# medvedevgroup/TwoPaCo

Measured on AMD Instinct MI355X. Metric: kmers_hashed_per_sec, higher is better.
Workload: dtype u64

## Files before the change

### include/twopaco_hip.h

```cpp
#ifndef TWOPACO_HIP_H_
#define TWOPACO_HIP_H_

#include <stddef.h>
#include <stdint.h>

#ifdef __cplusplus
extern "C" {
#endif

typedef struct tpc_ctx tpc_ctx;

#define TPC_MAX_Q 64
#define TPC_INVALID_VERTEX INT64_MAX

enum {
    TPC_K_FILTER_RESET = 0,
    TPC_K_INSERT = 1,
    TPC_K_QUERY = 2,
    TPC_K_COMPACT = 3,
    TPC_K_FILTER2 = 4,
    TPC_K_SCAN2 = 5,
    TPC_K_SORT = 6,
    TPC_K_EMIT = 7,
    TPC_K_SPLIT = 8,
// ... 44 lines not shown
                         uint32_t *bins_host);

int tpc_pass1_query(tpc_ctx *ctx, uint64_t lo, uint64_t hi, uint64_t *n_marks);
int tpc_pass1_query_begin(tpc_ctx *ctx, uint64_t lo, uint64_t hi);

int tpc_pass2_filter(tpc_ctx *ctx, uint64_t abundance, uint64_t *n_true, uint64_t *n_false, uint64_t *table_size);

int tpc_pass2_marks(tpc_ctx *ctx, uint64_t *n_marks);
int tpc_pass2_mark_owners(tpc_ctx *ctx, uint32_t world, uint64_t *pos_dev, int32_t *owner_dev);
int tpc_pass2_filter_positions(tpc_ctx *ctx, const uint64_t *pos_dev, uint64_t n, uint64_t abundance, uint64_t *n_true, uint64_t *n_false,
                               uint64_t *table_size);
int tpc_pass2_mark_records(tpc_ctx *ctx, uint32_t world, uint64_t *records_dev, int32_t *owner_dev);
int tpc_pass2_filter_records(tpc_ctx *ctx, const uint64_t *records_dev, uint64_t n, uint64_t abundance, uint64_t *n_true, uint64_t *n_false,
                             uint64_t *table_size);
int tpc_pass2_aggregate_records(tpc_ctx *ctx, uint32_t world, uint64_t abundance, uint64_t *records_dev, int32_t *owner_dev, uint64_t *n_records);
int tpc_pass2_filter_aggregated(tpc_ctx *ctx, const uint64_t *records_dev, uint64_t n, uint64_t abundance, uint64_t *n_true, uint64_t *n_false,
                                uint64_t *table_size);
int tpc_shard_permute_rows(tpc_ctx *ctx, const uint64_t *src_dev, const uint32_t *perm_dev, uint64_t n, int row_words, uint64_t *dst_dev);

int tpc_junctions_finalize(tpc_ctx *ctx, uint64_t *n_junctions);

int tpc_key_words(const tpc_ctx *ctx);

int tpc_junction_keys(tpc_ctx *ctx, uint64_t *keys_host);

int tpc_junction_keys_raw(tpc_ctx *ctx, uint64_t *keys_host, uint64_t *n);
int tpc_junction_keys_set(tpc_ctx *ctx, const uint64_t *keys_host, uint64_t n);
int tpc_junction_keys_export(tpc_ctx *ctx, uint64_t *dst_dev, uint64_t cap_keys, uint64_t *n);
int tpc_junction_keys_import(tpc_ctx *ctx, const uint64_t *src_dev, uint64_t n, int append);

int64_t tpc_get_id(tpc_ctx *ctx, const char *kmer);

int tpc_emit(tpc_ctx *ctx, uint64_t *n_marked, uint64_t *n_valid);
int tpc_emit_fetch(tpc_ctx *ctx, uint64_t *g_host, int64_t *id_host);

int tpc_emit_export(tpc_ctx *ctx, uint64_t *g_dev, int64_t *id_dev);
int tpc_emit_import(tpc_ctx *ctx, const uint64_t *g_dev, const int64_t *id_dev, uint64_t n);

int tpc_emit_stream(tpc_ctx *ctx, const uint64_t *rec_start, const uint64_t *rec_len, uint32_t n_rec, uint64_t *n_bytes, uint64_t *n_records);
int tpc_emit_stream_fetch(tpc_ctx *ctx, uint64_t offset, uint64_t nbytes, void *dst_host);

int tpc_shard_chunk(const tpc_ctx *ctx, uint64_t *chunk_lo, uint64_t *chunk_hi);
int tpc_emit_stream_partial(tpc_ctx *ctx, const uint64_t *rec_start, const uint64_t *rec_len, uint32_t n_rec, uint64_t *cnt_host, uint32_t *flags_host);
int tpc_emit_stream_part(tpc_ctx *ctx, const uint64_t *rec_start, const uint64_t *rec_len, uint32_t n_rec, const uint32_t *gflags_host,
                         const uint64_t *e_scan_host, const uint64_t *s_scan_host, const uint64_t *before_host, uint32_t r_last,
                         uint64_t chunk_lo, uint64_t chunk_hi, uint64_t slot0, uint64_t n_slots, uint64_t *n_bytes);
int tpc_host_alloc(void **ptr, uint64_t bytes);
void tpc_host_free(void *ptr);

int tpc_shard_verify_local(tpc_ctx *ctx);

int tpc_shard_periodic_copy(tpc_ctx *ctx);
int tpc_periodic_download(tpc_ctx *ctx, uint32_t *qs_host, uint32_t *planes_host, uint32_t *ins_host);

#define TPC_SHARD_INSERT 0
#define TPC_SHARD_QUERY 1
int tpc_shard_config(tpc_ctx *ctx, uint32_t rank, uint32_t world);
int tpc_shard_plan(tpc_ctx *ctx, int pass, uint64_t lo, uint64_t hi, uint64_t *geom);
int tpc_shard_hash(tpc_ctx *ctx, int pass, uint64_t batch, uint64_t lo, uint64_t hi, void *send_regions_dev, void *send_counts_dev,
                   uint64_t *n_overflow);
int tpc_shard_plan_both(tpc_ctx *ctx, uint64_t lo, uint64_t hi, uint64_t *geom_insert , uint64_t *geom_query );
int tpc_shard_hash_begin(tpc_ctx *ctx, int pass, uint64_t batch, uint64_t lo, uint64_t hi, void *send_regions_dev, void *send_counts_dev);
int tpc_shard_hash_end(tpc_ctx *ctx, int pass, uint64_t *n_overflow);
int tpc_shard_overflow_get(tpc_ctx *ctx, int pass, void *dst_dev, uint64_t n);
int tpc_shard_overflow_set(tpc_ctx *ctx, int pass, const void *src_dev, uint64_t n);
int tpc_shard_apply(tpc_ctx *ctx, int pass, uint64_t batch, const void *recv_regions_dev, const void *recv_counts_dev, uint64_t *n_survivors);
int tpc_shard_pack(tpc_ctx *ctx, int pass, const void *send_regions_dev, const void *send_counts_dev, void *packed_dev, uint64_t *bytes_per_dest_host);
int tpc_shard_apply_packed(tpc_ctx *ctx, int pass, uint64_t batch, const void *recv_packed_dev, const void *recv_counts_dev, uint64_t *n_survivors);
int tpc_shard_apply_inplace(tpc_ctx *ctx, int pass, uint64_t batch, const void *recv_regions_dev, const void *recv_counts_dev,
                            const void *send_regions_dev, const void *send_counts_dev, uint64_t *n_survivors);
int tpc_shard_survivors(tpc_ctx *ctx, uint64_t *sid_dev);
int tpc_shard_survivors_home(tpc_ctx *ctx, uint64_t *tmp_dev, uint64_t *send_dev, uint64_t *counts_host);
int tpc_shard_verify_send(tpc_ctx *ctx, int fn, int fn_count, const uint64_t *sid_dev, uint64_t n, uint64_t *tmp_dev, uint64_t *send_dev, uint32_t *perm_dev,
                          uint64_t *counts_host);
int tpc_shard_finish(tpc_ctx *ctx, const uint64_t *sid_dev, uint64_t n, int fn_count, const uint8_t *hit_dev, const uint32_t *perm_dev, uint64_t *n_marked);
int tpc_shard_survivor_sources(tpc_ctx *ctx, const uint64_t *sid_dev, uint64_t n, int32_t *source_dev);
int tpc_shard_verify_addrs(tpc_ctx *ctx, int fn, int fn_count, const uint64_t *sid_dev, uint64_t n, uint64_t *addr_dev, int32_t *owner_dev);
int tpc_shard_probe(tpc_ctx *ctx, const uint64_t *addr_dev, uint64_t n, uint8_t *hit_dev);
int tpc_shard_mark(tpc_ctx *ctx, const uint64_t *sid_dev, uint64_t n);
int tpc_shard_route(tpc_ctx *ctx, const int32_t *owner_dev, uint64_t n, uint32_t *perm_dev, uint64_t *counts_host);
int tpc_shard_permute64(tpc_ctx *ctx, const uint64_t *src_dev, const uint32_t *perm_dev, uint64_t n, uint64_t *dst_dev);
int tpc_shard_select(tpc_ctx *ctx, const uint64_t *sid_dev, uint64_t n, int fn_count, const uint8_t *hit_dev, const uint32_t *perm_dev,
                     uint64_t *sid_out_dev, uint64_t *n_out);
int tpc_mask_export(tpc_ctx *ctx, uint32_t *dst_dev);
int tpc_mask_merge(tpc_ctx *ctx, const uint32_t *src_dev, uint32_t count);
int tpc_mask_export_padded(tpc_ctx *ctx, uint32_t *dst_dev, uint64_t total_words);
int tpc_mask_or_blocks(tpc_ctx *ctx, const uint32_t *blocks_dev, uint32_t count, uint64_t words, uint32_t *out_dev);
int tpc_mask_import(tpc_ctx *ctx, const uint32_t *src_dev);

int tpc_combine_info(tpc_ctx *ctx, uint32_t n_dest, uint64_t *info );
int tpc_combine_export(tpc_ctx *ctx, uint32_t n_dest, uint16_t *payload_dev, uint64_t cap_units, uint64_t *dir_dev, uint64_t *units_host);
int tpc_combine_merge(tpc_ctx *ctx, uint32_t n_src, const uint16_t *payload_dev, const uint64_t *src_base_host, const uint64_t *dir_dev, uint16_t *out_payload_dev,
                      uint64_t out_cap_units, uint64_t *out_dir_dev, uint64_t *units_host);
int tpc_combine_import(tpc_ctx *ctx, uint32_t n_src, uint32_t n_owner, const uint16_t *payload_dev, const uint64_t *src_base_host, const uint64_t *dir_dev, uint64_t dir_stride);
int tpc_combine_choose(uint32_t world, int L, uint64_t mean_export_units, double *bytes );
int tpc_filter_copy_out(tpc_ctx *ctx, uint64_t word0, uint64_t n_words, uint32_t *dst_dev);
int tpc_filter_copy_in(tpc_ctx *ctx, uint64_t word0, uint64_t n_words, const uint32_t *src_dev);

#define TPC_SEG_OK 0
#define TPC_SEG_CORRUPTED 1
#define TPC_SEG_ID_TOO_LARGE 2
int tpc_segments_build_host(tpc_ctx *ctx, const void *stream_host, uint64_t n_bytes, int k, const uint64_t *rec_start, const uint64_t *rec_len,
                            uint32_t n_rec, const uint64_t *amb_pos, uint64_t n_amb);
int tpc_segments_build_resident(tpc_ctx *ctx, int k, const uint64_t *rec_start, const uint64_t *rec_len, uint32_t n_rec, const uint64_t *amb_pos,
                                uint64_t n_amb);
int tpc_segments_counts(const tpc_ctx *ctx, uint64_t *counts );
// ... 106 lines not shown
```

### twopaco_amd/capi.py

```python
import ctypes
import os

import numpy as np

from .build import lib_dir

INVALID_VERTEX = (1 << 63) - 1
DISTANCES_TILE = 32
KERNELS = {"fused": 12, "filter_reset": 0, "insert": 1, "query": 2, "compact": 3, "filter2": 4, "scan2": 5, "sort": 6, "emit": 7, "split": 8,
           "shard_hash": 9, "shard_apply": 10, "stream": 11, "lookup": 13, "combine": 14, "segments": 15, "segtext": 16, "sketch": 17, "colors": 18, "links": 19, "bubbles": 20,
           "distances": 21, "components": 22, "superbubbles": 23, "anchors": 24, "locate": 25, "classes": 26, "tracks": 27, "variants": 28}

HIP_SYMBOLS = ["tpc_ctx_create", "tpc_ctx_destroy", "tpc_last_error", "tpc_set_params", "tpc_seq_upload",
               "tpc_run_begin", "tpc_filter_reset", "tpc_pass1_insert", "tpc_pass1_split_hist", "tpc_pass1_query", "tpc_pass2_filter",
               "tpc_junctions_finalize", "tpc_key_words", "tpc_junction_keys", "tpc_junction_keys_raw", "tpc_junction_keys_set", "tpc_get_id", "tpc_emit",
               "tpc_emit_fetch", "tpc_filter_words", "tpc_filter_download", "tpc_mask_words", "tpc_mask_download",
               "tpc_hash_dump", "tpc_kernel_ms", "tpc_set_option",
               "tpc_shard_config", "tpc_shard_plan", "tpc_shard_hash", "tpc_shard_overflow_get", "tpc_shard_overflow_set", "tpc_shard_apply",
               "tpc_shard_pack", "tpc_shard_apply_packed", "tpc_pass2_marks", "tpc_pass2_mark_owners", "tpc_pass2_filter_positions",
               "tpc_pass2_mark_records", "tpc_pass2_filter_records", "tpc_pass2_aggregate_records", "tpc_pass2_filter_aggregated", "tpc_shard_permute_rows", "tpc_emit_export", "tpc_emit_import",
               "tpc_shard_survivors", "tpc_shard_survivor_sources", "tpc_shard_verify_addrs", "tpc_shard_probe", "tpc_shard_mark", "tpc_mask_export", "tpc_mask_merge",
               "tpc_shard_route", "tpc_shard_permute64", "tpc_shard_select", "tpc_mask_export_padded", "tpc_mask_or_blocks", "tpc_mask_import",
               "tpc_emit_stream", "tpc_emit_stream_fetch", "tpc_host_alloc", "tpc_host_free", "tpc_get_stat", "tpc_filter_upload",
               "tpc_junction_keys_export", "tpc_junction_keys_import", "tpc_warmup", "tpc_preload", "tpc_reserve", "tpc_shard_chunk", "tpc_emit_stream_partial", "tpc_emit_stream_part",
               "tpc_shard_plan_both", "tpc_shard_hash_begin", "tpc_shard_hash_end", "tpc_shard_apply_inplace", "tpc_shard_survivors_home", "tpc_shard_verify_send", "tpc_shard_finish", "tpc_shard_verify_local", "tpc_shard_periodic_copy", "tpc_periodic_download",
               "tpc_pass1_query_begin", "tpc_combine_info", "tpc_combine_export", "tpc_combine_merge", "tpc_combine_import", "tpc_combine_choose", "tpc_filter_copy_out", "tpc_filter_copy_in",
               "tpc_segments_build_host", "tpc_segments_build_resident", "tpc_segments_counts", "tpc_segments_error", "tpc_segments_fetch_names", "tpc_segments_fetch_first",
               "tpc_segments_fetch_events", "tpc_segments_fetch_sequences", "tpc_segments_text_plan", "tpc_segments_text_fetch", "tpc_segments_text_write", "tpc_distinct_sketch",
               "tpc_segments_colors_build", "tpc_segments_colors_info", "tpc_segments_colors_fetch_rows", "tpc_segments_colors_fetch_presence", "tpc_segments_colors_fetch_hist",
               "tpc_segments_links_build", "tpc_segments_links_info", "tpc_segments_links_fetch_rows", "tpc_segments_links_fetch_first",
               "tpc_segments_bubbles_build", "tpc_segments_bubbles_info", "tpc_segments_bubbles_fetch_rows", "tpc_segments_bubbles_fetch_sides", "tpc_segments_bubbles_fetch_hist",
               "tpc_segments_distances_build", "tpc_segments_distances_info", "tpc_segments_distances_fetch",
               "tpc_segments_components_build", "tpc_segments_components_info", "tpc_segments_components_fetch_members", "tpc_segments_components_fetch_rows",
               "tpc_segments_components_fetch_presence",
               "tpc_segments_superbubbles_build", "tpc_segments_superbubbles_info", "tpc_segments_superbubbles_fetch_adjacency", "tpc_segments_superbubbles_fetch_exits",
               "tpc_segments_superbubbles_fetch_rows", "tpc_segments_superbubbles_fetch_members", "tpc_segments_superbubbles_fetch_presence",
               "tpc_segments_anchors_build", "tpc_segments_anchors_info", "tpc_segments_anchors_fetch_mates", "tpc_segments_anchors_fetch_rows",
               "tpc_segments_anchors_fetch_shared",
               "tpc_segments_edges_build", "tpc_segments_edges_info", "tpc_segments_locate", "tpc_segments_locate_info", "tpc_segments_locate_fetch_hits",
               "tpc_segments_locate_fetch_runs", "tpc_segments_locate_fetch_records", "tpc_segments_locate_fetch_shared",
               "tpc_segments_classes_build", "tpc_segments_classes_info", "tpc_segments_classes_fetch_members", "tpc_segments_classes_fetch_rows",
               "tpc_segments_classes_fetch_presence", "tpc_segments_classes_fetch_sets",
               "tpc_segments_tracks_build", "tpc_segments_tracks_info", "tpc_segments_tracks_fetch_rows", "tpc_segments_tracks_fetch_colors",
               "tpc_segments_tracks_fetch_depth",
               "tpc_segments_variants_build", "tpc_segments_variants_info", "tpc_segments_variants_fetch_traversals", "tpc_segments_variants_fetch_alleles",
               "tpc_segments_variants_fetch_presence", "tpc_segments_variants_fetch_sites", "tpc_segments_variants_fetch_hist"]
VARIANTS_NONE = 0xFFFFFFFF
TRACKS_ALL = 0xFFFFFFFF
SEGMENT_ERRORS = {0: None, 1: "The input is corrupted", 2: "A vertex id is too large, cannot generate GFA"}

_hip = None
_host = None


def combine_choose(world, L, mean_export_units):
    b = (ctypes.c_double * 3)()
    mode = hip().tpc_combine_choose(world, L, int(mean_export_units), b)
    return mode, [float(x) for x in b]


def _load(name):
    path = os.path.join(lib_dir(), name)
    if not os.path.exists(path):
        raise RuntimeError("%s is missing: run `python -c 'import __graft_entry__ as g; g.build()'` (no CPU fallback)" % path)
    return ctypes.CDLL(path, mode=ctypes.RTLD_GLOBAL)


def hip():
    global _hip
    if _hip is None:
        L = _load("libtwopaco_hip.so")
        u64, i64, p, ci = ctypes.c_uint64, ctypes.c_int64, ctypes.c_void_p, ctypes.c_int
        L.tpc_ctx_create.argtypes = [ci, ctypes.POINTER(p)]
        L.tpc_ctx_destroy.argtypes = [p]
        L.tpc_last_error.restype = ctypes.c_char_p
        L.tpc_last_error.argtypes = [p]
        L.tpc_set_params.argtypes = [p, ci, ci, ci, p]
        L.tpc_seq_upload.argtypes = [p, p, p, u64]
# ... 5 lines not shown
        L.tpc_pass2_filter.argtypes = [p, u64, p, p, p]
        L.tpc_junctions_finalize.argtypes = [p, p]
        L.tpc_key_words.argtypes = [p]
        L.tpc_junction_keys.argtypes = [p, p]
        L.tpc_junction_keys_raw.argtypes = [p, p, p]
        L.tpc_junction_keys_set.argtypes = [p, p, u64]
        L.tpc_junction_keys_export.argtypes = [p, p, u64, p]
        L.tpc_junction_keys_import.argtypes = [p, p, u64, ci]
        L.tpc_get_id.restype = i64
        L.tpc_get_id.argtypes = [p, ctypes.c_char_p]
        L.tpc_emit.argtypes = [p, p, p]
        L.tpc_emit_fetch.argtypes = [p, p, p]
        L.tpc_filter_words.restype = u64
        L.tpc_filter_words.argtypes = [p]
        L.tpc_filter_download.argtypes = [p, p]
        L.tpc_filter_upload.argtypes = [p, p]
        L.tpc_warmup.argtypes = [p]
        L.tpc_preload.argtypes = [ctypes.c_int]
        L.tpc_reserve.argtypes = [p, u64]
        L.tpc_mask_words.restype = u64
        L.tpc_mask_words.argtypes = [p]
        L.tpc_mask_download.argtypes = [p, ci, p]
        L.tpc_hash_dump.argtypes = [p, u64, u64, p]
        L.tpc_kernel_ms.restype = ctypes.c_double
        L.tpc_kernel_ms.argtypes = [p, ci]
        L.tpc_set_option.argtypes = [p, ctypes.c_char_p, i64]
        u32 = ctypes.c_uint32
        L.tpc_shard_config.argtypes = [p, u32, u32]
        L.tpc_shard_plan.argtypes = [p, ci, u64, u64, p]
        L.tpc_shard_hash.argtypes = [p, ci, u64, u64, u64, p, p, p]
        L.tpc_shard_plan_both.argtypes = [p, u64, u64, p, p]
        L.tpc_shard_hash_begin.argtypes = [p, ci, u64, u64, u64, p, p]
        L.tpc_shard_hash_end.argtypes = [p, ci, p]
        L.tpc_shard_overflow_get.argtypes = [p, ci, p, u64]
        L.tpc_shard_overflow_set.argtypes = [p, ci, p, u64]
        L.tpc_shard_apply.argtypes = [p, ci, u64, p, p, p]
        L.tpc_pass2_marks.argtypes = [p, p]
        L.tpc_pass2_mark_owners.argtypes = [p, u32, p, p]
        L.tpc_pass2_filter_positions.argtypes = [p, p, u64, u64, p, p, p]
        L.tpc_pass2_mark_records.argtypes = [p, u32, p, p]
        L.tpc_pass2_filter_records.argtypes = [p, p, u64, u64, p, p, p]
        L.tpc_pass2_aggregate_records.argtypes = [p, u32, u64, p, p, p]
        L.tpc_pass2_filter_aggregated.argtypes = [p, p, u64, u64, p, p, p]
        L.tpc_shard_permute_rows.argtypes = [p, p, p, u64, ci, p]
        L.tpc_shard_pack.argtypes = [p, ci, p, p, p, p]
        L.tpc_shard_apply_packed.argtypes = [p, ci, u64, p, p, p]
        L.tpc_shard_apply_inplace.argtypes = [p, ci, u64, p, p, p, p, p]
        L.tpc_shard_survivors_home.argtypes = [p, p, p, p]
        L.tpc_shard_verify_send.argtypes = [p, ci, ci, p, u64, p, p, p, p]
        L.tpc_shard_finish.argtypes = [p, p, u64, ci, p, p, p]
        L.tpc_shard_verify_local.argtypes = [p]
        L.tpc_shard_periodic_copy.argtypes = [p]
        L.tpc_periodic_download.argtypes = [p, p, p, p]
        L.tpc_pass1_query_begin.argtypes = [p, u64, u64]
        L.tpc_combine_info.argtypes = [p, u32, p]
        L.tpc_combine_export.argtypes = [p, u32, p, u64, p, p]
        L.tpc_combine_merge.argtypes = [p, u32, p, p, p, p, u64, p, p]
        L.tpc_combine_import.argtypes = [p, u32, u32, p, p, p, u64]
        L.tpc_combine_choose.argtypes = [u32, ci, u64, p]
        L.tpc_filter_copy_out.argtypes = [p, u64, u64, p]
        L.tpc_filter_copy_in.argtypes = [p, u64, u64, p]
        L.tpc_shard_survivors.argtypes = [p, p]
        L.tpc_shard_verify_addrs.argtypes = [p, ci, ci, p, u64, p, p]
        L.tpc_shard_survivor_sources.argtypes = [p, p, u64, p]
        L.tpc_shard_probe.argtypes = [p, p, u64, p]
        L.tpc_shard_mark.argtypes = [p, p, u64]
        L.tpc_mask_export.argtypes = [p, p]
        L.tpc_mask_merge.argtypes = [p, p, u32]
        L.tpc_shard_route.argtypes = [p, p, u64, p, p]
        L.tpc_shard_permute64.argtypes = [p, p, p, u64, p]
        L.tpc_shard_select.argtypes = [p, p, u64, ci, p, p, p, p]
        L.tpc_mask_export_padded.argtypes = [p, p, u64]
        L.tpc_mask_or_blocks.argtypes = [p, p, u32, u64, p]
        L.tpc_mask_import.argtypes = [p, p]
        L.tpc_emit_stream.argtypes = [p, p, p, u32, p, p]
        L.tpc_emit_stream_fetch.argtypes = [p, u64, u64, p]
        L.tpc_emit_import.argtypes = [p, p, p, u64]
        L.tpc_shard_chunk.argtypes = [p, p, p]
        L.tpc_emit_stream_partial.argtypes = [p, p, p, u32, p, p]
        L.tpc_emit_stream_part.argtypes = [p, p, p, u32, p, p, p, p, u32, u64, u64, u64, u64, p]
        L.tpc_segments_build_host.argtypes = [p, p, u64, ci, p, p, u32, p, u64]
        L.tpc_segments_build_resident.argtypes = [p, ci, p, p, u32, p, u64]
        L.tpc_segments_counts.argtypes = [p, p]
        L.tpc_segments_error.argtypes = [p, p, p]
        L.tpc_segments_fetch_names.argtypes = [p, u64, u64, p]
        L.tpc_segments_fetch_first.argtypes = [p, u64, u64, p]
        L.tpc_segments_fetch_events.argtypes = [p, u64, u64, p, p]
        L.tpc_segments_fetch_sequences.argtypes = [p, u64, u64, p]
        L.tpc_segments_text_plan.argtypes = [p, ci, p, p, p, p]
        L.tpc_segments_text_fetch.argtypes = [p, u64, u64, p]
        L.tpc_segments_text_write.argtypes = [p, ci, u64, u64, p]
        L.tpc_segments_colors_build.argtypes = [p, p, u32]
        L.tpc_segments_colors_info.argtypes = [p, p]
        L.tpc_segments_colors_fetch_rows.argtypes = [p, u64, u64, p, p, p, p]
        L.tpc_segments_colors_fetch_presence.argtypes = [p, u64, u64, p]
        L.tpc_segments_colors_fetch_hist.argtypes = [p, p, p]
        L.tpc_segments_links_build.argtypes = [p]
        L.tpc_segments_links_info.argtypes = [p, p]
        L.tpc_segments_links_fetch_rows.argtypes = [p, u64, u64, p, p, p]
        L.tpc_segments_links_fetch_first.argtypes = [p, u64, u64, p]
        L.tpc_segments_bubbles_build.argtypes = [p]
        L.tpc_segments_bubbles_info.argtypes = [p, p]
        L.tpc_segments_bubbles_fetch_rows.argtypes = [p, u64, u64, p, p, p, p]
        L.tpc_segments_bubbles_fetch_sides.argtypes = [p, u64, u64, p, p, p]
        L.tpc_segments_bubbles_fetch_hist.argtypes = [p, p]
        L.tpc_segments_distances_build.argtypes = [p]
# ... 863 lines not shown
    def shard_overflow_set(self, which, src_ptr, n):
        self._ck(hip().tpc_shard_overflow_set(self._h, which, src_ptr, n))

    def shard_apply(self, which, batch, recv_regions_ptr, recv_counts_ptr):
        n = ctypes.c_uint64(0)
        self._ck(hip().tpc_shard_apply(self._h, which, batch, recv_regions_ptr, recv_counts_ptr, ctypes.byref(n)))
        return n.value

    def shard_pack(self, which, send_regions_ptr, send_counts_ptr, packed_ptr, world):
        out = (ctypes.c_uint64 * world)()
        self._ck(hip().tpc_shard_pack(self._h, which, send_regions_ptr, send_counts_ptr, packed_ptr, out))
        return [int(x) for x in out]

    def shard_apply_packed(self, which, batch, recv_packed_ptr, recv_counts_ptr):
        n = ctypes.c_uint64(0)
        self._ck(hip().tpc_shard_apply_packed(self._h, which, batch, recv_packed_ptr, recv_counts_ptr, ctypes.byref(n)))
        return n.value

    def shard_apply_inplace(self, which, batch, recv_regions_ptr, recv_counts_ptr, send_regions_ptr, send_counts_ptr):
        n = ctypes.c_uint64(0)
        self._ck(hip().tpc_shard_apply_inplace(self._h, which, batch, recv_regions_ptr, recv_counts_ptr, send_regions_ptr, send_counts_ptr, ctypes.byref(n)))
        return n.value

    def shard_survivors_home(self, tmp_ptr, send_ptr, world):
        out = (ctypes.c_uint64 * world)()
        self._ck(hip().tpc_shard_survivors_home(self._h, tmp_ptr, send_ptr, out))
        return [int(x) for x in out]

    def shard_verify_send(self, fn, fn_count, sid_ptr, n, tmp_ptr, send_ptr, perm_ptr, world):
        out = (ctypes.c_uint64 * world)()
        self._ck(hip().tpc_shard_verify_send(self._h, fn, fn_count, sid_ptr, n, tmp_ptr, send_ptr, perm_ptr, out))
        return [int(x) for x in out]

    def shard_finish(self, sid_ptr, n, fn_count, hit_ptr, perm_ptr):
        m = ctypes.c_uint64(0)
        self._ck(hip().tpc_shard_finish(self._h, sid_ptr, n, fn_count, hit_ptr, perm_ptr, ctypes.byref(m)))
        return m.value

    def shard_periodic_copy(self):
        self._ck(hip().tpc_shard_periodic_copy(self._h))

    def periodic_download(self):
        nw = hip().tpc_mask_words(self._h)
        qs, planes, ins = np.zeros(nw, dtype=np.uint32), np.zeros((6, nw), dtype=np.uint32), np.zeros(nw, dtype=np.uint32)
        self._ck(hip().tpc_periodic_download(self._h, qs.ctypes.data, planes.ctypes.data, ins.ctypes.data))

        def bits(w):
            return np.unpackbits(w.astype("<u4").view(np.uint8), bitorder="little")

        dist = np.zeros(nw * 32, dtype=np.uint8)
        for b in range(6):
            dist |= bits(planes[b]) << b
        return bits(qs).astype(bool), dist, bits(ins).astype(bool)

    def shard_verify_local(self):
        self._ck(hip().tpc_shard_verify_local(self._h))

    def shard_survivors(self, sid_ptr):
        self._ck(hip().tpc_shard_survivors(self._h, sid_ptr))

    def shard_survivor_sources(self, sid_ptr, n, src_ptr):
        self._ck(hip().tpc_shard_survivor_sources(self._h, sid_ptr, n, src_ptr))

    def shard_verify_addrs(self, fn, fn_count, sid_ptr, n, addr_ptr, owner_ptr):
        self._ck(hip().tpc_shard_verify_addrs(self._h, fn, fn_count, sid_ptr, n, addr_ptr, owner_ptr))

    def shard_probe(self, addr_ptr, n, hit_ptr):
        self._ck(hip().tpc_shard_probe(self._h, addr_ptr, n, hit_ptr))

    def shard_mark(self, sid_ptr, n):
        self._ck(hip().tpc_shard_mark(self._h, sid_ptr, n))

    def mask_export(self, dst_ptr):
        self._ck(hip().tpc_mask_export(self._h, dst_ptr))

    def mask_merge(self, src_ptr, count):
        self._ck(hip().tpc_mask_merge(self._h, src_ptr, count))

    def mask_words(self):
        return int(hip().tpc_mask_words(self._h))

    def shard_route(self, owner_ptr, n, perm_ptr, world):
        counts = np.zeros(64, dtype=np.uint64)
        self._ck(hip().tpc_shard_route(self._h, owner_ptr, n, perm_ptr, counts.ctypes.data))
        return [int(x) for x in counts[:world]]

    def shard_permute64(self, src_ptr, perm_ptr, n, dst_ptr):
        self._ck(hip().tpc_shard_permute64(self._h, src_ptr, perm_ptr, n, dst_ptr))

    def shard_select(self, sid_ptr, n, fn_count, hit_ptr, perm_ptr, out_ptr):
        m = ctypes.c_uint64(0)
        self._ck(hip().tpc_shard_select(self._h, sid_ptr, n, fn_count, hit_ptr, perm_ptr, out_ptr, ctypes.byref(m)))
        return m.value

    def mask_export_padded(self, dst_ptr, total_words):
        self._ck(hip().tpc_mask_export_padded(self._h, dst_ptr, total_words))

    def mask_or_blocks(self, blocks_ptr, count, words, out_ptr):
        self._ck(hip().tpc_mask_or_blocks(self._h, blocks_ptr, count, words, out_ptr))

    def mask_import(self, src_ptr):
        self._ck(hip().tpc_mask_import(self._h, src_ptr))

    def combine_info(self, n_dest):
        g = np.zeros(8, dtype=np.uint64)
        self._ck(hip().tpc_combine_info(self._h, n_dest, g.ctypes.data))
# ... 175 lines not shown
```

### twopaco_amd/csrc/tpc_capi.hip

```cpp
#include "tpc_ctx.h"

namespace tpch {

int fail(tpc_ctx *c, int code, const char *fmt, ...)
{
    char buf[512];
    va_list ap;
    va_start(ap, fmt);
    vsnprintf(buf, sizeof buf, fmt, ap);
    va_end(ap);
    if (c) c->err = buf;
    return code;
}





TpcLaunch make_launch(const tpc_ctx *c)
{
    TpcLaunch a;
    a.P = c->P; a.tab = c->tab; a.bases = c->bases; a.nmask = c->nmask; a.n_text = c->n_text;
    a.n_tiles = c->n_tiles; a.filter = c->filter; a.stream = c->stream;
    a.stat_kernel = c->stat_kernel;
    a.stat_split = c->stat_split;
    if (c->P.k <= TPC_QSEED_MAXK) a.qseed = c->tab + TPC_TAB_WORDS;
    return a;
}

TpcLaunch make_launch_periodic(const tpc_ctx *c)
{
    TpcLaunch a = make_launch(c);
    if (c->periodic && c->periodic_valid) {
        if (c->periodic_any_q) a.per_qs = c->periodic;
        if (c->periodic_any_i) a.per_i = c->periodic + (size_t)(1 + TPC_PER_PLANES) * c->n_words_alloc;
    }
    return a;
}

void ensure_periodic(tpc_ctx *c)
{
    if (c->periodic_valid || !c->opt_periodic || !c->bases || !c->have_params || c->n_words_alloc == 0) return;
    if ((c->sh_world > 1 || c->text_windowed) && !c->opt_shard_periodic && !replicated(c)) return;
    TpcLaunch a = make_launch(c);
    const uint64_t w0 = c->text_windowed ? c->text_w0 : 0, w1 = c->text_windowed ? std::min(c->text_w1, c->n_words) : c->n_words;
    const uint64_t pos_hi = c->text_windowed ? c->text_w1 << 5 : ~0ull;
    uint32_t any[2] = {0, 0};
    uint32_t *flags = reinterpret_cast<uint32_t *>(c->counters + 6);
    if (hipMemsetAsync(flags, 0, sizeof any, c->stream) != hipSuccess) return;
    tpc_launch_periodic_build(a, nullptr, nullptr, 0, nullptr, w0, w1, w0 << 5, pos_hi, flags);
    if (hipMemcpyAsync(any, flags, sizeof any, hipMemcpyDeviceToHost, c->stream) != hipSuccess || hipStreamSynchronize(c->stream) != hipSuccess) return;
    c->periodic_any_q = any[0] != 0; c->periodic_any_i = any[1] != 0;
    if (any[0] || any[1]) {
        const size_t words = (size_t)(2 + TPC_PER_PLANES) * c->n_words_alloc;
        if (!c->periodic && hipMalloc((void **)&c->periodic, words * sizeof(uint32_t)) != hipSuccess) { (void)hipGetLastError(); c->periodic = nullptr; return; }
        if (hipMemsetAsync(c->periodic, 0, words * sizeof(uint32_t), c->stream) != hipSuccess) return;
        tpc_launch_periodic_build(a, c->periodic, c->periodic + c->n_words_alloc, c->n_words_alloc, c->periodic + (size_t)(1 + TPC_PER_PLANES) * c->n_words_alloc, w0, w1, w0 << 5, pos_hi, flags);
        if (hipStreamSynchronize(c->stream) != hipSuccess) return;
    }
    c->periodic_valid = true;
}

uint64_t rotln_host(uint64_t x, int L, int r)
{
    if (r == 0) return x;
    const uint64_t maskn = (1ull << (L - r)) - 1ull;
    return ((x & maskn) << r) | (x >> (L - r));
}

std::atomic<int> tpc_test_fail_mallocs{0};
hipError_t dev_malloc(tpc_ctx *c, void **p, size_t bytes)
{
    hipError_t e = hipErrorOutOfMemory;
    if (tpc_test_fail_mallocs.load(std::memory_order_relaxed) > 0 && tpc_test_fail_mallocs.fetch_sub(1) > 0) *p = nullptr; else e = hipMalloc(p, bytes);
    if (e == hipSuccess) return e;
    (void)hipGetLastError();
    if (!release_partition_buffers(c)) return e;
    e = hipMalloc(p, bytes);
    if (e != hipSuccess) *p = nullptr;
    return e;
}


int read_counter(tpc_ctx *c, int i, uint64_t *out)
{
    unsigned long long v = 0;
    HIPCHK(c, hipMemcpyAsync(&v, c->counters + i, sizeof v, hipMemcpyDeviceToHost, c->stream));
    HIPCHK(c, hipStreamSynchronize(c->stream));
    *out = v;
    return 0;
// ... 167 lines not shown
        if ((rc = read_counter(c, 2, &n))) return rc;
    }
    rc = ensure(c, c->marks, c->marks_cap, n);
    if (rc) return rc;
    if (n) tpc_launch_mask_scatter(c->stream, m, c->n_words, c->block_sums, c->marks);
    c->n_marks = n;
    return 0;
}

}

extern "C" {

int tpc_ctx_create(int device, tpc_ctx **out)
{
    if (!out) return -1;
    *out = nullptr;
    int n = 0;
    if (hipGetDeviceCount(&n) != hipSuccess || n <= 0) return -2;
    if (device < 0 || device >= n) return -3;
    if (hipSetDevice(device) != hipSuccess) return -4;
    tpc_ctx *c = new tpc_ctx();
    c->device = device;
    c->dbg_ovf = getenv("TPC_DEBUG_OVF") != nullptr; c->dbg_phases = getenv("TPC_PROFILE_PHASES") != nullptr; c->dbg_timing = getenv("TWOPACO_TIMING") != nullptr; c->no_lean = TpcEnv::get().no_lean;
    if (const char *e = getenv("TPC_SHARD_TIGHT")) c->opt_shard_tight = atoi(e) ? 1 : 0;
    if (hipStreamCreate(&c->stream) != hipSuccess) { delete c; return -5; }
    for (int i = 0; i < TPC_K_COUNT; i++) {
        if (hipEventCreate(&c->ev0[i]) != hipSuccess || hipEventCreate(&c->ev1[i]) != hipSuccess) { delete c; return -5; }
    }
    if (hipMalloc((void **)&c->tab, sizeof c->tab_host) != hipSuccess ||
        hipMalloc((void **)&c->counters, 8 * sizeof(unsigned long long)) != hipSuccess ||
        hipMalloc((void **)&c->route_scratch, 128 * sizeof(unsigned long long)) != hipSuccess) { delete c; return -6; }
    *out = c;
    return 0;
}

void tpc_ctx_destroy(tpc_ctx *c)
{
    if (!c) return;
    (void)hipSetDevice(c->device);
    (void)hipStreamSynchronize(c->stream);
    void *ptrs[] = { c->tab, c->bases_alloc, c->nmask_alloc, c->filter, c->rmask, c->mask, c->marks, c->block_sums, c->table,
                     c->keys, c->idtab, c->emit_id, c->stream_buf, c->counters, c->route_scratch, c->sh_off, c->scan_blocks, c->sort_scratch, c->seg.name, c->seg.first, c->seg.ev[0], c->seg.ev[1], c->seg.ev[2],
                     c->seg.rec, c->seg.amb, c->text_plan.off, c->text_plan.piece, c->text_names, c->text_win };
    for (void *p : ptrs) if (p) (void)hipFree(p);
    stream_part_release(c);
    colors_drop(c);
    links_drop(c);
    anchors_drop(c);
    edges_drop(c);
    for (void *p : c->pbuf) if (p) (void)hipFree(p);
    for (void *p : c->ikeep) if (p) (void)hipFree(p);
    if (c->periodic) (void)hipFree(c->periodic);
    if (c->cmb_base) (void)hipFree(c->cmb_base);
    if (c->cmb_cur) (void)hipFree(c->cmb_cur);
    if (c->ikeep_ovf) (void)hipFree(c->ikeep_ovf);
    if (c->iovf_cnt) (void)hipFree(c->iovf_cnt);
    if (c->iovf_off) (void)hipFree(c->iovf_off);
    for (int i = 0; i < TPC_K_COUNT; i++) { if (c->ev0[i]) (void)hipEventDestroy(c->ev0[i]); if (c->ev1[i]) (void)hipEventDestroy(c->ev1[i]); }
    if (c->stream2) (void)hipStreamDestroy(c->stream2);
    if (c->stream) (void)hipStreamDestroy(c->stream);
    delete c;
}

const char *tpc_last_error(const tpc_ctx *c) { return c ? c->err.c_str() : "null context"; }

int tpc_set_option(tpc_ctx *c, const char *name, int64_t value)
{
    if (!c || !name) return -1;
    if (!strcmp(name, "insert_test_first")) { c->opt_test_first = value != 0; return 0; }
    if (!strcmp(name, "insert_mode")) { c->opt_insert_mode = (int)value; return 0; }
    if (!strcmp(name, "slice_bits")) { c->opt_slice_bits = (int)value; return 0; }
    if (!strcmp(name, "query_mode")) { c->opt_query_mode = (int)value; return 0; }
    if (!strcmp(name, "part_budget_bytes")) { c->opt_part_budget = value; return 0; }
    if (!strcmp(name, "part_levels")) { c->opt_part_levels = (int)value; return 0; }
    if (!strcmp(name, "shard_tight_regions")) { c->opt_shard_tight = value ? 1 : 0; c->sh_have[0] = c->sh_have[1] = false; return 0; }
    if (!strcmp(name, "part_min_tiles")) { c->opt_part_min_tiles = value < 1 ? 1 : value; return 0; }
    if (!strcmp(name, "verify_marks")) { c->opt_verify_marks = value != 0; return 0; }
    if (!strcmp(name, "mark_bucket_bits")) { tpc_test_mark_bucket_bits = (int)value; return 0; }
    if (!strcmp(name, "mark_region_cap")) { tpc_test_mark_region_cap = (int)value; return 0; }
    if (!strcmp(name, "mark_slice_bits")) { tpc_test_mark_slice_bits = (int)value; return 0; }
    if (!strcmp(name, "qhash_pushes")) { tpc_opt_qhash_pushes = value == 8 ? 8 : 6; return 0; }
    if (!strcmp(name, "qhash_roll_scalars")) { tpc_opt_qhash_roll = value != 0; return 0; }
    if (!strcmp(name, "qhash_seed_scalars")) { tpc_opt_qhash_seed = value != 0; return 0; }
    if (!strcmp(name, "fuse_apply_lookup")) { c->opt_fuse = value != 0; return 0; }
    if (!strcmp(name, "test_q6_pb2")) { tpc_test_q6_pb2 = (int)value; return 0; }
    if (!strcmp(name, "insert_entry_fmt")) { tpc_test_insert_p3 = value == 3; return 0; }
    if (!strcmp(name, "shard_periodic_skip")) { c->opt_shard_periodic = value != 0; return 0; }
    if (!strcmp(name, "periodic_skip")) { c->opt_periodic = value != 0; if (!value) c->periodic_valid = false; return 0; }
    if (!strcmp(name, "test_tight_pinch")) { tpc_test_tight_pinch = (int)value; c->sh_have[0] = c->sh_have[1] = false; return 0; }
    if (!strcmp(name, "test_sched_cap")) { tpc_test_sched_cap = value > 0 ? (uint32_t)value : 0; return 0; }
    if (!strcmp(name, "test_mask_scan")) { tpc_test_mask_scan = value == 1 || value == 2 ? (int)value : 0; return 0; }
    if (!strcmp(name, "text_window")) { c->opt_text_window = value != 0; return 0; }
    if (!strcmp(name, "replicate_filter")) { c->opt_replicate = value != 0; return 0; }
    if (!strcmp(name, "test_force_anyq")) { tpc_test_force_anyq = value != 0; return 0; }
    if (!strcmp(name, "test_sketch_grid")) { tpc_test_sketch_grid = value > 0 ? (int)value : 0; return 0; }
    if (!strcmp(name, "test_links_slots_log2")) { c->opt_links_slots_log2 = (int)std::max<int64_t>(-1, std::min<int64_t>(value, 64)); return 0; }
    if (!strcmp(name, "test_edges_slots_log2")) { c->opt_edges_slots_log2 = (int)std::max<int64_t>(-1, std::min<int64_t>(value, 64)); return 0; }
    if (!strcmp(name, "test_edges_hash_bits")) { c->opt_edges_hash_bits = (int)std::max<int64_t>(-1, std::min<int64_t>(value, 65)); return 0; }
    if (!strcmp(name, "test_locate_grid")) { c->opt_locate_grid = value > 0 ? (int)std::min<int64_t>(value, 1 << 20) : 0; return 0; }
    if (!strcmp(name, "test_distances_chunk_words")) { c->opt_distances_chunk_words = (int)std::max<int64_t>(-1, std::min<int64_t>(value, 1 << 20)); return 0; }
    if (!strcmp(name, "test_components_step_limit")) { c->opt_components_step_limit = (int)std::max<int64_t>(-1, std::min<int64_t>(value, 0x7FFFFFFF)); return 0; }
    if (!strcmp(name, "test_classes_slots_log2")) { c->opt_classes_slots_log2 = (int)std::max<int64_t>(-1, std::min<int64_t>(value, 64)); return 0; }
    if (!strcmp(name, "test_classes_hash_bits")) { c->opt_classes_hash_bits = (int)std::max<int64_t>(-1, std::min<int64_t>(value, 65)); return 0; }
    if (!strcmp(name, "test_classes_grid")) { c->opt_classes_grid = value > 0 ? (int)std::min<int64_t>(value, 1 << 20) : 0; return 0; }
    if (!strcmp(name, "test_classes_wide")) { c->opt_classes_wide = (int)std::max<int64_t>(-1, std::min<int64_t>(value, 3)); return 0; }
    if (!strcmp(name, "test_tracks_grid")) { c->opt_tracks_grid = value > 0 ? (int)std::min<int64_t>(value, 1 << 20) : 0; return 0; }
    if (!strcmp(name, "test_variants_grid")) { c->opt_variants_grid = value > 0 ? (int)std::min<int64_t>(value, 1 << 20) : 0; return 0; }
    if (!strcmp(name, "test_fail_mallocs")) { tpc_test_fail_mallocs.store(value > 0 ? (int)value : 0); return 0; }
    return fail(c, -1, "unknown option %s", name);
}

int tpc_preload(int device)
{
    if (hipSetDevice(device) != hipSuccess) { (void)hipGetLastError(); return -10; }
    const bool timing = getenv("TWOPACO_TIMING") != nullptr;
    int (*const warm[4])() = { tpc_warm_partition, tpc_warm_qpartition, tpc_warm_pass2, tpc_warm_stream };
    const char *const name[4] = { "partition", "qpartition", "pass2", "stream" };
    for (int i = 0; i < 4; i++) {
        const auto t0 = std::chrono::steady_clock::now();
        if (warm[i]() != 0) return -10;
        if (timing) fprintf(stderr, "[timing]     code object %s: %.1f ms\n", name[i], std::chrono::duration<double, std::milli>(std::chrono::steady_clock::now() - t0).count());
    }
    return 0;
}

int tpc_warmup(tpc_ctx *c)
{
    if (!c) return -1;
    return tpc_preload(c->device);
}

int64_t tpc_get_stat(const tpc_ctx *c, const char *name)
{
    if (!c || !name) return -1;
    if (!strcmp(name, "insert_path")) return c->stat_path[0];
    if (!strcmp(name, "query_path")) return c->stat_path[1];
    if (!strcmp(name, "insert_entry_fmt")) return c->stat_fmt[0];
    if (!strcmp(name, "query_entry_fmt")) return c->stat_fmt[1];
    if (!strcmp(name, "insert_hash_kernel")) return c->stat_kernel[0];
    if (!strcmp(name, "query_hash_kernel")) return c->stat_kernel[1];
    if (!strcmp(name, "query_verify_kernel")) return c->stat_kernel[2];
    if (!strcmp(name, "query_hash_form")) return c->stat_kernel[3];
    if (!strcmp(name, "query_hash_seed")) return c->stat_kernel[4];
    if (!strcmp(name, "split_kernel")) return c->stat_split[0];
    if (!strcmp(name, "split_phases")) return c->stat_split[1];
    if (!strcmp(name, "query_hash_seed_maxk")) return TPC_QSEED_MAXK;
    if (!strcmp(name, "query_mark_path")) return c->stat_mark_path;
    if (!strcmp(name, "query_mark_fallback")) return c->stat_mark_fallback;
    if (!strcmp(name, "insert_batches")) return c->stat_batches[0];
    if (!strcmp(name, "query_batches")) return c->stat_batches[1];
    if (!strcmp(name, "query_tiles_per_batch")) return c->stat_q_plan[0];
    if (!strcmp(name, "query_b1")) return c->stat_q_plan[1];
    if (!strcmp(name, "query_b2")) return c->stat_q_plan[2];
    if (!strcmp(name, "query_begun")) return c->stat_q_begun;
    if (!strcmp(name, "filter2_retries")) return c->stat_filter2_retries;
    if (!strcmp(name, "aggregate_retries")) return c->stat_aggregate_retries;
    if (!strcmp(name, "filter2_counted")) return c->stat_filter2_counted;
    if (!strcmp(name, "fused_lookups")) return c->stat_fused;
    if (!strcmp(name, "query_overflow_entries")) return c->stat_query_overflow;
    if (!strcmp(name, "insert_overflow_entries")) return c->stat_insert_overflow;
    if (!strcmp(name, "periodic_skip")) return c->periodic_valid ? 1 : 0;
    if (!strcmp(name, "pbuf_releases")) return c->stat_pbuf_releases;
    if (!strcmp(name, "distances_tile")) return TPC_DISTANCES_TILE;
    if (!strcmp(name, "text_words")) return (int64_t)(c->text_w1 - c->text_w0);
    if (!strcmp(name, "text_word_begin")) return (int64_t)c->text_w0;
    if (!strcmp(name, "text_word_end")) return (int64_t)c->text_w1;
    if (!strcmp(name, "periodic_any_query")) return c->periodic_valid && c->periodic_any_q ? 1 : 0;
    if (!strcmp(name, "periodic_any_insert")) return c->periodic_valid && c->periodic_any_i ? 1 : 0;
    if (!strcmp(name, "text_write_us")) return c->text_write_us;
    if (!strcmp(name, "text_wait_us")) return c->text_wait_us;
    if (!strcmp(name, "text_window_bytes")) return c->text_window_bytes;
    if (!strcmp(name, "device_free_bytes") || !strcmp(name, "device_total_bytes")) {
        size_t free_b = 0, total_b = 0;
        if (hipSetDevice(c->device) != hipSuccess || hipMemGetInfo(&free_b, &total_b) != hipSuccess) { (void)hipGetLastError(); return -1; }
        return (int64_t)(name[7] == 'f' ? free_b : total_b);
    }
    if (!strcmp(name, "mask_scan_form")) return tpc_stat_mask_scan_form.load(std::memory_order_relaxed);
    if (!strcmp(name, "round_marks")) return c->marks_valid ? (int64_t)c->n_marks : -1;
    return -1;
}

int tpc_set_params(tpc_ctx *c, int k, int L, int q, const uint64_t *seed_table)
{
    if (!c || !seed_table) return -1;
    if (q < 1 || q > TPC_MAX_Q) return fail(c, -1, "q=%d unsupported (1..%d)", q, TPC_MAX_Q);
    if (L < 2 || L > 62) return fail(c, -1, "filter bits L=%d unsupported (2..62)", L);
    if (k < 1) return fail(c, -1, "k must be positive");
    const int C = (k + 4 + 31) / 32;
    if (C >= 20)
        return fail(c, -1, "The value of K is too big. Please refer to documentaion how to increase the max supported value of K.");
    HIPCHK(c, hipSetDevice(c->device));
    c->P.k = k; c->P.L = L; c->P.q = q; c->P.rk = k % L; c->P.lmask = (1ull << L) - 1ull;
    if (C != c->C && c->keys) {
        (void)hipFree(c->keys);
        c->keys = nullptr; c->keys_cap = 0;
    }
    c->C = C;
    memset(c->tab_host, 0, sizeof c->tab_host);
    for (int i = 0; i < q; i++)
        for (int ch = 0; ch < 5; ch++) {
            const uint64_t h = seed_table[i * 5 + ch];
            if (h > c->P.lmask) return fail(c, -1, "seed table entry exceeds L bits");
            c->tab_host[i * 5 + ch] = h;
            c->tab_host[TPC_TAB_HK + i * 5 + ch] = rotln_host(h, L, c->P.rk);
        }
    if (k <= TPC_QSEED_MAXK)
        for (int t = 0; t < k; t++)
            for (int ch = 0; ch < 5; ch++) {
                const int rc = ch == 4 ? 4 : 3 - ch;
                c->tab_host[TPC_TAB_WORDS + (t * 5 + ch) * 2] = rotln_host(c->tab_host[ch], L, (k - 1 - t) % L);
                c->tab_host[TPC_TAB_WORDS + (t * 5 + ch) * 2 + 1] = rotln_host(c->tab_host[rc], L, t % L);
            }
    HIPCHK(c, hipMemcpy(c->tab, c->tab_host, sizeof c->tab_host, hipMemcpyHostToDevice));
    const uint64_t fw = filter_words_for(L, c->opt_replicate ? 1 : c->sh_world);
    c->sh_have[0] = c->sh_have[1] = false;
    c->pending_lists = false; c->cmb_have_geo = false;
    if (fw != c->filter_words) {
        if (c->filter) (void)hipFree(c->filter);
        c->filter = nullptr;
        HIPCHK(c, hipMalloc((void **)&c->filter, fw * sizeof(uint32_t)));
        c->filter_words = fw;
    }
    c->have_params = true;
    c->periodic_valid = false;
    c->pending_apply = false;
    c->qb_valid = false;
    c->n_keys = 0; c->finalized = false; c->rounds_done = 0; c->mask_dirty = false; c->marks_valid = false; c->rmask_sums_valid = false;
    return 0;
}

int tpc_seq_upload(tpc_ctx *c, const uint64_t *bases, const uint32_t *nmask, uint64_t n_text)
{
    if (!c || !bases || !nmask || n_text < 2) return fail(c, -1, "bad text");
    HIPCHK(c, hipSetDevice(c->device));
    const auto t_begin = std::chrono::steady_clock::now();
    c->qb_valid = false;
    const uint64_t nw = (n_text + 31) / 32;
    if (!((nmask[0] & 1u) && ((nmask[(n_text - 1) >> 5] >> ((n_text - 1) & 31)) & 1u)))
        return fail(c, -1, "text must start and end with the N separator");
    const uint64_t tiles = (nw + TPC_TILE_THREADS - 1) / TPC_TILE_THREADS;
    const uint64_t alloc = ((n_text / TPC_RUN + 512) / 512) * 512 + TPC_XW_MAX + 2;
    uint64_t w0 = 0, w1 = alloc;
    const bool windowed = c->opt_text_window && c->sh_world > 1;
    if (windowed) {
        const uint64_t t512 = (n_text / TPC_RUN + 512) / 512, chunk = (t512 + c->sh_world - 1) / c->sh_world;
        const uint64_t ta = std::min<uint64_t>(t512, (uint64_t)c->sh_rank * chunk), tb = std::min<uint64_t>(t512, ta + chunk);
        w0 = ta * 512 > 0 ? ta * 512 - 1 : 0;
        w1 = std::min<uint64_t>(alloc, tb * 512 + TPC_XW_MAX + 2);
        if (w1 <= w0) w1 = w0 + 1;
    }
    for (void *p : { (void *)c->bases_alloc, (void *)c->nmask_alloc, (void *)c->rmask, (void *)c->mask, (void *)c->block_sums, (void *)c->periodic })
        if (p) (void)hipFree(p);
    c->periodic = nullptr; c->periodic_valid = false;
    c->bases = nullptr; c->nmask = nullptr; c->bases_alloc = nullptr; c->nmask_alloc = nullptr; c->rmask = nullptr; c->mask = nullptr; c->block_sums = nullptr;
    const uint64_t wn = w1 - w0;
    HIPCHK(c, dev_malloc(c, (void **)&c->bases_alloc, wn * sizeof(uint64_t)));
    HIPCHK(c, dev_malloc(c, (void **)&c->nmask_alloc, wn * sizeof(uint32_t)));
    HIPCHK(c, dev_malloc(c, (void **)&c->rmask, alloc * sizeof(uint32_t)));
    HIPCHK(c, dev_malloc(c, (void **)&c->mask, alloc * sizeof(uint32_t)));
    HIPCHK(c, dev_malloc(c, (void **)&c->block_sums, (alloc / 256 + 2 + 64) * sizeof(uint64_t)));
    HIPCHK(c, hipMemsetAsync(c->bases_alloc, 0, wn * sizeof(uint64_t), c->stream));
    HIPCHK(c, hipMemsetAsync(c->nmask_alloc, 0xFF, wn * sizeof(uint32_t), c->stream));
    HIPCHK(c, hipMemsetAsync(c->rmask, 0, alloc * sizeof(uint32_t), c->stream));
    HIPCHK(c, hipMemsetAsync(c->mask, 0, alloc * sizeof(uint32_t), c->stream));
    const uint64_t ce = std::min(nw, w1);
    uint32_t last_word = 0;
    if (ce > w0) {
        HIPCHK(c, hipMemcpyAsync(c->bases_alloc, bases + w0, (ce - w0) * sizeof(uint64_t), hipMemcpyHostToDevice, c->stream));
        HIPCHK(c, hipMemcpyAsync(c->nmask_alloc, nmask + w0, (ce - w0) * sizeof(uint32_t), hipMemcpyHostToDevice, c->stream));
        if ((n_text & 31) && ce == nw) {
            last_word = nmask[nw - 1] | (~0u << (n_text & 31));
            HIPCHK(c, hipMemcpyAsync(c->nmask_alloc + (nw - 1 - w0), &last_word, sizeof last_word, hipMemcpyHostToDevice, c->stream));
        }
    }
    HIPCHK(c, hipStreamSynchronize(c->stream));
    if (c->dbg_timing)
        fprintf(stderr, "[timing]   tpc_seq_upload (allocations, %.0f MB host to device): %.1f ms\n", (double)(ce > w0 ? (ce - w0) * 12 : 0) / 1e6,
                std::chrono::duration<double, std::milli>(std::chrono::steady_clock::now() - t_begin).count());
    c->bases = c->bases_alloc - w0;
    c->nmask = c->nmask_alloc - w0;
    c->text_windowed = windowed; c->text_w0 = w0; c->text_w1 = w1;
    c->pending_apply = false;
    c->n_text = n_text; c->n_words = (n_text >> 5) + 1; c->n_words_alloc = alloc; c->n_tiles = tiles;
    c->text_uploads++;
    c->n_keys = 0; c->finalized = false; c->rounds_done = 0; c->mask_dirty = false; c->marks_valid = false; c->rmask_sums_valid = false;
    return 0;
}

int tpc_run_begin(tpc_ctx *c)
{
    if (!c) return -1;
    c->n_keys = 0; c->finalized = false; c->rounds_done = 0; c->mask_dirty = false; c->marks_valid = false; c->rmask_sums_valid = false;
    c->n_marks = 0; c->n_emit = 0; c->keys_host.clear();
    return 0;
}

int tpc_filter_reset(tpc_ctx *c)
{
    if (!c || !c->have_params) return fail(c, -1, "set_params first");
    c->filter_zero_pending = true;
    c->pending_apply = false;
    c->pending_shard = false;
    c->pending_lists = false;
    c->ev_used[TPC_K_FILTER_RESET] = false;
    return 0;
}

int tpc_pass1_insert(tpc_ctx *c, uint64_t lo, uint64_t hi, uint64_t *n_kmers)
{
    if (!c || !c->have_params || !c->bases) return fail(c, -1, "set_params and seq_upload first");
    if (c->sh_world > 1 && !c->opt_replicate) return fail(c, -1, "the filter is sharded: use tpc_shard_hash / tpc_shard_apply");
    HIPCHK(c, hipSetDevice(c->device));
    const bool gated = !(lo == 0 && hi >= c->P.lmask);
    { int rc0 = flush_pending_apply(c); if (rc0) return rc0; }
    c->qb_valid = false;
    ensure_periodic(c);
    if (n_kmers) HIPCHK(c, hipMemsetAsync(c->counters, 0, sizeof(unsigned long long), c->stream));
    uint64_t t_begin, t_end;
    pass_tiles(c, t_begin, t_end);
    TpcPartPlan pl;
    const double m_ins = gated ? range_mass(c, lo, hi) : 1.0;
    const double ins_frac = gated ? std::min(1.0, (1.0 - (1.0 - m_ins) * (1.0 - m_ins)) * 1.15) : 1.0;
    const uint64_t tiles = pass_tile_count(c);
    uint64_t batches = 1;
    bool defer = false;
    bool part = ((c->opt_insert_mode != 1 && !(c->opt_insert_mode == 0 && c->P.L < 28)) || replicated(c)) && part_hash_supported(c);
    if (replicated(c) && !part && c->P.q <= TPC_KERNEL_MAXQ)
        return fail(c, -1, "a replicated multi-GPU pass needs the partitioned hash kernels (q=%d, L=%d, slice_bits=%d are outside what they cover)", c->P.q, c->P.L, c->opt_slice_bits);
    if (part) {
        const int64_t budget = part_budget(c);
        for (;; batches = next_batches(batches)) {
            const uint64_t per = (tiles + batches - 1) / batches;
            if (!tpc_part_plan(c->P.L, c->P.q, c->opt_slice_bits, per, ins_frac, pl, c->opt_part_levels)) { part = false; break; }
            if ((int64_t)(std::max(tpc_part_buf1_bytes(pl), tpc_part_buf3_bytes(pl)) + tpc_part_buf2_bytes(pl)) <= budget || (int64_t)per <= c->opt_part_min_tiles) break;
        }
        if (part && c->opt_insert_mode == 0 && batches > 1 && !replicated(c)) {
            const double per_slice = (double)c->P.q * ins_frac * (double)pl.n_tiles * 512 * TPC_RUN / (double)(1ull << (c->P.L - pl.slice_bits));
            if (per_slice < (double)(1ull << pl.slice_bits) / 800.0) part = false;
        }
    }
    if (part) {
        size_t need[tpc_ctx::NPBUF] = { std::max(tpc_part_buf1_bytes(pl), tpc_part_buf3_bytes(pl)), tpc_part_cnt1_bytes(pl), tpc_part_buf2_bytes(pl), tpc_part_cnt2_bytes(pl),
                                        pl.ovf_cap * sizeof(uint64_t), 32 * sizeof(unsigned long long), 0, 0, 0, 0, tpc_part_cnt3_bytes(pl), 0 };
        TpcQPlan qpl;
        const bool qpart = plan_query(c, lo, hi, gated, qpl);
        for (int i = 0; i < tpc_ctx::NPBUF && qpart; i++) need[i] = std::max(need[i], qpart_need(qpl, i));
        for (int i = 0; i < tpc_ctx::NPBUF && part; i++) if (need[i]) part = ensure_pbuf(c, i, need[i]);
        defer = part && c->opt_fuse && batches == 1 && qpart && pl.b3 == 0 && qpl.b3 == 0 && qpl.slice_bits == pl.slice_bits &&
                qpl.b1 == pl.b1 && qpl.b2 == pl.b2 && (qpl.fmt == 6 || pl.fmt2 == 0);
        if (defer) {
            const size_t want[2] = { tpc_part_buf2_bytes(pl), tpc_part_cnt2_bytes(pl) };
            for (int i = 0; i < 2 && defer; i++) {
                if (want[i] <= c->ikeep_bytes[i]) continue;
                if (c->ikeep[i]) (void)hipFree(c->ikeep[i]);
                c->ikeep[i] = nullptr; c->ikeep_bytes[i] = 0;
                if (hipMalloc(&c->ikeep[i], want[i]) != hipSuccess) { (void)hipGetLastError(); defer = false; break; }
                c->ikeep_bytes[i] = want[i];
            }
        }
    }
    if (part) {
        pl.buf1 = (uint32_t *)c->pbuf[0]; pl.cnt1 = (uint32_t *)c->pbuf[1]; pl.buf2 = (uint32_t *)c->pbuf[2]; pl.cnt2 = (uint32_t *)c->pbuf[3];
        pl.ovf = (uint64_t *)c->pbuf[4]; pl.ovf_cur = (unsigned long long *)c->pbuf[5];
        pl.buf3 = (uint32_t *)c->pbuf[0]; pl.cnt3 = (uint32_t *)c->pbuf[10];
        if (defer) { pl.buf2 = (uint32_t *)c->ikeep[0]; pl.cnt2 = (uint32_t *)c->ikeep[1]; }
        bool fresh = c->filter_zero_pending;
        unsigned long long ov[2] = {0, 0};
        bool overflowed = false;
        uint64_t per_batch = 1;
// ... 148 lines not shown
        HIPCHK(c, hipMemcpyAsync(d_rec, rs.data(), rs.size() * sizeof(uint64_t), hipMemcpyHostToDevice, c->stream));
        HIPCHK(c, hipMemcpyAsync(d_rec + rs.size(), rl.data(), rl.size() * sizeof(uint64_t), hipMemcpyHostToDevice, c->stream));
    }
    tpc_launch_split_emask(c->stream, d_rec, d_rec + rs.size(), (uint32_t)rs.size(), c->P.k, c->n_words_alloc, d_em);
    HIPCHK(c, hipMemsetAsync(d_bins, 0, BINS * sizeof(uint32_t), c->stream));
    HIPCHK(c, hipMemsetAsync(c->filter, 0, c->filter_words * sizeof(uint32_t), c->stream));
    const uint64_t real = 1ull << c->P.L;
    const uint64_t bin_size = std::max<uint64_t>(1, real / BINS);
    {
        Timed t(c, TPC_K_SPLIT);
        tpc_launch_split(make_launch(c), d_em, d_bins, bin_size);
    }
    HIPCHK(c, hipMemcpyAsync(bins_host, d_bins, BINS * sizeof(uint32_t), hipMemcpyDeviceToHost, c->stream));
    HIPCHK(c, hipStreamSynchronize(c->stream));
    (void)hipFree(d_em);
    (void)hipFree(d_bins);
    (void)hipFree(d_rec);
    if (c->dbg_timing)
        fprintf(stderr, "[timing]   tpc_pass1_split_hist: %.1f ms in all, the split kernel %.1f ms\n", std::chrono::duration<double, std::milli>(std::chrono::steady_clock::now() - t_begin).count(),
                tpc_kernel_ms(c, TPC_K_SPLIT));
    return 0;
}

namespace {
int pass1_query_impl(tpc_ctx *c, uint64_t lo, uint64_t hi, uint64_t *n_marks, bool begin_only);
}

int tpc_pass1_query(tpc_ctx *c, uint64_t lo, uint64_t hi, uint64_t *n_marks) { return pass1_query_impl(c, lo, hi, n_marks, false); }

int tpc_pass1_query_begin(tpc_ctx *c, uint64_t lo, uint64_t hi) { return pass1_query_impl(c, lo, hi, nullptr, true); }

namespace {

int pass1_query_impl(tpc_ctx *c, uint64_t lo, uint64_t hi, uint64_t *n_marks, bool begin_only)
{
    if (!c || !c->have_params || !c->bases) return fail(c, -1, "set_params and seq_upload first");
    if (c->sh_world > 1 && !c->opt_replicate) return fail(c, -1, "the filter is sharded: use tpc_shard_hash / tpc_shard_apply");
    HIPCHK(c, hipSetDevice(c->device));
    const bool gated = !(lo == 0 && hi >= c->P.lmask);
    bool begun = !begin_only && c->qb_valid && c->qb_lo == lo && c->qb_hi == hi;
    c->qb_valid = false;
    auto fuses = [c](const TpcQPlan &p) {
        return c->pending_apply && !c->pending_shard && p.b3 == 0 && p.slice_bits == c->pending_pl.slice_bits && p.b1 == c->pending_pl.b1 && p.b2 == c->pending_pl.b2 &&
               (p.fmt == 6 || c->pending_pl.fmt2 == 0);
    };
    if (begun && c->pending_apply && !fuses(c->qb_pl)) {
        int rc0 = materialize_reset(c);
        if (rc0) return rc0;
        begun = false;
    }
    c->stat_q_begun = begun ? 1 : 0;
    c->marks_valid = false; c->rmask_sums_valid = false;
    ensure_periodic(c);
    TpcQPlan pl;
    uint64_t t_begin, t_end;
    pass_tiles(c, t_begin, t_end);
    bool part = begun ? (pl = c->qb_pl, true) : plan_query(c, lo, hi, gated, pl);
    if (replicated(c)) {
        if (!part && c->P.q <= TPC_KERNEL_MAXQ) return fail(c, -1, "a replicated multi-GPU pass needs the partitioned query (q=%d, L=%d, slice_bits=%d)", c->P.q, c->P.L, c->opt_slice_bits);
        if (!begun) HIPCHK(c, hipMemsetAsync(c->rmask, 0, c->n_words_alloc * sizeof(uint32_t), c->stream));
    }
    if (begin_only && !part) return 0;
    if (part)
        for (int i = 0; i < tpc_ctx::NPBUF && part; i++) if (qpart_need(pl, i)) part = ensure_pbuf(c, i, qpart_need(pl, i));
    const bool fused = !begin_only && part && fuses(pl);
    if (!fused && !begin_only) { int rc0 = materialize_reset(c); if (rc0) return rc0; }
    if (part) {
        pl.buf1 = (uint64_t *)c->pbuf[0]; pl.cnt1 = (uint32_t *)c->pbuf[1]; pl.buf2 = (uint64_t *)c->pbuf[2]; pl.cnt2 = (uint32_t *)c->pbuf[3];
        pl.ovf = (uint64_t *)c->pbuf[4]; pl.ovf_cur = (unsigned long long *)c->pbuf[5];
        pl.surv = (uint64_t *)c->pbuf[6]; pl.surv_cur = (unsigned long long *)c->pbuf[7];
        pl.off2 = (const uint64_t *)c->pbuf[8];
        if (c->off2_uploaded != pl.off2_host) {
            HIPCHK(c, hipMemcpy(c->pbuf[8], pl.off2_host.data(), pl.off2_host.size() * 8, hipMemcpyHostToDevice));
            c->off2_uploaded = pl.off2_host;
        }
        pl.buf3 = (uint64_t *)c->pbuf[0]; pl.cnt3 = (uint32_t *)c->pbuf[10]; pl.off3 = (const uint64_t *)c->pbuf[11];
        pl.bnd = (uint32_t *)c->pbuf[18];
        pl.pass = pl.mark_buf = pl.mark_cnt = nullptr;
        const int env_marks = TpcEnv::get().verify_marks;
        const bool mark_lists = env_marks >= 0 ? env_marks != 0 : c->opt_verify_marks != 0;
        if (mark_lists && tpc_qpart_bytes(pl, 19) <= c->pbytes[0]) tpc_qpart_mark_pointers(pl, c->pbuf[0]);
        if (pl.b3 && c->off3_uploaded != pl.off3_host) {
            HIPCHK(c, hipMemcpy(c->pbuf[11], pl.off3_host.data(), pl.off3_host.size() * 8, hipMemcpyHostToDevice));
            c->off3_uploaded = pl.off3_host;
        }
        unsigned long long f1[3] = {0, 0, 0}, f2 = 0, lost_marks = 0;
        bool overflowed = false, f1_counted = false;
        uint64_t per_batch = 1;
        {
            Timed t(c, TPC_K_QUERY);
            const uint64_t per = pl.n_tiles;
            per_batch = per;
            for (uint64_t t0 = t_begin; (t0 < t_end || t0 == t_begin) && !overflowed; t0 += per) {
                f1_counted = false;
                pl.tile0 = t0;
                pl.tile0_global = t0;
                pl.n_tiles = t0 < t_end ? std::min<uint64_t>(per, t_end - t0) : 0;
                const bool presplit = begun && t0 == t_begin;
                if (!presplit) {
                    HIPCHK(c, hipMemsetAsync(pl.ovf_cur, 0, 32 * sizeof(unsigned long long), c->stream));
                    HIPCHK(c, hipMemsetAsync(pl.surv_cur, 0, TPC_SURV_CUR_WORDS * sizeof(unsigned long long), c->stream));
                }
                if (begin_only) {
                    TpcQPlan p1 = pl;
                    p1.rbuf1 = p1.buf1; p1.rcnt1 = p1.cnt1;
                    if (tpc_launch_query_part_hash(make_launch_periodic(c), p1, c->rmask, lo, hi, gated) || tpc_launch_query_part_split(make_launch(c), p1))
                        return fail(c, -1, "partitioned query launch failed");
                    HIPCHK(c, hipGetLastError());
                    c->qb_valid = true; c->qb_lo = lo; c->qb_hi = hi;
                    c->qb_pl = pl; c->qb_pl.n_tiles = per;
                    return 0;
                }
                if (fused && t0 == t_begin) {
                    TpcQPlan p1 = pl;
                    p1.rbuf1 = p1.buf1; p1.rcnt1 = p1.cnt1;
                    p1.presplit = presplit;
                    c->pending_apply = false;
                    c->stat_fused++;
                    if (!presplit && tpc_launch_query_part_hash(make_launch_periodic(c), p1, c->rmask, lo, hi, gated)) return fail(c, -1, "partitioned query launch failed");
                    {
                        Timed tf(c, TPC_K_FUSED);
                        TpcLaunch af = make_launch(c);
                        af.ev_lookup0 = c->ev0[TPC_K_LOOKUP]; af.ev_lookup1 = c->ev1[TPC_K_LOOKUP]; c->ev_used[TPC_K_LOOKUP] = true;
                        const bool lists = c->pending_lists;
                        c->pending_lists = false;
                        if (tpc_launch_query_part_fused_lookup(af, p1, c->pending_pl, c->pending_fresh, c->pending_novf && !lists ? c->ikeep_ovf + c->ikeep_ovf_cap : nullptr,
                                                               c->pending_novf && !lists ? c->iovf_off : nullptr, lists ? &c->cmb_ls : nullptr)) return fail(c, -1, "fused lookup launch failed");
                    }
                    if (tpc_launch_query_verify(make_launch(c), p1, c->rmask)) return fail(c, -1, "verify launch failed");
                } else if (presplit) {
                    TpcQPlan p1 = pl;
                    p1.rbuf1 = p1.buf1; p1.rcnt1 = p1.cnt1;
                    p1.presplit = true;
                    if (tpc_launch_query_part_lookup(make_launch(c), p1) || tpc_launch_query_verify(make_launch(c), p1, c->rmask)) return fail(c, -1, "partitioned query launch failed");
                } else
                if (tpc_launch_query_partitioned(make_launch_periodic(c), pl, c->rmask, lo, hi, gated)) return fail(c, -1, "partitioned query launch failed");
                HIPCHK(c, hipMemcpyAsync(f1, pl.ovf_cur, sizeof f1, hipMemcpyDeviceToHost, c->stream));
                HIPCHK(c, hipMemcpyAsync(&f2, pl.surv_cur + 64, sizeof f2, hipMemcpyDeviceToHost, c->stream));
                if (t0 + per < t_end) {
                    unsigned long long sc[TPC_SURV_CUR_WORDS], batch_marks = 0;
                    const uint64_t w0 = t0 * 512, wn = std::min<uint64_t>(pl.n_tiles * 512, c->n_words > w0 ? c->n_words - w0 : 0);
                    if (wn) tpc_launch_mask_count(c->stream, c->rmask + w0, wn, c->block_sums, c->counters + 3);
                    HIPCHK(c, hipMemcpyAsync(sc, pl.surv_cur, sizeof sc, hipMemcpyDeviceToHost, c->stream));
                    if (wn) HIPCHK(c, hipMemcpyAsync(&batch_marks, c->counters + 3, sizeof batch_marks, hipMemcpyDeviceToHost, c->stream));
                    HIPCHK(c, hipStreamSynchronize(c->stream));
                    overflowed = f1[1] != 0 || f2 != 0;
                    lost_marks += f1[2];
                    f1_counted = true;
                    unsigned long long surv = 0;
                    for (int i = 0; i < 64; i++) surv += std::min<unsigned long long>(sc[i], pl.surv_cap);
                    if (surv > 0) pl.group_survivors = batch_marks * 4 >= surv;
                }
            }
            if (c->periodic_valid && c->periodic_any_q && c->periodic) tpc_launch_periodic_copy(c->stream, c->rmask, c->periodic, c->periodic + c->n_words_alloc, c->n_words_alloc, c->n_words);
            tpc_launch_mask_count(c->stream, c->rmask, c->n_words, c->block_sums, c->counters + 1);
        }
        HIPCHK(c, hipGetLastError());
        uint64_t n = 0;
        int rc = read_counter(c, 1, &n);
        if (rc) return rc;
        overflowed = overflowed || f1[1] != 0 || f2 != 0;
        if (!f1_counted) lost_marks += f1[2];
        c->stat_query_overflow = (int64_t)f1[0];
        c->stat_path[1] = (pl.b3 ? 3 : 2) + (overflowed ? 10 : 0);
        c->stat_mark_path = pl.pass && !overflowed ? 1 : 0;
        c->stat_mark_fallback = c->stat_mark_path ? (int64_t)lost_marks : 0;
        c->stat_fmt[1] = pl.fmt;
        c->stat_batches[1] = (int64_t)((pass_tile_count(c) + per_batch - 1) / per_batch);
        c->stat_q_plan[0] = (int64_t)per_batch; c->stat_q_plan[1] = pl.b1; c->stat_q_plan[2] = pl.b2;
        if (c->dbg_ovf) {
            unsigned long long sc[65];
            (void)hipMemcpy(sc, pl.surv_cur, sizeof sc, hipMemcpyDeviceToHost);
            unsigned long long tot = 0, most = 0;
            for (int i = 0; i < 64; i++) { tot += sc[i]; most = std::max(most, sc[i]); }
            fprintf(stderr, "[ovf] query: %llu overflow entries (cap %llu, flag %llu), survivors %llu (fullest list %llu of %llu, flag %llu) b1=%d b2=%d ppr=%d loads=%d\n", f1[0],
                    (unsigned long long)pl.ovf_cap, f1[1], tot, most, (unsigned long long)pl.surv_cap, f2, pl.b1, pl.b2, pl.pos_per_round, pl.loads);
            static const char *const dump_path = getenv("TPC_DUMP_SURV");
            if (const char *path = dump_path) {
                if (FILE *fp = fopen(path, "w")) {
                    for (int i = 0; i < 64; i++) {
                        const size_t n = (size_t)std::min<unsigned long long>(sc[i], pl.surv_cap);
                        std::vector<uint64_t> ids(n);
                        if (n) (void)hipMemcpy(ids.data(), pl.surv + (size_t)i * pl.surv_cap, n * 8, hipMemcpyDeviceToHost);
                        for (uint64_t v : ids) fprintf(fp, "%llu\n", (unsigned long long)v);
                    }
                    fclose(fp);
                }
            }
            static const bool dbg_regions = getenv("TPC_DEBUG_OVF_REGIONS") != nullptr;
            if (dbg_regions && f1[0]) {
                const size_t n = (size_t)std::min<unsigned long long>(f1[0], 1u << 22);
                std::vector<uint64_t> ent(2 * n);
                (void)hipMemcpy(ent.data(), pl.ovf, 2 * n * 8, hipMemcpyDeviceToHost);
                std::map<uint32_t, uint32_t> h;
                std::map<uint64_t, uint32_t> ha;
                for (size_t i = 0; i < n; i++) { h[(uint32_t)(ent[2 * i] >> pl.slice_bits)]++; ha[ent[2 * i]]++; }
                std::vector<std::pair<uint32_t, uint32_t>> top;
                for (auto &kv : h) top.push_back({kv.second, kv.first});
                std::sort(top.rbegin(), top.rend());
                fprintf(stderr, "[ovf]   %zu entries in %zu permuted slices, %zu distinct addresses; top:", n, h.size(), ha.size());
                for (size_t i = 0; i < std::min<size_t>(top.size(), 10); i++) fprintf(stderr, " slice %u x %u;", top[i].second, top[i].first);
                std::vector<std::pair<uint32_t, uint64_t>> topa;
                for (auto &kv : ha) topa.push_back({kv.second, kv.first});
                std::sort(topa.rbegin(), topa.rend());
                for (size_t i = 0; i < std::min<size_t>(topa.size(), 6); i++) fprintf(stderr, " addr %llx x %u (edge %llu pos %llu);", (unsigned long long)topa[i].second, topa[i].first, 0ull, 0ull);
                fprintf(stderr, "\n");
            }
// ... 49 lines not shown

uint64_t tpc_filter_words(const tpc_ctx *c) { return c ? c->filter_words : 0; }

int tpc_filter_download(tpc_ctx *c, uint32_t *words_host)
{
    if (!c || !c->filter) return -1;
    HIPCHK(c, hipSetDevice(c->device));
    { int rc0 = materialize_reset(c); if (rc0) return rc0; }
    HIPCHK(c, hipStreamSynchronize(c->stream));
    HIPCHK(c, hipMemcpy(words_host, c->filter, c->filter_words * sizeof(uint32_t), hipMemcpyDeviceToHost));
    return 0;
}

int tpc_filter_upload(tpc_ctx *c, const uint32_t *words_host)
{
    if (!c || !c->filter || !words_host) return -1;
    HIPCHK(c, hipSetDevice(c->device));
    HIPCHK(c, hipStreamSynchronize(c->stream));
    HIPCHK(c, hipMemcpy(c->filter, words_host, c->filter_words * sizeof(uint32_t), hipMemcpyHostToDevice));
    c->filter_zero_pending = false;
    c->pending_apply = false;
    return 0;
}

uint64_t tpc_mask_words(const tpc_ctx *c) { return c ? c->n_words : 0; }

int tpc_mask_download(tpc_ctx *c, int run_wide, uint32_t *words_host)
{
    if (!c || !c->rmask) return -1;
    HIPCHK(c, hipSetDevice(c->device));
    HIPCHK(c, hipStreamSynchronize(c->stream));
    HIPCHK(c, hipMemcpy(words_host, run_wide ? c->mask : c->rmask, c->n_words * sizeof(uint32_t), hipMemcpyDeviceToHost));
    return 0;
}

int tpc_periodic_download(tpc_ctx *c, uint32_t *qs_host, uint32_t *planes_host, uint32_t *ins_host)
{
    if (!c || !c->have_params || !c->bases || !qs_host || !planes_host || !ins_host) return fail(c, -1, "set_params and seq_upload first");
    HIPCHK(c, hipSetDevice(c->device));
    ensure_periodic(c);
    const size_t nw = c->n_words, stride = c->n_words_alloc;
    memset(qs_host, 0, nw * sizeof(uint32_t));
    memset(planes_host, 0, nw * TPC_PER_PLANES * sizeof(uint32_t));
    memset(ins_host, 0, nw * sizeof(uint32_t));
    if (!(c->periodic_valid && c->periodic && (c->periodic_any_q || c->periodic_any_i))) return 0;
    HIPCHK(c, hipStreamSynchronize(c->stream));
    HIPCHK(c, hipMemcpy(qs_host, c->periodic, nw * sizeof(uint32_t), hipMemcpyDeviceToHost));
    for (int b = 0; b < TPC_PER_PLANES; b++)
        HIPCHK(c, hipMemcpy(planes_host + (size_t)b * nw, c->periodic + (size_t)(1 + b) * stride, nw * sizeof(uint32_t), hipMemcpyDeviceToHost));
    HIPCHK(c, hipMemcpy(ins_host, c->periodic + (size_t)(1 + TPC_PER_PLANES) * stride, nw * sizeof(uint32_t), hipMemcpyDeviceToHost));
    return 0;
}

int tpc_hash_dump(tpc_ctx *c, uint64_t g0, uint64_t n, uint64_t *out_host)
{
    if (!c || !c->have_params || !c->bases) return -1;
    if (g0 + n + c->P.k > c->n_text) return fail(c, -1, "range past the text");
    if (c->text_windowed) return fail(c, -1, "this context holds only its window of the text");
    HIPCHK(c, hipSetDevice(c->device));
    uint64_t *d = nullptr;
    const size_t bytes = n * 2 * c->P.q * sizeof(uint64_t);
    HIPCHK(c, hipMalloc((void **)&d, bytes));
    tpc_launch_hash_dump(make_launch(c), g0, n, d);
    HIPCHK(c, hipMemcpy(out_host, d, bytes, hipMemcpyDeviceToHost));
    (void)hipFree(d);
    return 0;
}

double tpc_kernel_ms(const tpc_ctx *c, int which)
{
    if (c && which == TPC_K_SEGTEXT) return c->text_valid ? c->text_ms : -1.0;
    if (!c || which < 0 || which >= TPC_K_COUNT || !c->ev_used[which]) return -1.0;
    if (hipEventSynchronize(c->ev1[which]) != hipSuccess) return -1.0;
    float ms = 0;
    if (hipEventElapsedTime(&ms, c->ev0[which], c->ev1[which]) != hipSuccess) return -1.0;
    return ms;
}

}
```

### twopaco_amd/csrc/tpc_capi_shard.hip

```cpp
#include "tpc_ctx.h"

int tpc_shard_config(tpc_ctx *c, uint32_t rank, uint32_t world)
{
    if (!c) return -1;
    if (world == 0 || (world & (world - 1)) || rank >= world) return fail(c, -1, "world must be a power of two and rank < world");
    HIPCHK(c, hipSetDevice(c->device));
    c->sh_rank = rank; c->sh_world = world;
    c->sh_have[0] = c->sh_have[1] = false;
    c->pending_apply = false;
    if (c->have_params) {
        const uint64_t fw = filter_words_for(c->P.L, c->opt_replicate ? 1 : world);
        if (fw != c->filter_words) {
            if (c->filter) (void)hipFree(c->filter);
            c->filter = nullptr; c->filter_words = 0;
            HIPCHK(c, hipMalloc((void **)&c->filter, fw * sizeof(uint32_t)));
            c->filter_words = fw;
        }
        c->filter_zero_pending = true;
    }
    return 0;
}

int tpc_shard_plan(tpc_ctx *c, int pass, uint64_t lo, uint64_t hi, uint64_t *geom)
{
    if (!c || !c->have_params || !c->bases || !geom) return fail(c, -1, "set_params and seq_upload first");
    c->qb_valid = false;
    if (pass != TPC_SHARD_INSERT && pass != TPC_SHARD_QUERY) return fail(c, -1, "bad pass");
    HIPCHK(c, hipSetDevice(c->device));
    if (!part_hash_supported(c))
        return fail(c, -1, "a sharded filter needs the partitioned hash kernels: q=%d, L=%d, slice_bits=%d are outside what they cover (1..8 functions, or 9..16 with L - slice_bits <= 24)",
                    c->P.q, c->P.L, c->opt_slice_bits);
    const bool gated = !(lo == 0 && hi >= c->P.lmask);
    if (pass == TPC_SHARD_INSERT) { int rc0 = flush_pending_apply(c); if (rc0) return rc0; }
    if (c->opt_shard_periodic) ensure_periodic(c);
    const uint64_t W = c->sh_world, tiles = text_tiles512(c);
    const uint64_t per_total = (tiles + W - 1) / W;
    const double m = gated ? range_mass(c, lo, hi) : 1.0;
    uint64_t per = per_total;
    if (pass == TPC_SHARD_INSERT) {
        const double frac = gated ? std::min(1.0, (1.0 - (1.0 - m) * (1.0 - m)) * 1.15) : 1.0;
        TpcPartPlan &pl = c->sh_ipl;
        for (uint64_t batches = 1;; batches = next_batches(batches)) {
            per = (per_total + batches - 1) / batches;
            if (!tpc_part_plan_sharded(c->P.L, c->P.q, c->opt_slice_bits, per, frac, c->sh_rank, c->sh_world, pl, c->opt_part_levels, c->opt_shard_tight != 0))
                return fail(c, -1, "no sharded partition geometry for L=%d, slice_bits=%d, world=%u", c->P.L, c->opt_slice_bits, c->sh_world);
            if ((int64_t)(2 * tpc_part_buf1_bytes(pl) + tpc_part_buf2_bytes(pl) + tpc_part_buf3_bytes(pl)) <= part_budget(c) || (int64_t)per <= c->opt_part_min_tiles) break;
        }
        const size_t need[6] = { 0, 0, tpc_part_buf2_bytes(pl), tpc_part_cnt2_bytes(pl), pl.ovf_cap * sizeof(uint64_t), 32 * sizeof(unsigned long long) };
        for (int i = 2; i < 6; i++) if (!ensure_pbuf(c, i, need[i])) return fail(c, -10, "out of device memory for the partition buffers");
        if (!ensure_pbuf(c, 12, need[4]) || !ensure_pbuf(c, 13, need[5])) return fail(c, -10, "out of device memory for the partition buffers");
        if (pl.b3 && (!ensure_pbuf(c, 9, tpc_part_buf3_bytes(pl)) || !ensure_pbuf(c, 10, tpc_part_cnt3_bytes(pl)))) return fail(c, -10, "out of device memory for the partition buffers");
        pl.buf2 = (uint32_t *)c->pbuf[2]; pl.cnt2 = (uint32_t *)c->pbuf[3]; pl.ovf = (uint64_t *)c->pbuf[4]; pl.ovf_cur = (unsigned long long *)c->pbuf[5];
        pl.buf3 = (uint32_t *)c->pbuf[9]; pl.cnt3 = (uint32_t *)c->pbuf[10];
        c->sh_defer = false;
        if (c->opt_fuse && per == per_total && pl.b3 == 0) {
            const size_t want[2] = { tpc_part_buf2_bytes(pl), tpc_part_cnt2_bytes(pl) };
            bool ok = true;
            for (int i = 0; i < 2 && ok; i++) {
                if (want[i] <= c->ikeep_bytes[i]) continue;
                if (c->ikeep[i]) (void)hipFree(c->ikeep[i]);
// ... 26 lines not shown
            c->off3_uploaded = pl.off3_host;
        }
        pl.buf2 = (uint64_t *)c->pbuf[2]; pl.cnt2 = (uint32_t *)c->pbuf[3]; pl.ovf = (uint64_t *)c->pbuf[14]; pl.ovf_cur = (unsigned long long *)c->pbuf[15];
        pl.surv = (uint64_t *)c->pbuf[6]; pl.surv_cur = (unsigned long long *)c->pbuf[7]; pl.off2 = (const uint64_t *)c->pbuf[8];
        if (c->off2_uploaded != pl.off2_host) {
            HIPCHK(c, hipMemcpy(c->pbuf[8], pl.off2_host.data(), pl.off2_host.size() * 8, hipMemcpyHostToDevice));
            c->off2_uploaded = pl.off2_host;
        }
        geom[2] = tpc_qpart_bytes(pl, 0) / W; geom[3] = tpc_qpart_bytes(pl, 1) / W;
        geom[4] = 64 * pl.surv_cap; geom[5] = pl.ovf_cap; geom[6] = 16;
        geom[7] = pl.slice_bits; geom[8] = pl.b1; geom[9] = pl.b2; geom[10] = pl.perm_mult; geom[11] = pl.perm_inv; geom[12] = pl.b3;
    }
    c->sh_per[pass] = per;
    c->sh_batches[pass] = (per_total + per - 1) / per;
    c->sh_have[pass] = true;
    c->sh_have[1 - pass] = false;
    geom[0] = c->sh_batches[pass]; geom[1] = per;
    for (int i = 13; i < 16; i++) geom[i] = 0;
    return 0;
}

int tpc_shard_plan_both(tpc_ctx *c, uint64_t lo, uint64_t hi, uint64_t *geom_insert, uint64_t *geom_query)
{
    int rc = tpc_shard_plan(c, TPC_SHARD_INSERT, lo, hi, geom_insert);
    if (rc) return rc;
    if ((rc = tpc_shard_plan(c, TPC_SHARD_QUERY, lo, hi, geom_query))) return rc;
    TpcPartPlan &pl = c->sh_ipl;
    pl.buf2 = (uint32_t *)c->pbuf[2]; pl.cnt2 = (uint32_t *)c->pbuf[3]; pl.ovf = (uint64_t *)c->pbuf[4]; pl.ovf_cur = (unsigned long long *)c->pbuf[5];
    pl.buf3 = (uint32_t *)c->pbuf[9]; pl.cnt3 = (uint32_t *)c->pbuf[10];
    if (tpc_part_buf2_bytes(pl) > c->pbytes[2] || tpc_part_cnt2_bytes(pl) > c->pbytes[3] || (pl.b3 && (tpc_part_buf3_bytes(pl) > c->pbytes[9] || tpc_part_cnt3_bytes(pl) > c->pbytes[10])))
        return fail(c, -10, "partition buffers smaller than the insert's plan");
    c->sh_have[TPC_SHARD_INSERT] = true;
    return 0;
}

namespace {

int shard_hash_impl(tpc_ctx *c, int pass, uint64_t batch, uint64_t lo, uint64_t hi, void *send_regions, void *send_counts, uint64_t *n_overflow, bool async)
{
    if (!c || (pass != TPC_SHARD_INSERT && pass != TPC_SHARD_QUERY) || !c->sh_have[pass]) return fail(c, -1, "tpc_shard_plan for this pass first");
    c->qb_valid = false;
    if (!send_regions || !send_counts || batch >= c->sh_batches[pass]) return fail(c, -1, "bad arguments");
    if (c->sh_async[pass]) return fail(c, -1, "a hash of this pass is still in flight: tpc_shard_hash_end first");
    HIPCHK(c, hipSetDevice(c->device));
    if (async && !c->stream2) HIPCHK(c, hipStreamCreate(&c->stream2));
    hipStream_t st = async ? c->stream2 : c->stream;
    const bool gated = !(lo == 0 && hi >= c->P.lmask);
    const uint64_t W = c->sh_world, per = c->sh_per[pass], tiles = text_tiles512(c);
    const uint64_t chunk = (tiles + W - 1) / W, c0 = std::min(tiles, c->sh_rank * chunk), c1 = std::min(tiles, c0 + chunk);
    const uint64_t t0 = c0 + batch * per;
    const uint64_t n = t0 < c1 ? std::min<uint64_t>(per, c1 - t0) : 0;
    unsigned long long *ov = c->sh_ov_host[pass];
    ov[0] = ov[1] = 0;
    TpcLaunch a = c->opt_shard_periodic ? make_launch_periodic(c) : make_launch(c);
    a.stream = st;
    if (pass == TPC_SHARD_INSERT) {
        TpcPartPlan pl = c->sh_ipl;
        pl.tile0 = t0; pl.n_tiles = n;
        pl.buf1 = (uint32_t *)send_regions; pl.cnt1 = (uint32_t *)send_counts;
        HIPCHK(c, hipMemsetAsync(pl.ovf_cur, 0, 32 * sizeof(unsigned long long), st));
        if (async) {
            if (tpc_launch_insert_part_hash(a, pl, lo, hi, gated, nullptr)) return fail(c, -1, "hash launch failed");
        } else {
            Timed t(c, TPC_K_SHARD_HASH);
            if (tpc_launch_insert_part_hash(a, pl, lo, hi, gated, nullptr)) return fail(c, -1, "hash launch failed");
        }
        HIPCHK(c, hipMemcpyAsync(ov, pl.ovf_cur, 2 * sizeof(unsigned long long), hipMemcpyDeviceToHost, st));
#ifdef TPC_BINS3_DEBUG
        if (!async) {
            unsigned long long d[12];
            (void)hipMemcpy(d, pl.ovf_cur, sizeof d, hipMemcpyDeviceToHost);
            fprintf(stderr, "[bins3] insert hash: ring-lost %llu region-lost %llu retry-iterations %llu waited-and-stored %llu (overflow list %llu) ppr=%d cap1=%llu\n", d[8], d[9], d[10], d[11], d[0], pl.pos_per_round, (unsigned long long)pl.cap1);
        }
#endif
    } else {
        TpcQPlan pl = c->sh_qpl;
        pl.tile0 = t0; pl.n_tiles = n; pl.tile0_global = t0;
        pl.buf1 = (uint64_t *)send_regions; pl.cnt1 = (uint32_t *)send_counts;
        if (!async && !c->pending_apply) { int rc0 = materialize_reset(c); if (rc0) return rc0; }
        HIPCHK(c, hipMemsetAsync(pl.ovf_cur, 0, 32 * sizeof(unsigned long long), st));
        if (!async) HIPCHK(c, hipMemsetAsync(pl.surv_cur, 0, TPC_SURV_CUR_WORDS * sizeof(unsigned long long), st));
        if (batch == 0) HIPCHK(c, hipMemsetAsync(c->rmask, 0, c->n_words_alloc * sizeof(uint32_t), st));
        c->marks_valid = false; c->rmask_sums_valid = false;
        if (async) {
            if (tpc_launch_query_part_hash(a, pl, c->rmask, lo, hi, gated)) return fail(c, -1, "hash launch failed");
        } else {
            Timed t(c, TPC_K_SHARD_HASH);
            if (tpc_launch_query_part_hash(a, pl, c->rmask, lo, hi, gated)) return fail(c, -1, "hash launch failed");
        }
        HIPCHK(c, hipMemcpyAsync(ov, pl.ovf_cur, 2 * sizeof(unsigned long long), hipMemcpyDeviceToHost, st));
    }
    HIPCHK(c, hipGetLastError());
    if (async) { c->sh_async[pass] = true; return 0; }
    HIPCHK(c, hipStreamSynchronize(c->stream));
    if (n_overflow) *n_overflow = ov[1] ? (1ull << 62) : (uint64_t)ov[0];
    return 0;
}

}

int tpc_shard_hash(tpc_ctx *c, int pass, uint64_t batch, uint64_t lo, uint64_t hi, void *send_regions, void *send_counts, uint64_t *n_overflow)
{
    return shard_hash_impl(c, pass, batch, lo, hi, send_regions, send_counts, n_overflow, false);
}

int tpc_shard_hash_begin(tpc_ctx *c, int pass, uint64_t batch, uint64_t lo, uint64_t hi, void *send_regions, void *send_counts)
{
// ... 472 lines not shown
```

### twopaco_amd/csrc/tpc_ctx.h

```cpp
#pragma once
#include "../../include/twopaco_hip.h"
#include "tpc_internal.h"

#include <algorithm>
#include <atomic>
#include <cmath>
#include <chrono>
#include <cstdarg>
#include <cstdio>
#include <cstdlib>
#include <cstring>
#include <string>
#include <vector>
#include <map>

struct tpc_ctx {
    __attribute__((always_inline)) tpc_ctx() = default;
    int device = 0;
    hipStream_t stream = nullptr;
    std::string err;
    bool have_params = false;
    TpcHashParams P{};
    uint64_t tab_host[TPC_TAB_WORDS + TPC_QSEED_WORDS]{};
    uint64_t *tab = nullptr;
    int C = 1;
    uint64_t *bases = nullptr;
    uint32_t *nmask = nullptr;
    uint64_t n_text = 0, n_words = 0, n_words_alloc = 0, n_tiles = 0;
    uint64_t text_uploads = 0;
    uint32_t *periodic = nullptr;
    bool periodic_valid = false;
    bool periodic_any_q = false, periodic_any_i = false;
    int opt_periodic = 1;
    bool opt_shard_periodic = false;
    uint64_t *bases_alloc = nullptr;
    uint32_t *nmask_alloc = nullptr;
    int opt_text_window = 0;
    bool text_windowed = false;
    uint64_t text_w0 = 0, text_w1 = 0;
    uint32_t *filter = nullptr;
    uint64_t filter_words = 0;
    uint32_t *rmask = nullptr, *mask = nullptr;
    bool mask_dirty = false;
    int rounds_done = 0;
    uint64_t *marks = nullptr;
    uint64_t marks_cap = 0, n_marks = 0;
    bool marks_valid = false;
    bool rmask_sums_valid = false;
    uint64_t rmask_sums_n = 0;
    uint64_t *block_sums = nullptr;
    uint64_t *scan_blocks = nullptr;
    void *table = nullptr;
    uint64_t table_cap = 0, table_alloc = 0;
    uint64_t *keys = nullptr;
    uint64_t n_keys = 0, keys_cap = 0;
    bool finalized = false;
    std::vector<uint64_t> keys_host;
    uint32_t *idtab = nullptr;
    uint64_t idtab_cap = 0;
    size_t idtab_bytes = 0;
    void *sort_scratch = nullptr;
    size_t sort_scratch_bytes = 0;
    int64_t *emit_id = nullptr;
    uint64_t emit_cap = 0, n_emit = 0;
    uint32_t *stream_buf = nullptr;
    uint64_t stream_cap = 0, stream_bytes = 0;
    uint64_t *sp_rec = nullptr, *sp_vscan = nullptr, *sp_cnt = nullptr, *sp_lo = nullptr;
    uint32_t *sp_flags = nullptr;
    uint32_t sp_n_rec = 0;
    struct Segments {
        int64_t *name = nullptr;
        uint32_t *first = nullptr;
        uint32_t *ev[3] = {nullptr, nullptr, nullptr};
        uint32_t n_rec = 0;
        uint64_t events = 0, segments = 0, named = 0, table_bytes = 0, slots = 0, peak_bytes = 0;
        uint64_t err_slot = 0;
        int err_kind = 0;
        bool valid = false;
        uint64_t *rec = nullptr, *amb = nullptr;
        uint64_t n_amb = 0, text_n = 0, text_uploads = 0;
        const void *text_bases = nullptr;
        int k = 0;
    } seg;
    TpcTextPlan text_plan;
    void *text_names = nullptr;
    uint8_t *text_win = nullptr;
    size_t text_win_cap = 0;
// ... 113 lines not shown
    int opt_variants_grid = 0;
    int opt_tracks_grid = 0;
    int opt_edges_slots_log2 = 0;
    int opt_edges_hash_bits = 0;
    int opt_locate_grid = 0;
    int opt_components_step_limit = 0;
    int opt_distances_chunk_words = 0;
    unsigned long long *counters = nullptr;
    unsigned long long *route_scratch = nullptr;
    uint64_t *sh_off = nullptr;
    size_t sh_off_bytes = 0;
    int opt_test_first = 0;
    int opt_insert_mode = 0;
    int opt_slice_bits = 20;
    bool filter_zero_pending = false;
    static constexpr int NPBUF = 19;
    void *pbuf[NPBUF] = {};
    size_t pbytes[NPBUF] = {};
    std::vector<uint64_t> off2_uploaded, off3_uploaded;
    int opt_part_levels = 0;
    int opt_shard_tight = 1;
    int stat_path[2] = {0, 0};
    int64_t stat_batches[2] = {0, 0};
    mutable int stat_kernel[5] = {0, 0, 0, 0, 0};
    mutable int stat_split[2] = {0, 0};
    int stat_fmt[2] = {0, 0};
    int64_t stat_filter2_retries = 0;
    int64_t stat_aggregate_retries = 0;
    int stat_filter2_counted = 0;
    int opt_verify_marks = 1;
    int stat_mark_path = 0;
    int64_t stat_mark_fallback = 0;
    int64_t opt_part_min_tiles = 256;
    int64_t opt_part_budget = 0;
    int opt_query_mode = 0;
    int opt_fuse = 1;
    bool pending_apply = false;
    bool pending_fresh = false;
    bool pending_shard = false;
    TpcPartPlan pending_pl;
    void *ikeep[2] = {nullptr, nullptr};
    size_t ikeep_bytes[2] = {0, 0};
    uint64_t *ikeep_ovf = nullptr;
    uint64_t ikeep_ovf_cap = 0;
    uint64_t pending_novf = 0;
    uint32_t *iovf_cnt = nullptr;
    uint64_t *iovf_off = nullptr;
    uint32_t iovf_slices = 0;
    int64_t stat_fused = 0;
    int64_t stat_query_overflow = 0;
    int64_t stat_insert_overflow = 0;
    int64_t stat_pbuf_releases = 0;
    uint32_t sh_rank = 0, sh_world = 1;
    TpcPartPlan sh_ipl;
    TpcQPlan sh_qpl;
    bool sh_have[2] = {false, false};
    uint64_t sh_per[2] = {0, 0}, sh_batches[2] = {0, 0};
    uint64_t sh_nsurv = 0;
    bool sh_defer = false;
    bool sh_ovf_set[2] = {false, false};
    hipStream_t stream2 = nullptr;
    bool sh_async[2] = {false, false};
    unsigned long long sh_ov_host[2][2] = {{0, 0}, {0, 0}};
    int opt_replicate = 0;
    bool qb_valid = false;
    uint64_t qb_lo = 0, qb_hi = 0;
    TpcQPlan qb_pl;
    int64_t stat_q_plan[3] = {0, 0, 0};
    int stat_q_begun = 0;
    bool pending_lists = false;
    TpcListSrc cmb_ls;
    TpcPartPlan cmb_geo;
    bool cmb_have_geo = false;
    uint64_t *cmb_base = nullptr;
    unsigned long long *cmb_cur = nullptr;
    hipEvent_t ev0[TPC_K_COUNT]{}, ev1[TPC_K_COUNT]{};
    bool ev_used[TPC_K_COUNT]{};
    bool dbg_ovf = false, dbg_phases = false, dbg_timing = false, no_lean = false;
    uint64_t reserve_text_bytes = 0;
};

namespace tpch {

int fail(tpc_ctx *c, int code, const char *fmt, ...);
TpcLaunch make_launch(const tpc_ctx *c);
TpcLaunch make_launch_periodic(const tpc_ctx *c);
void ensure_periodic(tpc_ctx *c);
uint64_t rotln_host(uint64_t x, int L, int r);
hipError_t dev_malloc(tpc_ctx *c, void **p, size_t bytes);
int read_counter(tpc_ctx *c, int i, uint64_t *out);
int materialize_reset(tpc_ctx *c);
int flush_pending_apply(tpc_ctx *c);
double range_mass(const tpc_ctx *c, uint64_t lo, uint64_t hi);
bool ensure_pbuf(tpc_ctx *c, int i, size_t need);
bool release_partition_buffers(tpc_ctx *c);
uint64_t filter_words_for(int L, uint32_t world);
int64_t part_budget(const tpc_ctx *c);
uint64_t next_batches(uint64_t b);
uint64_t text_tiles512(const tpc_ctx *c);
bool replicated(const tpc_ctx *c);
void pass_tiles(const tpc_ctx *c, uint64_t &t_begin, uint64_t &t_end);
uint64_t pass_tile_count(const tpc_ctx *c);
size_t qpart_need(const TpcQPlan &pl, int i);
bool part_hash_supported(const tpc_ctx *c);
bool plan_query(const tpc_ctx *c, uint64_t lo, uint64_t hi, bool gated, TpcQPlan &pl);
int compact_mask(tpc_ctx *c, const uint32_t *m);
void stream_part_release(tpc_ctx *c);
void colors_drop(tpc_ctx *c);
void links_drop(tpc_ctx *c);
void bubbles_drop(tpc_ctx *c);
void distances_drop(tpc_ctx *c);
void components_drop(tpc_ctx *c);
void superbubbles_drop(tpc_ctx *c);
void anchors_drop(tpc_ctx *c);
void edges_drop(tpc_ctx *c);
void locate_drop(tpc_ctx *c);
void classes_drop(tpc_ctx *c);
void tracks_drop(tpc_ctx *c);
void variants_drop(tpc_ctx *c);

#define HIPCHK(c, expr)                                                                         \
    do {                                                                                        \
        hipError_t e_ = (expr);                                                                 \
        if (e_ != hipSuccess) return tpch::fail(c, -10, "%s failed: %s", #expr, hipGetErrorString(e_)); \
    } while (0)

constexpr int TPC_DISTANCES_TILE = 32;

struct Timed {
    tpc_ctx *c;
    int which;
    Timed(tpc_ctx *c_, int w) : c(c_), which(w) { (void)hipEventRecord(c->ev0[w], c->stream); }
    ~Timed() { (void)hipEventRecord(c->ev1[which], c->stream); c->ev_used[which] = true; }
};

template <typename T>
int ensure(tpc_ctx *c, T *&p, uint64_t &cap, uint64_t need)
{
    if (need <= cap && p) return 0;
    if (p) (void)hipFree(p);
// ... 12 lines not shown
```

### twopaco_amd/csrc/tpc_internal.h

```cpp
#pragma once
#include "tpc_device.h"
#include <algorithm>
#include <atomic>
#include <cstdlib>
#include <vector>

struct TpcEnv {
    bool no_lean, rb_hash, verify_eager, gated_full;
    int verify_marks;
    int qhash_pushes, qhash_roll, qhash_seed;
    int ppr_insert, gated_loads, split_loads9;
    int slice_grid;
    static const TpcEnv &get()
    {
        static const TpcEnv e = [] {
            TpcEnv v;
            v.no_lean = getenv("TPC_NO_LEAN") != nullptr;
            v.rb_hash = getenv("TPC_RB_HASH") != nullptr;
            const char *lz = getenv("TPC_VERIFY_LAZY");
            v.verify_eager = lz && lz[0] == '0';
            v.gated_full = getenv("TPC_GATED_FULL_REGIONS") != nullptr;
            const char *vm = getenv("TPC_VERIFY_MARKS");
            v.verify_marks = vm && vm[0] ? (vm[0] != '0' ? 1 : 0) : -1;
            const char *qp = getenv("TPC_QHASH_PUSHES");
// ... 6 lines not shown
            v.ppr_insert = p ? atoi(p) : 0;
            v.gated_loads = g ? atoi(g) : 0;
            const char *s9 = getenv("TPC_SPLIT_LOADS9");
            v.split_loads9 = s9 ? atoi(s9) : 0;
            const char *lg = getenv("TPC_LOOKUP_GRID");
            int n_cu = 0, dev = 0;
            if (hipGetDevice(&dev) != hipSuccess || hipDeviceGetAttribute(&n_cu, hipDeviceAttributeMultiprocessorCount, dev) != hipSuccess || n_cu <= 0) { (void)hipGetLastError(); n_cu = 256; }
            v.slice_grid = lg ? atoi(lg) : 2 * n_cu;
            return v;
        }();
        return e;
    }
};

inline uint32_t tpc_slice_grid(uint32_t n_slices)
{
    const int g = TpcEnv::get().slice_grid;
    return g > 0 ? std::min<uint32_t>(n_slices, (uint32_t)g) : n_slices;
}

extern int tpc_opt_qhash_pushes, tpc_opt_qhash_roll, tpc_opt_qhash_seed;
inline bool tpc_qhash_roll_scalars() { const int e = TpcEnv::get().qhash_roll; return (e >= 0 ? e : tpc_opt_qhash_roll) != 0; }
inline bool tpc_qhash_seed_scalars() { const int e = TpcEnv::get().qhash_seed; return (e >= 0 ? e : tpc_opt_qhash_seed) != 0; }
inline bool tpc_qhash_compact() { const int e = TpcEnv::get().qhash_pushes; return (e ? e : tpc_opt_qhash_pushes) != 8; }

#define TPC_TAB_MAXQ 64
#define TPC_KERNEL_MAXQ 16
#define TPC_TAB_HK (TPC_TAB_MAXQ * 5)
#define TPC_TAB_WORDS (2 * TPC_TAB_MAXQ * 5)
#define TPC_QSEED_MAXK 64
#define TPC_QSEED_WORDS (TPC_QSEED_MAXK * 5 * 2)

struct TpcLaunch {
    TpcHashParams P;
    const uint64_t *tab;
    const uint64_t *qseed = nullptr;
    const uint64_t *bases;
    const uint32_t *nmask;
    uint64_t n_text;
    uint64_t n_tiles;
    uint32_t *filter;
    hipStream_t stream;
    const uint32_t *per_i = nullptr, *per_qs = nullptr;
    uint64_t g_begin = 0, g_end = ~0ull;
    hipEvent_t ev_lookup0 = nullptr, ev_lookup1 = nullptr;
    int *stat_kernel = nullptr;
    int *stat_split = nullptr;
};
constexpr int TPC_PER_MAXP = 63;
constexpr int TPC_PER_PLANES = 6;
int tpc_launch_periodic_build(const TpcLaunch &a, uint32_t *qs, uint32_t *qd, uint64_t stride, uint32_t *ins, uint64_t w_begin, uint64_t w_end, uint64_t pos_lo, uint64_t pos_hi,
                              uint32_t *any);
int tpc_launch_periodic_copy(hipStream_t stream, uint32_t *rmask, const uint32_t *qs, const uint32_t *qd, uint64_t stride, uint64_t n_words);

int tpc_launch_insert(const TpcLaunch &a, uint64_t lo, uint64_t hi, bool gated, bool test, unsigned long long *n_kmers);
int tpc_launch_query(const TpcLaunch &a, uint32_t *rmask, uint64_t lo, uint64_t hi, bool gated, unsigned long long *n_marks);
int tpc_launch_split(const TpcLaunch &a, uint32_t *emask, uint32_t *bins, uint64_t bin_size);
int tpc_launch_split_emask(hipStream_t s, const uint64_t *d_rec_start, const uint64_t *d_rec_len, uint32_t n_rec, int k, uint64_t n_words, uint32_t *emask);
int tpc_launch_hash_dump(const TpcLaunch &a, uint64_t g0, uint64_t n, uint64_t *out);
int tpc_launch_insert_anyq(const TpcLaunch &a, uint64_t lo, uint64_t hi, bool gated, bool test, unsigned long long *n_kmers);
int tpc_launch_query_anyq(const TpcLaunch &a, uint32_t *rmask, uint64_t lo, uint64_t hi, bool gated, unsigned long long *n_marks);
int tpc_launch_split_anyq(const TpcLaunch &a, uint32_t *emask, uint32_t *bins, uint64_t bin_size);
extern int tpc_test_force_anyq;

struct TpcPartPlan {
    int slice_bits, b1, b2, pos_per_round;
    int b3 = 0;
    uint32_t perm_mult, perm_inv;
    uint64_t tile0, n_tiles;
    uint32_t nwg1, wpb;
    uint32_t wpb3 = 1;
    uint64_t cap1, cap2;
    uint64_t cap3 = 0;
    int fmt2 = 0;
    uint64_t ovf_cap;
    uint32_t *buf1, *cnt1, *buf2, *cnt2;
    uint32_t *buf3 = nullptr, *cnt3 = nullptr;
    uint64_t *ovf;
    unsigned long long *ovf_cur;
    uint32_t rank = 0, world = 1;
    const uint32_t *rbuf1 = nullptr, *rcnt1 = nullptr;
    const uint64_t *roff1 = nullptr;
    const uint32_t *rown1 = nullptr, *rowncnt1 = nullptr;
};
bool tpc_part_plan(int L, int q, int slice_bits, uint64_t n_tiles, double frac, TpcPartPlan &pl, int levels = 0);
size_t tpc_part_buf1_bytes(const TpcPartPlan &pl);
size_t tpc_part_cnt1_bytes(const TpcPartPlan &pl);
size_t tpc_part_buf2_bytes(const TpcPartPlan &pl);
size_t tpc_part_cnt2_bytes(const TpcPartPlan &pl);
size_t tpc_part_buf3_bytes(const TpcPartPlan &pl);
size_t tpc_part_cnt3_bytes(const TpcPartPlan &pl);
bool tpc_part_plan_sharded(int L, int q, int slice_bits, uint64_t n_tiles, double frac, uint32_t rank, uint32_t world, TpcPartPlan &pl, int levels = 0, bool tight = false,
                           bool packed = false);
int tpc_launch_insert_partitioned(const TpcLaunch &a, const TpcPartPlan &pl, uint64_t lo, uint64_t hi, bool gated, bool fresh,
                                  unsigned long long *n_kmers);
int tpc_launch_insert_part_hash(const TpcLaunch &a, const TpcPartPlan &pl, uint64_t lo, uint64_t hi, bool gated, unsigned long long *n_kmers);
int tpc_launch_insert_part_apply(const TpcLaunch &a, const TpcPartPlan &pl, bool fresh);

struct TpcQPlan {
    int slice_bits, b1, b2, pos_per_round, sub_rounds, loads;
    int b3 = 0, loads3 = 1;
    uint32_t wpb3 = 1;
    uint64_t cap2 = 0;
    std::vector<uint64_t> off3_host;
    uint64_t buf3_entries = 0;
    uint64_t *buf3 = nullptr;
    uint32_t *cnt3 = nullptr;
    const uint64_t *off3 = nullptr;
    uint32_t perm_mult, perm_inv;
    uint64_t tile0, n_tiles;
    uint64_t tile0_global = 0;
    uint32_t nwg1, wpb;
    uint64_t cap1;
    std::vector<uint64_t> off2_host;
    uint64_t buf2_entries;
    const uint64_t *off2;
    uint64_t ovf_cap;
    uint64_t surv_cap;
    uint64_t *buf1, *buf2;
    uint32_t *cnt1, *cnt2;
    uint64_t *ovf;
    unsigned long long *ovf_cur;
    uint64_t *surv;
    unsigned long long *surv_cur;
    uint32_t rank = 0, world = 1;
    const uint64_t *rbuf1 = nullptr;
    const uint32_t *rcnt1 = nullptr;
    const uint64_t *roff1 = nullptr;
    const uint64_t *rown1 = nullptr;
    const uint32_t *rowncnt1 = nullptr;
    bool group_survivors = true;
    int fmt = 0;
    bool presplit = false;
    uint32_t tiles_per_wg = 0, n_groups = 0, pb2 = 0;
    uint32_t *bnd = nullptr;
    uint32_t *pass = nullptr;
    uint32_t *mark_buf = nullptr;
    uint32_t *mark_cnt = nullptr;
    int MB = 0, mark_lnb = 0, mark_sub_bits = 0;
    uint32_t mark_nb = 0, mark_wg = 0, mark_cap = 0;
};
#define TPC_SURV_CUR_WORDS 72
bool tpc_qpart_plan(int L, int slice_bits, uint64_t n_tiles, double frac, TpcQPlan &pl, int levels = 0);
size_t tpc_qpart_bytes(const TpcQPlan &pl, int which);
void tpc_qpart_mark_pointers(TpcQPlan &pl, void *base);
bool tpc_qpart_plan_sharded(int L, int slice_bits, uint64_t n_tiles, double frac, uint32_t rank, uint32_t world, TpcQPlan &pl, int levels = 0, bool tight = false,
                            bool packed = false);
int tpc_launch_query_partitioned(const TpcLaunch &a, const TpcQPlan &pl, uint32_t *rmask, uint64_t lo, uint64_t hi, bool gated);
int tpc_launch_insert_part_split(const TpcLaunch &a, const TpcPartPlan &pl);
int tpc_launch_insert_part_apply_only(const TpcLaunch &a, const TpcPartPlan &pl, bool fresh);
struct TpcListSrc;
int tpc_launch_query_part_fused_lookup(const TpcLaunch &a, const TpcQPlan &pl, const TpcPartPlan &ipl, bool fresh, const uint64_t *iovf_sorted, const uint64_t *iovf_off,
                                       const TpcListSrc *lists = nullptr);
int tpc_launch_ovf_by_slice(const TpcLaunch &a, const uint64_t *list, uint64_t n, int slice_bits, uint32_t n_slices, uint32_t *cnt, uint32_t *cursor,
                            uint64_t *off, uint64_t *sorted, uint32_t rank = 0, uint32_t world = 1, int log_nb2 = 0);
#define TPC_FUSE_MAX_OVF (16ull << 20)
int tpc_launch_query_verify(const TpcLaunch &a, const TpcQPlan &pl, uint32_t *rmask);
extern int tpc_test_tight_pinch;
extern int tpc_test_mark_bucket_bits, tpc_test_mark_region_cap, tpc_test_mark_slice_bits;
extern int tpc_test_q6_pb2;
extern int tpc_test_insert_p3;
extern uint32_t tpc_test_sched_cap;
int tpc_launch_region_offsets(const TpcLaunch &a, const uint32_t *cnt, uint32_t n_regions, uint64_t *off);
int tpc_launch_region_pack(const TpcLaunch &a, const void *regions, uint64_t cap_entries, uint32_t entry_bytes, const uint32_t *cnt, const uint64_t *off,
                           uint32_t n_regions, void *packed);
int tpc_launch_query_part_hash(const TpcLaunch &a, const TpcQPlan &pl, uint32_t *rmask, uint64_t lo, uint64_t hi, bool gated);
int tpc_launch_query_part_lookup(const TpcLaunch &a, const TpcQPlan &pl);
int tpc_launch_query_part_split(const TpcLaunch &a, const TpcQPlan &pl);
int tpc_launch_surv_gather(const TpcLaunch &a, const TpcQPlan &pl, uint64_t *out);
int tpc_launch_verify_addrs(const TpcLaunch &a, const TpcQPlan &pl, int fn, int fn_count, const uint64_t *sid, uint64_t n, uint64_t *addr_out, int32_t *owner_out,
                            unsigned long long *owner_counts = nullptr);
#define TPC_V_OWNER_SHIFT 56
int tpc_launch_finish(hipStream_t s, const TpcQPlan &pl, const uint64_t *sid, uint64_t n, int fn_count, const uint8_t *hit, const uint32_t *perm, uint32_t *rmask,
                      unsigned long long *n_marked);
int tpc_launch_route64(hipStream_t s, const uint64_t *v, uint64_t n, int shift, uint32_t omask, uint64_t keep, unsigned long long *counts, unsigned long long *cursor,
                       uint32_t *perm, uint64_t *dst, int phase);
int tpc_launch_shard_probe(const TpcLaunch &a, const uint64_t *addr, uint64_t n, uint8_t *hit);
int tpc_launch_shard_mark(const TpcLaunch &a, const TpcQPlan &pl, const uint64_t *sid, uint64_t n, uint32_t *rmask);

int tpc_launch_survivor_sources(hipStream_t s, const uint64_t *sid, uint64_t n, uint32_t world, int32_t *src);
int tpc_launch_route(hipStream_t s, const int32_t *owner, uint64_t n, unsigned long long *counts, unsigned long long *cursor, uint32_t *perm, int phase);
int tpc_launch_permute64(hipStream_t s, const uint64_t *src, const uint32_t *perm, uint64_t n, uint64_t *dst);
int tpc_launch_select(hipStream_t s, const uint64_t *sid, uint64_t n, int fn_count, const uint8_t *hit, const uint32_t *perm, uint64_t *out, unsigned long long *n_out);

constexpr int TPC_LIST_WINDOW_BITS = 16;
constexpr int TPC_LIST_WINDOW_WORDS = 1 << (TPC_LIST_WINDOW_BITS - 5);

// ... 92 lines not shown
```

### twopaco_amd/csrc/tpc_qpartition.hip

```cpp
#ifndef TPC_QPARTITION_PART
#define TPC_QPARTITION_PART 0
#endif
#include "tpc_rbins.h"
#include "tpc_bins3.h"
#include "tpc_binsp.h"
#include "tpc_lean.h"
#include "tpc_internal.h"
#include "tpc_lists.h"
#include <algorithm>
#include <type_traits>
#include <cstdio>
#include <cstdlib>
#include <cmath>

#if TPC_QPARTITION_PART == 0
int tpc_test_q6_pb2 = 0;
int tpc_opt_qhash_pushes = 6, tpc_opt_qhash_roll = 1, tpc_opt_qhash_seed = 1;
int tpc_test_mark_bucket_bits = 0, tpc_test_mark_region_cap = 0, tpc_test_mark_slice_bits = 0;
#endif

namespace {

constexpr int QE_E_SHIFT = 31;
constexpr uint64_t QE_REM_MASK = (1ull << QE_E_SHIFT) - 1ull;
// ... 146 lines not shown
                                    eb[4 + c] = (uint32_t)(a0 >> shift);
                                    ev[4 + c] = (a0 & (((uint64_t)1 << shift) - 1)) | ((sid_g | (uint64_t)(4 + c)) << QE_E_SHIFT);
                                    eok[4 + c] = c != c_next;
                                }
                            }
                            bins.template push_batch<8>(eb, ev, eok, lost);
                        }
                    }
                    v.pos[0] = r1p ^ s_h[c_next] ^ s_hk[c_first];
                    v.neg[0] = tpc_rotr1(v.neg[0] ^ s_hk[tpc_rc(c_next)] ^ s_h[tpc_rc(c_first)], P.L);
                    ncnt += (c_next == TPC_CODE_N) - (c_first == TPC_CODE_N);
                    c_prev = c_first;
                    c_first = c_first_nx;
                }
            }
            bins.template flush<false>(lost);
        }
        rmask16[(wfirst * 2) + tid] = (uint16_t)word;
    }
    if constexpr (RB) { bins.flush(true, reg, lost); bins.store_counts(cnt1, reg, ridx); }
    else { bins.template flush<true>(lost); bins.store_counts(cnt1, ridx); }
}

constexpr int QT_MAXK = TPC_QSEED_MAXK;
constexpr uint32_t QH_ROLL_S = 1u;
constexpr uint32_t QH_SEED_S = 2u;

__device__ __forceinline__ uint32_t q_xor_and(uint32_t v, uint32_t row, uint32_t mask)
{
#if __has_builtin(__builtin_amdgcn_bitop3_b32)
    return __builtin_amdgcn_bitop3_b32(row, mask, v, 0x6Au);
#else
    return v ^ (row & mask);
#endif
}

__device__ __forceinline__ uint64_t q_spread2(uint32_t m)
{
    uint64_t x = m;
    x = (x | (x << 16)) & 0x0000FFFF0000FFFFull;
    x = (x | (x << 8)) & 0x00FF00FF00FF00FFull;
    x = (x | (x << 4)) & 0x0F0F0F0F0F0F0F0Full;
    x = (x | (x << 2)) & 0x3333333333333333ull;
    x = (x | (x << 1)) & 0x5555555555555555ull;
    return x | (x << 1);
}

template <bool GATED, bool SHARDED, bool HALF, bool LHI, bool PUSH6>
__global__ void __launch_bounds__(QH_THREADS)
k_q_hash2(int LOG_NB, TpcHashParams P, const uint64_t *__restrict__ tab, const uint64_t *__restrict__ bases,
          const uint32_t *__restrict__ nmask, uint64_t n_text, uint64_t tile0, uint64_t n_tiles, int pos_per_round,
          uint64_t lo, uint64_t hi, uint64_t *buf1, uint32_t *cnt1, uint64_t cap1, QOverflow ovf, PtPerm perm, PtShard sh,
          uint64_t gbase, uint32_t *__restrict__ rmask, uint32_t tiles_per_wg, const uint16_t *__restrict__ skip16, uint32_t mode,
          const uint4 *__restrict__ qseed)
{
    using V = LeanV<LHI>;
    extern __shared__ __attribute__((aligned(16))) unsigned char smem[];
    const int NB = 1 << LOG_NB;
    constexpr int TW = PT_THREADS + 1 + TPC_XW_MAX;
    Bins3<uint64_t, QH_THREADS> bins;
    uint64_t *s_b = reinterpret_cast<uint64_t *>(bins.carve(smem, LOG_NB));
    uint64_t *s_roll = s_b + TW;
    uint64_t *s_seed = s_roll + 20;
    uint32_t *s_n = reinterpret_cast<uint32_t *>(s_seed + QT_MAXK * 10);
    const uint32_t tid = threadIdx.x;
    const int k = P.k, L = P.L;
    if (tid < 5) {
        const uint32_t c = tid, rc = c == 4 ? 4u : 3u - c;
        s_roll[c * 2] = tab[c]; s_roll[c * 2 + 1] = tab[TPC_TAB_HK + rc];
        s_roll[10 + c * 2] = tab[TPC_TAB_HK + c]; s_roll[10 + c * 2 + 1] = tab[rc];
    }
    if (k <= QT_MAXK && !(mode & QH_SEED_S))
        for (uint32_t i = tid; i < 5u * (uint32_t)k; i += QH_THREADS) {
            const uint32_t t = i / 5u, c = i % 5u, rc = c == 4 ? 4u : 3u - c;
            s_seed[2 * i] = q_rotl_n(tab[c], L, (k - 1 - (int)t) % L);
            s_seed[2 * i + 1] = q_rotl_n(tab[rc], L, (int)t % L);
        }
    const int shift = L - LOG_NB;
    const uint32_t wg = blockIdx.x, nwg = gridDim.x;
    auto ridx = [sh, NB, wg, nwg](uint32_t b) { return SHARDED ? pt_r1_send(sh, (uint32_t)NB, nwg, wg, b) : (uint64_t)wg * NB + b; };
    auto lost = [shift, ovf](uint32_t b, uint64_t val) { ovf.push(((uint64_t)b << shift) | (val & QE_REM_MASK), val >> QE_E_SHIFT, 1); };
    bins.init(buf1, [cap1, ridx](uint32_t b) { return make_uint2((uint32_t)((ridx(b) * cap1) >> 4), (uint32_t)cap1); });
    LeanRotH<LHI> R;
    R.set(L);
    LeanSplit S;
    S.set(perm, LOG_NB);
    const int xw = (k + 1) / 32 + 2;
    uint16_t *rmask16 = reinterpret_cast<uint16_t *>(rmask);
    uint32_t h0l[5], h0h[5], hk0l[5], hk0h[5];
#pragma unroll
    for (int c = 0; c < 5; c++) {
        const uint64_t h = tab[c], hk = tab[TPC_TAB_HK + c];
        h0l[c] = (uint32_t)h; h0h[c] = (uint32_t)(h >> 32); hk0l[c] = (uint32_t)hk; hk0h[c] = (uint32_t)(hk >> 32);
    }
    auto hot = [](uint32_t chars, uint32_t nbits, uint32_t i, uint32_t (&m)[5]) {
        const uint32_t m0 = (uint32_t)__builtin_amdgcn_sbfe((int)chars, 2u * i, 1u), m1 = (uint32_t)__builtin_amdgcn_sbfe((int)chars, 2u * i + 1u, 1u);
        m[4] = (uint32_t)__builtin_amdgcn_sbfe((int)nbits, i, 1u);
        m[0] = ~(m0 | m1 | m[4]); m[1] = m0 & ~m1; m[2] = m1 & ~m0; m[3] = m0 & m1;
    };
    const uint32_t ppr_mask = (uint32_t)pos_per_round - 1u;
    constexpr bool half_rounds = HALF;
    const uint32_t p0 = 32u + tid * (uint32_t)QH_RUN;
    const uint64_t t_first = tile0 + (tiles_per_wg ? (uint64_t)blockIdx.x * tiles_per_wg : (uint64_t)blockIdx.x);
    const uint64_t t_end = tiles_per_wg ? min(tile0 + n_tiles, t_first + tiles_per_wg) : tile0 + n_tiles;
    const uint64_t t_step = tiles_per_wg ? 1u : gridDim.x;
    for (uint64_t tile = t_first; tile < t_end; tile += t_step) {
        const uint64_t wfirst = tile * PT_THREADS;
        __syncthreads();
        const uint32_t sk = skip16 ? (uint32_t)skip16[(wfirst * 2) + tid] : 0u;
        for (int i = (int)tid; i < PT_THREADS + 1 + xw; i += QH_THREADS) {
            const int64_t w = (int64_t)wfirst - 1 + i;
            uint64_t b = w >= 0 ? bases[w] : 0ull;
            const uint32_t m = w >= 0 ? nmask[w] : 0xFFFFFFFFu;
            if (m) b &= ~q_spread2(m);
            s_b[i] = b;
            s_n[i] = m;
        }
        __syncthreads();
        const uint32_t cw = lean_chars16(s_b, p0), nw = lean_nbits32(s_n, p0);
        const uint32_t cx = lean_chars16(s_b, p0 + (uint32_t)k), nx = lean_nbits32(s_n, p0 + (uint32_t)k);
        uint32_t cp = lean_char(s_b, s_n, p0 - 1u);
        int ncnt = 0;
        for (int t = 0; t < k; t += 32) {
            uint32_t bits = lean_nbits32(s_n, p0 + (uint32_t)t);
            if (k - t < 32) bits &= (1u << (k - t)) - 1u;
            ncnt += __popc(bits);
        }
        V pos = lv_make<LHI>(0u, 0u), neg = lv_make<LHI>(0u, 0u);
        if (mode & QH_SEED_S) {
            for (int t0 = 0; t0 < k; t0 += 16) {
                const uint32_t ch = lean_chars16(s_b, p0 + (uint32_t)t0), nb = lean_nbits32(s_n, p0 + (uint32_t)t0);
                const int m = min(16, k - t0);
                const uint4 *row = qseed + t0 * 5;
                for (int j = 0; j < m; j++) {
                    uint32_t mk[5];
                    hot(ch, nb, (uint32_t)j, mk);
                    const uint4 r0 = row[j * 5], r1 = row[j * 5 + 1], r2 = row[j * 5 + 2], r3 = row[j * 5 + 3], r4 = row[j * 5 + 4];
                    auto mix = [&mk](uint32_t v, uint32_t a, uint32_t c, uint32_t g, uint32_t t, uint32_t x) {
                        return q_xor_and(q_xor_and(q_xor_and(q_xor_and(q_xor_and(v, a, mk[0]), c, mk[1]), g, mk[2]), t, mk[3]), x, mk[4]);
                    };
                    pos.lo = mix(pos.lo, r0.x, r1.x, r2.x, r3.x, r4.x);
                    neg.lo = mix(neg.lo, r0.z, r1.z, r2.z, r3.z, r4.z);
                    if constexpr (LHI) {
                        pos.hi = mix(pos.hi, r0.y, r1.y, r2.y, r3.y, r4.y);
                        neg.hi = mix(neg.hi, r0.w, r1.w, r2.w, r3.w, r4.w);
                    }
                }
            }
        } else if (k <= QT_MAXK) {
            for (int t0 = 0; t0 < k; t0 += 16) {
                uint32_t ch = lean_chars16(s_b, p0 + (uint32_t)t0), nb = lean_nbits32(s_n, p0 + (uint32_t)t0);
                const int m = min(16, k - t0);
                const uint4 *row = reinterpret_cast<const uint4 *>(s_seed) + t0 * 5;
                for (int j = 0; j < m; j++) {
                    const uint32_t c = (ch & 3u) | ((nb & 1u) << 2);
                    ch >>= 2; nb >>= 1;
                    const uint4 e = row[j * 5 + c];
                    pos = lv_xor<LHI>(pos, e.x, e.y);
                    neg = lv_xor<LHI>(neg, e.z, e.w);
                }
            }
        } else {
// ... 50 lines not shown
                    }
                } else if constexpr (!half_rounds) bins.template push_batch<8>(eb, ev, eok, lost);
                else {
                    uint32_t b4[4];
                    uint64_t v4[4];
                    bool o4[4];
#pragma unroll
                    for (int c = 0; c < 4; c++) { b4[c] = eb[c]; v4[c] = ev[c]; o4[c] = eok[c]; }
                    bins.template push_batch<4>(b4, v4, o4, lost);
                }
                probing = true;
            }
            if constexpr (half_rounds) {
                bins.template flush<false>(lost);
                if (probing) {
                    if constexpr (PUSH6) {
                        const uint32_t b3[3] = {b6[3], b6[4], b6[5]};
                        const uint64_t v3[3] = {v6[3], v6[4], v6[5]};
                        bins.template push_batch<3>(b3, v3, all3, lost);
                    } else {
                        uint32_t b4[4];
                        uint64_t v4[4];
                        bool o4[4];
#pragma unroll
                        for (int c = 0; c < 4; c++) { b4[c] = eb[4 + c]; v4[c] = ev[4 + c]; o4[c] = eok[4 + c]; }
                        bins.template push_batch<4>(b4, v4, o4, lost);
                    }
                }
            }
            if (s + 1 < QH_RUN) {
                if ((PUSH6 || !SHARDED) && (mode & QH_ROLL_S)) {
                    uint32_t mnx[5], mfx[5];
                    hot(cx, nx, (uint32_t)s, mnx); hot(cw, nw, (uint32_t)s, mfx);
                    V p = r1p, q = neg;
#pragma unroll
                    for (int c = 0; c < 5; c++) {
                        const int r = c == 4 ? 4 : 3 - c;
                        p.lo = q_xor_and(q_xor_and(p.lo, h0l[c], mnx[c]), hk0l[c], mfx[c]);
                        q.lo = q_xor_and(q_xor_and(q.lo, hk0l[r], mnx[c]), h0l[r], mfx[c]);
                        if constexpr (LHI) {
                            p.hi = q_xor_and(q_xor_and(p.hi, h0h[c], mnx[c]), hk0h[c], mfx[c]);
                            q.hi = q_xor_and(q_xor_and(q.hi, hk0h[r], mnx[c]), h0h[r], mfx[c]);
                        }
                    }
                    pos = p; neg = R.rotr1(q);
                } else {
                    const uint4 en = reinterpret_cast<const uint4 *>(s_roll)[cn], ef = reinterpret_cast<const uint4 *>(s_roll)[5 + cf];
                    pos = lv_xor<LHI>(lv_xor<LHI>(r1p, en.x, en.y), ef.x, ef.y);
                    neg = R.rotr1(lv_xor<LHI>(lv_xor<LHI>(neg, en.z, en.w), ef.z, ef.w));
                }
                ncnt += (int)(cn >> 2) - (int)(cf >> 2);
                cp = cf;
            }
            if ((((uint32_t)s + 1u) & ppr_mask) == 0u) bins.template flush<false>(lost);
        }
        rmask16[(wfirst * 2) + tid] = (uint16_t)word;
    }
    bins.template flush<true>(lost);
    bins.store_counts(cnt1, ridx);
}

constexpr int QS_THREADS = 1024;
template <bool SHARDED, bool RB, bool P6 = false>
__global__ void __launch_bounds__(QS_THREADS)
k_q_split(int LOG_NB1, int LOG_NB2, int L, int slice_bits, int loads, uint32_t nwg1, uint32_t wpb, const uint64_t *__restrict__ buf1,
          const uint32_t *__restrict__ cnt1, uint64_t cap1, uint64_t *buf2, uint32_t *cnt2, const uint64_t *__restrict__ off2, QOverflow ovf,
          PtShard sh, uint32_t prev_wpb, int log_prev_nb2, uint32_t nreg_cap, uint32_t sched_cap, const uint64_t *__restrict__ off1,
          const uint64_t *__restrict__ own1, const uint32_t *__restrict__ owncnt1, uint32_t *__restrict__ bnd = nullptr, uint32_t n_groups = 0,
          uint32_t tiles_per_wg = 0, uint32_t batch_tiles = 0, uint32_t pb2 = 0)
{
    extern __shared__ __attribute__((aligned(16))) unsigned char smem[];
    const uint32_t NB1 = 1u << LOG_NB1, NB2 = 1u << LOG_NB2;
    constexpr int LOADS = P6 ? 5 : 4;
    constexpr uint64_t SENT = ~0ull;
    static_assert(!P6 || (!SHARDED && !RB), "the 6-byte output is the one-rank, flush-per-round form");
    typename std::conditional<P6, BinsP<PFmt6, QS_THREADS>,
                              typename std::conditional<RB, RBins<uint64_t, QS_THREADS>, Bins3<uint64_t, QS_THREADS>>::type>::type bins;
    uint64_t *s_off = reinterpret_cast<uint64_t *>(bins.carve(smem, LOG_NB2));
    if constexpr (RB) bins.init();
    else {
        const uint64_t *o2 = off2 + (uint64_t)blockIdx.x * NB2;
        if constexpr (P6) bins.init(buf2, [o2](uint32_t b) { const uint64_t o = o2[b]; return make_uint2((uint32_t)o, (uint32_t)(o2[b + 1] - o)); });
        else bins.init(buf2, [o2](uint32_t b) { const uint64_t o = o2[b]; return make_uint2((uint32_t)(o >> 4), (uint32_t)(o2[b + 1] - o)); });
    }
    for (uint32_t i = threadIdx.x; i <= NB2; i += QS_THREADS) s_off[i] = off2[(uint64_t)blockIdx.x * NB2 + i];
    const uint32_t bl = blockIdx.x / wpb, j = blockIdx.x % wpb;
    const uint32_t b1 = prev_wpb ? (sh.world > 1 ? ((((bl >> log_prev_nb2) * sh.world + sh.rank) << log_prev_nb2) | (bl & ((1u << log_prev_nb2) - 1u))) : bl)
                                 : (SHARDED ? bl * sh.world + sh.rank : bl);
    const uint32_t nvw = prev_wpb ? prev_wpb : SHARDED ? nwg1 * sh.world : nwg1;
    auto r1 = [=](uint32_t vw) {
        if (prev_wpb) return ((((uint64_t)(bl >> log_prev_nb2) * prev_wpb) + vw) << log_prev_nb2) + (bl & ((1u << log_prev_nb2) - 1u));
        return SHARDED ? pt_r1_recv(sh, NB1, nwg1, vw / nwg1, vw % nwg1, bl) : (uint64_t)vw * NB1 + bl;
    };
    auto mine = [=](uint32_t vw) { return SHARDED && own1 && !prev_wpb && vw / nwg1 == sh.rank; };
    const int shift1 = L - LOG_NB1;
    const uint64_t rem_mask = ((uint64_t)1 << shift1) - 1;
    auto reg = [buf2, s_off](uint32_t b) { const uint64_t o = s_off[b]; return PtRegion<uint64_t>{buf2 + o, s_off[b + 1] - o}; };
    const uint32_t S6 = (uint32_t)slice_bits, PB2 = pb2;
    uint32_t next_g = 1;
    uint32_t *my_bnd = P6 ? bnd + (uint64_t)blockIdx.x * NB2 * n_groups * 2u : nullptr;
    auto gmax = [=](uint32_t w) { return (uint32_t)((min((uint64_t)(w + 1u) * tiles_per_wg, (uint64_t)batch_tiles) * (uint64_t)(PT_THREADS * TPC_RUN) - 1ull) >> PB2); };
    struct Lost6 {
        QOverflow ovf; const uint32_t *next_g; uint32_t b1, S6, PB2; int shift1;
        __device__ __forceinline__ void pair(uint32_t b2, uint64_t val, uint64_t &addr, uint64_t &sid) const
        {
            const uint32_t z = *next_g - 1u;
            const uint64_t plow = (val >> (S6 + 3u)) & ((1ull << PB2) - 1ull);
            const uint64_t g = (z & 1u) == ((uint32_t)(val >> 47) & 1u) ? z : z - 1u;
            addr = ((uint64_t)b1 << shift1) | ((uint64_t)b2 << S6) | (val & ((1ull << S6) - 1ull));
            sid = ((val >> S6) & 7ull) | (((g << PB2) | plow) << 3);
        }
        __device__ __forceinline__ void operator()(uint32_t b2, uint64_t val) const { uint64_t a, i; pair(b2, val, a, i); ovf.push(a, i, 3); }
        __device__ __forceinline__ unsigned long long reserve(uint32_t n) const { return atomicAdd(ovf.cursor, (unsigned long long)n); }
        __device__ __forceinline__ void put(uint32_t b2, uint64_t val, unsigned long long at) const
        {
            uint64_t a, i;
            pair(b2, val, a, i);
            if (at < ovf.cap) { ovf.list[2 * at] = a; ovf.list[2 * at + 1] = i; } else ovf.cursor[1] = 1ull;
        }
    };
    const Lost6 lost_p6{ovf, &next_g, b1, S6, PB2, shift1};
    struct Lost8 {
        QOverflow ovf; uint32_t b1; int shift1; uint64_t rem_mask;
        __device__ __forceinline__ void operator()(uint32_t, uint64_t val) const { ovf.push(((uint64_t)b1 << shift1) | (val & rem_mask), val >> QE_E_SHIFT, 3); }
        __device__ __forceinline__ unsigned long long reserve(uint32_t n) const { return atomicAdd(ovf.cursor, (unsigned long long)n); }
        __device__ __forceinline__ void put(uint32_t, uint64_t val, unsigned long long at) const
        {
            if (at < ovf.cap) { ovf.list[2 * at] = ((uint64_t)b1 << shift1) | (val & rem_mask); ovf.list[2 * at + 1] = val >> QE_E_SHIFT; } else ovf.cursor[1] = 1ull;
        }
    };
    const Lost8 lost{ovf, b1, shift1, rem_mask};
    auto snapshot = [&](uint32_t lo, uint32_t hi) {
      if constexpr (P6) {
        const uint32_t ng = n_groups;
        uint32_t *mb0 = my_bnd;
        bins.template flush_with<true, false>(lost_p6,
            [lo, hi, ng, mb0](uint32_t b, uint32_t n) {
                const uint32_t padded = (n + (uint32_t)PFmt6::GROUP - 1u) / (uint32_t)PFmt6::GROUP * (uint32_t)PFmt6::GROUP;
                uint32_t *mb = mb0 + (uint64_t)b * 2u * ng, *mv = mb + ng;
                mv[lo - 1u] = n;
                for (uint32_t g = lo; g < hi; g++) { mb[g] = padded; mv[g] = padded; }
            });
        next_g = hi;
      }
    };
    __syncthreads();
    const uint32_t nreg = j < nvw ? (nvw - j + wpb - 1) / wpb : 0;
    const uint32_t step = (uint32_t)loads * QS_THREADS;
    uint32_t *s_scan = reinterpret_cast<uint32_t *>(s_off + NB2 + 1);
    uint32_t *s_cnt = s_scan + 32;
    uint32_t *s_sched = s_cnt + nreg_cap;
    struct Round { uint32_t t, base, n; };
    uint64_t va[LOADS], vb[LOADS], vc[LOADS];
    for (uint32_t skip = 0;; skip += sched_cap) {
// ... 840 lines not shown
        __syncthreads();
#pragma unroll
        for (int u = 0; u < RT_CHUNK / 256; u++) {
            const uint64_t i = c0 + (uint64_t)u * 256 + threadIdx.x;
            if (own[u] >= 0) {
                const uint64_t slot = base[own[u]] + rank[u];
                dst[slot] = val[u] & keep;
                if (perm) perm[i] = (uint32_t)slot;
            }
        }
        __syncthreads();
    }
}

__global__ void __launch_bounds__(256)
k_route_count64(const uint64_t *__restrict__ v, uint64_t n, int shift, uint32_t omask, unsigned long long *counts)
{
    __shared__ uint32_t h[RT_MAXW];
    if (threadIdx.x < RT_MAXW) h[threadIdx.x] = 0;
    __syncthreads();
    const uint64_t stride = (uint64_t)gridDim.x * blockDim.x;
    for (uint64_t i = (uint64_t)blockIdx.x * blockDim.x + threadIdx.x; i < n; i += stride) atomicAdd(&h[(uint32_t)(v[i] >> shift) & omask & (RT_MAXW - 1)], 1u);
    __syncthreads();
    if (threadIdx.x < RT_MAXW && h[threadIdx.x]) atomicAdd(&counts[threadIdx.x], (unsigned long long)h[threadIdx.x]);
}

#endif
#if TPC_QPARTITION_PART == 0
inline bool q_use_rbins(int log_nb) { return log_nb >= 9; }

void launch_qhash(const TpcLaunch &a, const TpcQPlan &pl, bool gated, uint64_t lo, uint64_t hi, uint32_t *rmask)
{
    QOverflow ovf{pl.ovf, pl.ovf_cur, pl.ovf_cap};
    const PtPerm perm{pl.slice_bits, pl.b1 + pl.b2 + pl.b3, pl.perm_mult, pl.perm_inv};
    const PtShard sh{pl.rank, pl.world};
    const bool rb = q_use_rbins(pl.b1);
    const bool lean = pl.b1 <= 9 && pl.sub_rounds <= 2 && perm.F <= 24 && !TpcEnv::get().no_lean && !(rb && TpcEnv::get().rb_hash);
    if (a.stat_kernel) { a.stat_kernel[1] = lean ? 1 : 2; a.stat_kernel[3] = 0; a.stat_kernel[4] = 0; }
    if (lean) {
        const size_t lds = Bins3<uint64_t, QH_THREADS>::lds_bytes(pl.b1) + (size_t)(PT_THREADS + 1 + TPC_XW_MAX) * 12 + 160 + (size_t)QT_MAXK * 80 + 64;
        const uint32_t mode = (tpc_qhash_roll_scalars() && (tpc_qhash_compact() || pl.world == 1) ? QH_ROLL_S : 0u) |
                              (tpc_qhash_seed_scalars() && a.qseed && a.P.k <= QT_MAXK ? QH_SEED_S : 0u);
        if (a.stat_kernel) {
            a.stat_kernel[3] = (tpc_qhash_compact() ? 1 : 0) | (mode & QH_ROLL_S ? 2 : 0) | (gated ? 4 : 0);
            a.stat_kernel[4] = mode & QH_SEED_S ? 1 : 0;
        }
#define TPC_QHASH2_GO(G, S, H, X, C)                                                                                                          \
    do {                                                                                                                                    \
        (void)hipFuncSetAttribute((const void *)k_q_hash2<G, S, H, X, C>, hipFuncAttributeMaxDynamicSharedMemorySize, (int)lds);               \
        hipLaunchKernelGGL((k_q_hash2<G, S, H, X, C>), dim3(pl.nwg1), dim3(QH_THREADS), lds, a.stream, pl.b1, a.P, a.tab, a.bases, a.nmask, a.n_text, \
                           pl.tile0, pl.n_tiles, pl.pos_per_round, lo, hi, pl.buf1, pl.cnt1, pl.cap1, ovf, perm, sh,                          \
                           pl.tile0_global * (uint64_t)(PT_THREADS * TPC_RUN), rmask, pl.fmt == 6 ? pl.tiles_per_wg : 0u,                  \
                           reinterpret_cast<const uint16_t *>(a.per_qs),            \
                           mode, reinterpret_cast<const uint4 *>(a.qseed));                                                                \
    } while (0)
#define TPC_QHASH2_GS(H, X, C)                                                                                                              \
    do {                                                                                                                                    \
        if (pl.world > 1) { if (gated) TPC_QHASH2_GO(true, true, H, X, C); else TPC_QHASH2_GO(false, true, H, X, C); }                      \
        else { if (gated) TPC_QHASH2_GO(true, false, H, X, C); else TPC_QHASH2_GO(false, false, H, X, C); }                                 \
    } while (0)
#define TPC_QHASH2_HX(C)                                                                                                                    \
    do {                                                                                                                                    \
        if (a.P.L > 32) { if (pl.b1 >= 9) TPC_QHASH2_GS(true, true, C); else TPC_QHASH2_GS(false, true, C); }                               \
        else { if (pl.b1 >= 9) TPC_QHASH2_GS(true, false, C); else TPC_QHASH2_GS(false, false, C); }                                        \
    } while (0)
        if (tpc_qhash_compact()) TPC_QHASH2_HX(true); else TPC_QHASH2_HX(false);
#undef TPC_QHASH2_HX
#undef TPC_QHASH2_GS
#undef TPC_QHASH2_GO
        return;
    }
    const size_t lds = (rb ? RBins<uint64_t, QH_THREADS>::lds_bytes(pl.b1) : Bins3<uint64_t, QH_THREADS>::lds_bytes(pl.b1)) +
                       (size_t)(PT_THREADS + 1 + TPC_XW_MAX) * 12 + (size_t)5 * 16 + 64;
#define TPC_QHASH_GO(G, S, R)                                                                                                               \
    do {                                                                                                                                    \
        (void)hipFuncSetAttribute((const void *)k_q_hash<G, S, R>, hipFuncAttributeMaxDynamicSharedMemorySize, (int)lds);                   \
        hipLaunchKernelGGL((k_q_hash<G, S, R>), dim3(pl.nwg1), dim3(QH_THREADS), lds, a.stream, pl.b1, a.P, a.tab, a.bases, a.nmask, a.n_text,  \
                           pl.tile0, pl.n_tiles, pl.pos_per_round, pl.sub_rounds, lo, hi, pl.buf1, pl.cnt1, pl.cap1, ovf, perm, sh,              \
                           pl.tile0_global * (uint64_t)(PT_THREADS * TPC_RUN), rmask);                                                      \
    } while (0)
#define TPC_QHASH_GS(R)                                                                                                                     \
    do {                                                                                                                                    \
        if (pl.world > 1) { if (gated) TPC_QHASH_GO(true, true, R); else TPC_QHASH_GO(false, true, R); }                                    \
        else { if (gated) TPC_QHASH_GO(true, false, R); else TPC_QHASH_GO(false, false, R); }                                               \
    } while (0)
    if (rb) TPC_QHASH_GS(true); else TPC_QHASH_GS(false);
#undef TPC_QHASH_GS
#undef TPC_QHASH_GO
}

constexpr int PER_MAXP = TPC_PER_MAXP;
constexpr int PER_PLANES = TPC_PER_PLANES;
constexpr int PER_CBITS = 10;
__device__ __forceinline__ bool periodic_may_flag(const uint64_t *__restrict__ bases, const uint32_t *__restrict__ nmask, int k, int64_t first, int64_t lo, int64_t hi)
{
    const int B = min(16, (k + 2) / 2);
    if (B < 10) return true;
    int64_t s0 = first, s1 = first + 31 + k;
    if (k >= 31 + 2 * B - 1) { s0 = first + 31; s1 = first + k; }
    const uint32_t M = B == 16 ? 0xFFFFFFFFu : (1u << (2 * B)) - 1u;
    for (int64_t a = s0; a + B - 1 <= s1; a += B) {
        if (a - 63 < lo || a + B > hi) return true;
        const int64_t wl = (a - 63) >> 5;
        const uint32_t off = (uint32_t)((a - 63) & 31), sh = 2u * off;
        const bool four = off + 63u + (uint32_t)B > 96u;
        const uint64_t b0 = bases[wl], b1 = bases[wl + 1], b2 = bases[wl + 2], b3 = four ? bases[wl + 3] : 0ull;
        const uint64_t nlo = (uint64_t)nmask[wl] | ((uint64_t)nmask[wl + 1] << 32), nhi = (uint64_t)nmask[wl + 2] | ((uint64_t)(four ? nmask[wl + 3] : 0u) << 32);
// ... 103 lines not shown
#pragma unroll
                for (int q = 0; q < PER_PLANES; q++) dpl[q] = qd[cw + (uint64_t)q * stride];
            }
            const uint32_t bi = (uint32_t)i & 31u;
            uint32_t m;
            if ((sw >> bi) & 1u) {
                zeros = 0;
                uint32_t d = 0;
#pragma unroll
                for (int q = 0; q < PER_PLANES; q++) d |= ((dpl[q] >> bi) & 1u) << q;
                m = (uint32_t)(mh >> (d - 1u)) & 1u;
                add |= m << bi;
            } else {
                if (++zeros == PER_MAXP) break;
                m = (rw >> bi) & 1u;
            }
            mh = ((mh << 1) | (uint64_t)m) & ((1ull << PER_MAXP) - 1ull);
        }
        if (add) atomicOr(&rmask[cw], add);
    }
}

void launch_qsplit(const TpcLaunch &a, bool sharded, int log_nb1, int log_nb2, int low_bits, int loads, uint32_t nwg1, uint32_t wpb, uint32_t nvw,
                   const uint64_t *buf1, const uint32_t *cnt1, uint64_t cap1, uint64_t *buf2, uint32_t *cnt2, const uint64_t *off2, QOverflow ovf, PtShard sh,
                   uint32_t prev_wpb, int log_prev_nb2, const uint64_t *off1, unsigned grid, const uint64_t *own1 = nullptr, const uint32_t *owncnt1 = nullptr)
{
    const bool rb = q_use_rbins(log_nb2);
    const size_t lds_base = (rb ? RBins<uint64_t, QS_THREADS>::lds_bytes(log_nb2) : Bins3<uint64_t, QS_THREADS>::lds_bytes(log_nb2)) + ((size_t)8 << log_nb2) + 64 + 128;
    if (rb) loads = 4;
    uint32_t nreg_cap, sched_cap;
    size_t lds;
    pt_schedule_dims(nvw, wpb, cap1, (uint32_t)loads * QS_THREADS, lds_base, nreg_cap, sched_cap, lds);
#define TPC_QSPLIT_GO(S, R)                                                                                                                  \
    do {                                                                                                                                    \
        (void)hipFuncSetAttribute((const void *)k_q_split<S, R>, hipFuncAttributeMaxDynamicSharedMemorySize, (int)lds);                      \
        hipLaunchKernelGGL((k_q_split<S, R>), dim3(grid), dim3(QS_THREADS), lds, a.stream, log_nb1, log_nb2, a.P.L, low_bits, loads, nwg1, wpb, buf1, cnt1, cap1,   \
                           buf2, cnt2, off2, ovf, sh, prev_wpb, log_prev_nb2, nreg_cap, sched_cap, off1, own1, owncnt1);                     \
    } while (0)
    if (sharded) { if (rb) TPC_QSPLIT_GO(true, true); else TPC_QSPLIT_GO(true, false); }
    else { if (rb) TPC_QSPLIT_GO(false, true); else TPC_QSPLIT_GO(false, false); }
#undef TPC_QSPLIT_GO
}

void launch_qsplit6(const TpcLaunch &a, const TpcQPlan &pl, QOverflow ovf)
{
    const PtShard sh{0, 1};
    const size_t lds_base = BinsP<PFmt6, QS_THREADS>::lds_bytes(pl.b2) + ((size_t)8 << pl.b2) + 64 + 128;
    uint32_t nreg_cap, sched_cap;
    size_t lds;
    pt_schedule_dims(pl.nwg1, pl.wpb, pl.cap1, (uint32_t)pl.loads * QS_THREADS, lds_base, nreg_cap, sched_cap, lds);
    (void)hipFuncSetAttribute((const void *)k_q_split<false, false, true>, hipFuncAttributeMaxDynamicSharedMemorySize, (int)lds);
    hipLaunchKernelGGL((k_q_split<false, false, true>), dim3((1u << pl.b1) * pl.wpb), dim3(QS_THREADS), lds, a.stream, pl.b1, pl.b2, a.P.L, pl.slice_bits, pl.loads, pl.nwg1, pl.wpb,
                       pl.rbuf1, pl.rcnt1, pl.cap1, pl.buf2, pl.cnt2, pl.off2, ovf, sh, 0u, 0, nreg_cap, sched_cap, pl.roff1, (const uint64_t *)nullptr, (const uint32_t *)nullptr,
                       pl.bnd, pl.n_groups, pl.tiles_per_wg, (uint32_t)pl.n_tiles, pl.pb2);
}

constexpr int MK_LOADS = 4;
__global__ void __launch_bounds__(1024)
k_mark_split(const uint32_t *__restrict__ pass, const unsigned long long *__restrict__ surv_cur, uint64_t surv_cap, int MB, int LOG_NB, uint32_t nb, uint32_t *mark_buf,
             uint32_t *mark_cnt, uint32_t cap, uint64_t gbase, uint32_t *rmask, unsigned long long *n_lost)
{
    extern __shared__ __attribute__((aligned(16))) unsigned char smem[];
    Bins3<uint32_t, 1024> bins;
    (void)bins.carve(smem, LOG_NB);
    const uint32_t wg = blockIdx.x, per = gridDim.x / QS_LISTS;
    bins.init(mark_buf, [=](uint32_t b) { return b < nb ? make_uint2((uint32_t)((((uint64_t)wg * nb + b) * cap) >> 5), cap) : make_uint2(0u, 0u); });
    auto lost = [=](uint32_t b, uint32_t val) {
        const uint64_t g = gbase + ((uint64_t)b << MB) + val;
        atomicOr(&rmask[g >> 5], 1u << ((uint32_t)g & 31u));
        atomicAdd(n_lost, 1ull);
    };
    __syncthreads();
    const uint32_t list = wg / per, part = wg % per;
    const uint64_t n = min((uint64_t)surv_cur[list], surv_cap);
    const uint64_t chunk = ((n + per - 1) / per + 3) & ~3ull;
    const uint64_t begin = min(n, (uint64_t)part * chunk), end = min(n, begin + chunk);
    const uint32_t *src = pass + (uint64_t)list * surv_cap;
    const uint32_t low = (1u << MB) - 1u;
    constexpr uint64_t STEP = (uint64_t)MK_LOADS * 1024;
    if (begin < end) {
        uint32_t va[MK_LOADS], vb[MK_LOADS];
        auto load = [&](uint32_t (&d)[MK_LOADS], uint64_t base) {
#pragma unroll
            for (int i = 0; i < MK_LOADS; i++) d[i] = src[min(base + (uint64_t)i * 1024 + threadIdx.x, end - 1)];
        };
        auto round = [&](const uint32_t (&cur)[MK_LOADS], uint64_t base) {
            uint32_t bb[MK_LOADS], val[MK_LOADS];
            bool ok[MK_LOADS];
#pragma unroll
            for (int i = 0; i < MK_LOADS; i++) {
                ok[i] = base + (uint64_t)i * 1024 + threadIdx.x < end && cur[i] != 0xFFFFFFFFu;
                bb[i] = ok[i] ? cur[i] >> MB : 0u;
                val[i] = cur[i] & low;
            }
            bins.template push_batch<MK_LOADS>(bb, val, ok, lost);
            bins.template flush<false>(lost);
        };
        load(va, begin);
        for (uint64_t base = begin;; base += 2 * STEP) {
            if (base + STEP < end) load(vb, base + STEP);
            round(va, base);
            if (base + STEP >= end) break;
            if (base + 2 * STEP < end) load(va, base + 2 * STEP);
            round(vb, base + STEP);
            if (base + 2 * STEP >= end) break;
        }
    }
// ... 601 lines not shown
```

Before: 13.16 billion.

## Skip k-mers inside far repeated blocks and rebalance query tiles by live work

Adds a far-repeat detector that samples k-mers to find 1024-position blocks that copy an earlier region, builds query and insert skip masks for those positions, and later copies the query results from the source block level by level. Query hashing then skips those positions. Workgroups receive tile ranges weighted by live positions, and flushes happen less often on sparse tiles. This is meant to cut redundant hashing on repetitive genomes, at the cost of a detection pass, host syncs and more complex scheduling.

```diff
diff --git a/include/twopaco_hip.h b/include/twopaco_hip.h
--- a/include/twopaco_hip.h
+++ b/include/twopaco_hip.h
@@ -120,6 +120,8 @@
 
 int tpc_shard_periodic_copy(tpc_ctx *ctx);
 int tpc_periodic_download(tpc_ctx *ctx, uint32_t *qs_host, uint32_t *planes_host, uint32_t *ins_host);
+int tpc_far_download(tpc_ctx *ctx, uint64_t *d_host, uint32_t *level_host, uint32_t *qs_host, uint32_t *ins_host);
+int tpc_far_copy(tpc_ctx *ctx);
 
 #define TPC_SHARD_INSERT 0
 #define TPC_SHARD_QUERY 1
diff --git a/twopaco_amd/capi.py b/twopaco_amd/capi.py
--- a/twopaco_amd/capi.py
+++ b/twopaco_amd/capi.py
@@ -24,6 +24,7 @@
                "tpc_emit_stream", "tpc_emit_stream_fetch", "tpc_host_alloc", "tpc_host_free", "tpc_get_stat", "tpc_filter_upload",
                "tpc_junction_keys_export", "tpc_junction_keys_import", "tpc_warmup", "tpc_preload", "tpc_reserve", "tpc_shard_chunk", "tpc_emit_stream_partial", "tpc_emit_stream_part",
                "tpc_shard_plan_both", "tpc_shard_hash_begin", "tpc_shard_hash_end", "tpc_shard_apply_inplace", "tpc_shard_survivors_home", "tpc_shard_verify_send", "tpc_shard_finish", "tpc_shard_verify_local", "tpc_shard_periodic_copy", "tpc_periodic_download",
+               "tpc_far_download", "tpc_far_copy",
                "tpc_pass1_query_begin", "tpc_combine_info", "tpc_combine_export", "tpc_combine_merge", "tpc_combine_import", "tpc_combine_choose", "tpc_filter_copy_out", "tpc_filter_copy_in",
                "tpc_segments_build_host", "tpc_segments_build_resident", "tpc_segments_counts", "tpc_segments_error", "tpc_segments_fetch_names", "tpc_segments_fetch_first",
                "tpc_segments_fetch_events", "tpc_segments_fetch_sequences", "tpc_segments_text_plan", "tpc_segments_text_fetch", "tpc_segments_text_write", "tpc_distinct_sketch",
@@ -135,6 +136,8 @@
         L.tpc_shard_verify_local.argtypes = [p]
         L.tpc_shard_periodic_copy.argtypes = [p]
         L.tpc_periodic_download.argtypes = [p, p, p, p]
+        L.tpc_far_download.argtypes = [p, p, p, p, p]
+        L.tpc_far_copy.argtypes = [p]
         L.tpc_pass1_query_begin.argtypes = [p, u64, u64]
         L.tpc_combine_info.argtypes = [p, u32, p]
         L.tpc_combine_export.argtypes = [p, u32, p, u64, p, p]
@@ -1104,6 +1107,20 @@
         for b in range(6):
             dist |= bits(planes[b]) << b
         return bits(qs).astype(bool), dist, bits(ins).astype(bool)
+
+    def far_download(self):
+        nw, nb = hip().tpc_mask_words(self._h), self.stat("far_table_blocks")
+        d, lev = np.zeros(nb, dtype=np.uint64), np.zeros(nb, dtype=np.uint32)
+        qs, ins = np.zeros(nw, dtype=np.uint32), np.zeros(nw, dtype=np.uint32)
+        self._ck(hip().tpc_far_download(self._h, d.ctypes.data, lev.ctypes.data, qs.ctypes.data, ins.ctypes.data))
+
+        def bits(w):
+            return np.unpackbits(w.astype("<u4").view(np.uint8), bitorder="little").astype(bool)
+
+        return d, lev, bits(qs), bits(ins)
+
+    def far_copy(self):
+        self._ck(hip().tpc_far_copy(self._h))
 
     def shard_verify_local(self):
         self._ck(hip().tpc_shard_verify_local(self._h))
diff --git a/twopaco_amd/csrc/tpc_capi.hip b/twopaco_amd/csrc/tpc_capi.hip
--- a/twopaco_amd/csrc/tpc_capi.hip
+++ b/twopaco_amd/csrc/tpc_capi.hip
@@ -28,14 +28,158 @@
     return a;
 }
 
-TpcLaunch make_launch_periodic(const tpc_ctx *c)
+TpcLaunch make_launch_periodic(const tpc_ctx *c, bool with_far)
 {
     TpcLaunch a = make_launch(c);
     if (c->periodic && c->periodic_valid) {
         if (c->periodic_any_q) a.per_qs = c->periodic;
         if (c->periodic_any_i) a.per_i = c->periodic + (size_t)(1 + TPC_PER_PLANES) * c->n_words_alloc;
     }
+    if (with_far && c->far_valid && c->far_on) {
+        const size_t s = c->n_words_alloc;
+        if (c->far_any_q) a.per_qs = c->far_masks + (a.per_qs ? 2 * s : 0);
+        if (c->far_any_i) a.per_i = c->far_masks + (a.per_i ? 3 * s : s);
+    }
     return a;
+}
+
+void far_drop(tpc_ctx *c)
+{
+    for (void *p : { (void *)c->far_masks, (void *)c->far_D, (void *)c->far_lists, (void *)c->far_tile_live, (void *)c->far_tb }) if (p) (void)hipFree(p);
+    c->far_masks = nullptr; c->far_D = nullptr; c->far_lists = nullptr; c->far_tile_live = nullptr; c->far_tb = nullptr;
+    c->far_tile_live_host.clear(); c->far_tb_keys.clear(); c->far_stat_balanced = 0;
+    c->far_D_host.clear(); c->far_level_host.clear(); c->far_list_off.clear();
+    c->far_valid = c->far_on = c->far_any_q = c->far_any_i = false;
+    c->far_levels = 0; c->far_stat_q = c->far_stat_i = c->far_stat_blocks = 0;
+}
+
+void ensure_far(tpc_ctx *c)
+{
+    if (c->far_valid || !c->bases || !c->have_params || c->n_words_alloc == 0) return;
+    if (c->opt_periodic && !c->periodic_valid) return;
+    static const char *const env = getenv("TPC_FAR_SKIP");
+    const int mode = env && env[0] ? (env[0] == 'a' || atoi(env) < 0 ? -1 : atoi(env) != 0) : c->opt_far;
+    far_drop(c);
+    c->far_valid = true;
+    if (mode == 0 || (mode < 0 && (int64_t)c->n_text < c->opt_far_min)) return;
+    if (c->sh_configured || c->sh_world > 1 || c->text_windowed || replicated(c) || c->opt_shard_periodic) return;
+    const auto t_begin = std::chrono::steady_clock::now();
+    const uint64_t nw = c->n_words, nb = (nw + TPC_FAR_BLOCK / 32 - 1) / (TPC_FAR_BLOCK / 32);
+    if (nb < 3 || nb > 0x7FFFFFFFull) return;
+    int sample_bits = 6;
+    while ((c->n_text >> sample_bits) > (1ull << 25)) sample_bits++;
+    uint64_t slots = 1024;
+    while (slots < (c->n_text >> sample_bits) * 4) slots <<= 1;
+    unsigned long long *tab = nullptr;
+    auto off = [c, &tab]() {
+        if (tab) (void)hipFree(tab);
+        (void)hipGetLastError();
+        far_drop(c);
+        c->far_valid = true;
+        if (c->dbg_timing) fprintf(stderr, "[timing]   far repeats: off for this text (nothing found, or an allocation or launch failed)\n");
+    };
+    if (hipMalloc((void **)&tab, 2 * slots * sizeof(unsigned long long)) != hipSuccess || hipMalloc((void **)&c->far_D, nb * sizeof(uint64_t)) != hipSuccess) return off();
+    if (tpc_launch_far_detect(c->stream, c->bases, c->nmask, nw, c->P.k, sample_bits, tab, tab + slots, slots, c->far_D, nb)) return off();
+    c->far_D_host.assign(nb, 0);
+    if (hipMemcpyAsync(c->far_D_host.data(), c->far_D, nb * sizeof(uint64_t), hipMemcpyDeviceToHost, c->stream) != hipSuccess || hipStreamSynchronize(c->stream) != hipSuccess) return off();
+    (void)hipFree(tab); tab = nullptr;
+    c->far_level_host.assign(nb, 0);
+    int levels = 0;
+    bool changed = false;
+    uint64_t flagged = 0;
+    for (uint64_t b = 0; b < nb; b++) {
+        const uint64_t D = c->far_D_host[b];
+        if (!D) continue;
+        const uint64_t s = b * TPC_FAR_BLOCK - D;
+        const uint32_t l = 1 + std::max(c->far_level_host[s / TPC_FAR_BLOCK], c->far_level_host[(s + TPC_FAR_BLOCK - 1) / TPC_FAR_BLOCK]);
+        if (l > (uint32_t)TPC_FAR_MAX_LEVEL) { c->far_D_host[b] = 0; changed = true; continue; }
+        c->far_level_host[b] = l;
+        levels = std::max(levels, (int)l);
+        flagged++;
+    }
+    if (!flagged) return off();
+    if (changed && hipMemcpy(c->far_D, c->far_D_host.data(), nb * sizeof(uint64_t), hipMemcpyHostToDevice) != hipSuccess) return off();
+    std::vector<uint32_t> lists;
+    lists.reserve(flagged);
+    c->far_list_off.assign(1, 0);
+    for (int l = 1; l <= levels; l++) {
+        for (uint64_t b = 0; b < nb; b++) if (c->far_level_host[b] == (uint32_t)l) lists.push_back((uint32_t)b);
+        c->far_list_off.push_back((uint32_t)lists.size());
+    }
+    const bool pq = c->periodic && c->periodic_valid && c->periodic_any_q, pi = c->periodic && c->periodic_valid && c->periodic_any_i;
+    const size_t s = c->n_words_alloc;
+    if (hipMalloc((void **)&c->far_lists, lists.size() * sizeof(uint32_t)) != hipSuccess || hipMalloc((void **)&c->far_masks, (pq || pi ? 4 : 2) * s * sizeof(uint32_t)) != hipSuccess) return off();
+    unsigned long long *cnt = c->counters + 6, counts[2] = {0, 0};
+    if (hipMemcpy(c->far_lists, lists.data(), lists.size() * sizeof(uint32_t), hipMemcpyHostToDevice) != hipSuccess ||
+        hipMemsetAsync(c->far_masks, 0, (pq || pi ? 4 : 2) * s * sizeof(uint32_t), c->stream) != hipSuccess || hipMemsetAsync(cnt, 0, sizeof counts, c->stream) != hipSuccess) return off();
+    if (tpc_launch_far_build(c->stream, c->bases, c->nmask, nw, c->P.k, c->far_D, pq ? c->periodic : nullptr, pi ? c->periodic + (size_t)(1 + TPC_PER_PLANES) * s : nullptr, c->far_masks,
+                             c->far_masks + s, c->far_masks + (pq ? 2 * s : 0), c->far_masks + (pi ? 3 * s : s), cnt)) return off();
+    if (hipMemcpyAsync(counts, cnt, sizeof counts, hipMemcpyDeviceToHost, c->stream) != hipSuccess || hipStreamSynchronize(c->stream) != hipSuccess) return off();
+    c->far_any_q = counts[0] != 0; c->far_any_i = counts[1] != 0;
+    if (!c->far_any_q && !c->far_any_i) return off();
+    c->far_on = true;
+    c->far_levels = levels;
+    c->far_stat_q = (int64_t)counts[0]; c->far_stat_i = (int64_t)counts[1]; c->far_stat_blocks = (int64_t)flagged;
+    if (c->far_any_q) {
+        const uint64_t nt = c->n_words_alloc / 512 + 1;
+        const TpcLaunch a = make_launch_periodic(c);
+        c->far_tile_live_host.assign(nt, 0);
+        if (hipMalloc((void **)&c->far_tile_live, nt * sizeof(uint32_t)) != hipSuccess || tpc_launch_far_tile_live(c->stream, a.per_qs, c->nmask, nw, c->far_tile_live, nt) ||
+            hipMemcpyAsync(c->far_tile_live_host.data(), c->far_tile_live, nt * sizeof(uint32_t), hipMemcpyDeviceToHost, c->stream) != hipSuccess || hipStreamSynchronize(c->stream) != hipSuccess) {
+            (void)hipGetLastError();
+            if (c->far_tile_live) (void)hipFree(c->far_tile_live);
+            c->far_tile_live = nullptr; c->far_tile_live_host.clear();
+        }
+    }
+    if (c->dbg_timing)
+        fprintf(stderr, "[timing]   far repeats (detector, levels, masks): %.1f ms; %lld of %llu blocks in %d levels, %lld query and %lld insert positions skipped\n",
+                std::chrono::duration<double, std::milli>(std::chrono::steady_clock::now() - t_begin).count(), (long long)flagged, (unsigned long long)nb, levels, (long long)counts[0],
+                (long long)counts[1]);
+}
+
+static int far_tile_weight() { static const int v = [] { const char *e = getenv("TPC_FAR_TILE_WEIGHT"); return e && e[0] ? atoi(e) : 50; }(); return v; }
+static bool far_cadence() { static const bool v = [] { const char *e = getenv("TPC_FAR_CADENCE"); return !(e && e[0] == '0'); }(); return v; }
+
+const uint32_t *far_balance(tpc_ctx *c, const TpcQPlan &pl)
+{
+    const int pct = far_tile_weight();
+    if (!(c->far_valid && c->far_on) || !c->far_tile_live || pl.fmt != 6 || !pl.tiles_per_wg || pct < 0 || pl.n_tiles == 0 || pl.nwg1 == 0 || pl.nwg1 > (uint32_t)tpc_ctx::FAR_TB_WGS) return nullptr;
+    const uint64_t n = pl.n_tiles, t0 = pl.tile0, nwg = pl.nwg1, max_t = (1ull << pl.pb2) / (512ull * TPC_RUN);
+    if (t0 + n > c->far_tile_live_host.size() || max_t == 0 || nwg * max_t < n) return nullptr;
+    const size_t row = tpc_ctx::FAR_TB_WGS + 1;
+    for (size_t i = 0; i + 2 < c->far_tb_keys.size(); i += 3)
+        if (c->far_tb_keys[i] == t0 && c->far_tb_keys[i + 1] == n && c->far_tb_keys[i + 2] == nwg) return c->far_tb + (i / 3) * row;
+    const size_t slot = c->far_tb_keys.size() / 3;
+    if (slot >= (size_t)tpc_ctx::FAR_TB_KEYS) return nullptr;
+    if (!c->far_tb && hipMalloc((void **)&c->far_tb, tpc_ctx::FAR_TB_KEYS * row * sizeof(uint32_t)) != hipSuccess) { (void)hipGetLastError(); c->far_tb = nullptr; return nullptr; }
+    const uint64_t C = 512ull * TPC_RUN * (uint64_t)pct / 100;
+    std::vector<uint64_t> pre(n + 1, 0);
+    for (uint64_t t = 0; t < n; t++) pre[t + 1] = pre[t] + c->far_tile_live_host[t0 + t] + C;
+    std::vector<uint32_t> b(nwg + 1, 0);
+    uint64_t t = 0;
+    for (uint64_t w = 1; w < nwg; w++) {
+        const uint64_t want = pre[n] / nwg * w + pre[n] % nwg * w / nwg;
+        while (t < n && pre[t] < want) t++;
+        b[w] = (uint32_t)t;
+    }
+    b[nwg] = (uint32_t)n;
+    for (uint64_t w = 0; w < nwg; w++) b[w + 1] = (uint32_t)std::min<uint64_t>(b[w + 1], b[w] + max_t);
+    b[nwg] = (uint32_t)n;
+    for (uint64_t w = nwg; w > 0; w--) b[w - 1] = (uint32_t)std::max<uint64_t>(b[w - 1], b[w] > max_t ? b[w] - max_t : 0);
+    bool ok = b[0] == 0 && b[nwg] == n;
+    for (uint64_t w = 0; w < nwg && ok; w++) ok = b[w] <= b[w + 1] && b[w + 1] - b[w] <= max_t;
+    if (!ok) return nullptr;
+    if (hipMemcpy(c->far_tb + slot * row, b.data(), (nwg + 1) * sizeof(uint32_t), hipMemcpyHostToDevice) != hipSuccess) { (void)hipGetLastError(); return nullptr; }
+    c->far_tb_keys.push_back(t0); c->far_tb_keys.push_back(n); c->far_tb_keys.push_back(nwg);
+    return c->far_tb + slot * row;
+}
+
+int far_copy_levels(tpc_ctx *c)
+{
+    if (!(c->far_valid && c->far_on && c->far_any_q)) return 0;
+    for (int l = 1; l <= c->far_levels; l++)
+        if (tpc_launch_far_copy(c->stream, c->rmask, c->far_masks, c->far_D, c->far_lists + c->far_list_off[l - 1], c->far_list_off[l] - c->far_list_off[l - 1])) return -1;
+    return 0;
 }
 
 void ensure_periodic(tpc_ctx *c)
@@ -309,6 +453,7 @@
     for (void *p : c->pbuf) if (p) (void)hipFree(p);
     for (void *p : c->ikeep) if (p) (void)hipFree(p);
     if (c->periodic) (void)hipFree(c->periodic);
+    far_drop(c);
     if (c->cmb_base) (void)hipFree(c->cmb_base);
     if (c->cmb_cur) (void)hipFree(c->cmb_cur);
     if (c->ikeep_ovf) (void)hipFree(c->ikeep_ovf);
@@ -343,13 +488,15 @@
     if (!strcmp(name, "fuse_apply_lookup")) { c->opt_fuse = value != 0; return 0; }
     if (!strcmp(name, "test_q6_pb2")) { tpc_test_q6_pb2 = (int)value; return 0; }
     if (!strcmp(name, "insert_entry_fmt")) { tpc_test_insert_p3 = value == 3; return 0; }
-    if (!strcmp(name, "shard_periodic_skip")) { c->opt_shard_periodic = value != 0; return 0; }
-    if (!strcmp(name, "periodic_skip")) { c->opt_periodic = value != 0; if (!value) c->periodic_valid = false; return 0; }
+    if (!strcmp(name, "shard_periodic_skip")) { c->opt_shard_periodic = value != 0; c->far_valid = false; return 0; }
+    if (!strcmp(name, "periodic_skip")) { c->opt_periodic = value != 0; if (!value) c->periodic_valid = false; c->far_valid = false; return 0; }
+    if (!strcmp(name, "far_skip")) { c->opt_far = value < 0 ? -1 : value != 0; c->far_valid = false; c->qb_valid = false; return 0; }
+    if (!strcmp(name, "far_min_positions")) { c->opt_far_min = value < 0 ? 0 : value; c->far_valid = false; c->qb_valid = false; return 0; }
     if (!strcmp(name, "test_tight_pinch")) { tpc_test_tight_pinch = (int)value; c->sh_have[0] = c->sh_have[1] = false; return 0; }
     if (!strcmp(name, "test_sched_cap")) { tpc_test_sched_cap = value > 0 ? (uint32_t)value : 0; return 0; }
     if (!strcmp(name, "test_mask_scan")) { tpc_test_mask_scan = value == 1 || value == 2 ? (int)value : 0; return 0; }
     if (!strcmp(name, "text_window")) { c->opt_text_window = value != 0; return 0; }
-    if (!strcmp(name, "replicate_filter")) { c->opt_replicate = value != 0; return 0; }
+    if (!strcmp(name, "replicate_filter")) { c->opt_replicate = value != 0; c->far_valid = false; return 0; }
     if (!strcmp(name, "test_force_anyq")) { tpc_test_force_anyq = value != 0; return 0; }
     if (!strcmp(name, "test_sketch_grid")) { tpc_test_sketch_grid = value > 0 ? (int)value : 0; return 0; }
     if (!strcmp(name, "test_links_slots_log2")) { c->opt_links_slots_log2 = (int)std::max<int64_t>(-1, std::min<int64_t>(value, 64)); return 0; }
@@ -418,6 +565,15 @@
     if (!strcmp(name, "query_overflow_entries")) return c->stat_query_overflow;
     if (!strcmp(name, "insert_overflow_entries")) return c->stat_insert_overflow;
     if (!strcmp(name, "periodic_skip")) return c->periodic_valid ? 1 : 0;
+    if (!strcmp(name, "far_skip")) return c->far_valid && c->far_on ? 1 : 0;
+    if (!strcmp(name, "far_positions_query")) return c->far_on ? c->far_stat_q : 0;
+    if (!strcmp(name, "far_positions_insert")) return c->far_on ? c->far_stat_i : 0;
+    if (!strcmp(name, "far_levels")) return c->far_on ? c->far_levels : 0;
+    if (!strcmp(name, "far_balance")) return c->far_on ? c->far_stat_balanced : 0;
+    if (!strcmp(name, "far_blocks")) return c->far_on ? c->far_stat_blocks : 0;
+    if (!strcmp(name, "far_table_blocks")) return (int64_t)((c->n_words + TPC_FAR_BLOCK / 32 - 1) / (TPC_FAR_BLOCK / 32));
+    if (!strcmp(name, "far_block_positions")) return TPC_FAR_BLOCK;
+    if (!strcmp(name, "far_max_level")) return TPC_FAR_MAX_LEVEL;
     if (!strcmp(name, "pbuf_releases")) return c->stat_pbuf_releases;
     if (!strcmp(name, "distances_tile")) return TPC_DISTANCES_TILE;
     if (!strcmp(name, "text_words")) return (int64_t)(c->text_w1 - c->text_w0);
@@ -480,7 +636,7 @@
         c->filter_words = fw;
     }
     c->have_params = true;
-    c->periodic_valid = false;
+    c->periodic_valid = false; c->far_valid = false;
     c->pending_apply = false;
     c->qb_valid = false;
     c->n_keys = 0; c->finalized = false; c->rounds_done = 0; c->mask_dirty = false; c->marks_valid = false; c->rmask_sums_valid = false;
@@ -510,6 +666,7 @@
     for (void *p : { (void *)c->bases_alloc, (void *)c->nmask_alloc, (void *)c->rmask, (void *)c->mask, (void *)c->block_sums, (void *)c->periodic })
         if (p) (void)hipFree(p);
     c->periodic = nullptr; c->periodic_valid = false;
+    far_drop(c);
     c->bases = nullptr; c->nmask = nullptr; c->bases_alloc = nullptr; c->nmask_alloc = nullptr; c->rmask = nullptr; c->mask = nullptr; c->block_sums = nullptr;
     const uint64_t wn = w1 - w0;
     HIPCHK(c, dev_malloc(c, (void **)&c->bases_alloc, wn * sizeof(uint64_t)));
@@ -573,6 +730,7 @@
     { int rc0 = flush_pending_apply(c); if (rc0) return rc0; }
     c->qb_valid = false;
     ensure_periodic(c);
+    ensure_far(c);
     if (n_kmers) HIPCHK(c, hipMemsetAsync(c->counters, 0, sizeof(unsigned long long), c->stream));
     uint64_t t_begin, t_end;
     pass_tiles(c, t_begin, t_end);
@@ -827,6 +985,7 @@
     c->stat_q_begun = begun ? 1 : 0;
     c->marks_valid = false; c->rmask_sums_valid = false;
     ensure_periodic(c);
+    ensure_far(c);
     TpcQPlan pl;
     uint64_t t_begin, t_end;
     pass_tiles(c, t_begin, t_end);
@@ -871,6 +1030,9 @@
                 pl.tile0 = t0;
                 pl.tile0_global = t0;
                 pl.n_tiles = t0 < t_end ? std::min<uint64_t>(per, t_end - t0) : 0;
+                pl.tile_begin = far_balance(c, pl);
+                pl.tile_live = c->far_valid && c->far_on && far_cadence() ? c->far_tile_live : nullptr;
+                c->far_stat_balanced = pl.tile_begin ? 1 : 0;
                 const bool presplit = begun && t0 == t_begin;
                 if (!presplit) {
                     HIPCHK(c, hipMemsetAsync(pl.ovf_cur, 0, 32 * sizeof(unsigned long long), c->stream));
@@ -928,6 +1090,7 @@
                 }
             }
             if (c->periodic_valid && c->periodic_any_q && c->periodic) tpc_launch_periodic_copy(c->stream, c->rmask, c->periodic, c->periodic + c->n_words_alloc, c->n_words_alloc, c->n_words);
+            if (far_copy_levels(c)) return fail(c, -1, "far copy launch failed");
             tpc_launch_mask_count(c->stream, c->rmask, c->n_words, c->block_sums, c->counters + 1);
         }
         HIPCHK(c, hipGetLastError());
@@ -1083,6 +1246,41 @@
     return 0;
 }
 
+int tpc_far_download(tpc_ctx *c, uint64_t *d_host, uint32_t *level_host, uint32_t *qs_host, uint32_t *ins_host)
+{
+    if (!c || !c->have_params || !c->bases || !d_host || !level_host || !qs_host || !ins_host) return fail(c, -1, "set_params and seq_upload first");
+    HIPCHK(c, hipSetDevice(c->device));
+    ensure_periodic(c);
+    ensure_far(c);
+    const size_t nw = c->n_words, nb = (nw + TPC_FAR_BLOCK / 32 - 1) / (TPC_FAR_BLOCK / 32);
+    memset(d_host, 0, nb * sizeof(uint64_t));
+    memset(level_host, 0, nb * sizeof(uint32_t));
+    memset(qs_host, 0, nw * sizeof(uint32_t));
+    memset(ins_host, 0, nw * sizeof(uint32_t));
+    if (!(c->far_valid && c->far_on)) return 0;
+    memcpy(d_host, c->far_D_host.data(), nb * sizeof(uint64_t));
+    memcpy(level_host, c->far_level_host.data(), nb * sizeof(uint32_t));
+    HIPCHK(c, hipStreamSynchronize(c->stream));
+    HIPCHK(c, hipMemcpy(qs_host, c->far_masks, nw * sizeof(uint32_t), hipMemcpyDeviceToHost));
+    HIPCHK(c, hipMemcpy(ins_host, c->far_masks + c->n_words_alloc, nw * sizeof(uint32_t), hipMemcpyDeviceToHost));
+    return 0;
+}
+
+int tpc_far_copy(tpc_ctx *c)
+{
+    if (!c || !c->rmask || !c->have_params) return fail(c, -1, "no text");
+    HIPCHK(c, hipSetDevice(c->device));
+    ensure_periodic(c);
+    ensure_far(c);
+    if (c->far_valid && c->far_on && c->far_any_q) {
+        if (far_copy_levels(c)) return fail(c, -1, "far copy launch failed");
+        HIPCHK(c, hipGetLastError());
+        HIPCHK(c, hipStreamSynchronize(c->stream));
+        c->marks_valid = false; c->rmask_sums_valid = false;
+    }
+    return 0;
+}
+
 int tpc_hash_dump(tpc_ctx *c, uint64_t g0, uint64_t n, uint64_t *out_host)
 {
     if (!c || !c->have_params || !c->bases) return -1;
diff --git a/twopaco_amd/csrc/tpc_capi_shard.hip b/twopaco_amd/csrc/tpc_capi_shard.hip
--- a/twopaco_amd/csrc/tpc_capi_shard.hip
+++ b/twopaco_amd/csrc/tpc_capi_shard.hip
@@ -6,6 +6,7 @@
     if (world == 0 || (world & (world - 1)) || rank >= world) return fail(c, -1, "world must be a power of two and rank < world");
     HIPCHK(c, hipSetDevice(c->device));
     c->sh_rank = rank; c->sh_world = world;
+    c->sh_configured = true; c->far_valid = false;
     c->sh_have[0] = c->sh_have[1] = false;
     c->pending_apply = false;
     if (c->have_params) {
@@ -138,7 +139,7 @@
     const uint64_t n = t0 < c1 ? std::min<uint64_t>(per, c1 - t0) : 0;
     unsigned long long *ov = c->sh_ov_host[pass];
     ov[0] = ov[1] = 0;
-    TpcLaunch a = c->opt_shard_periodic ? make_launch_periodic(c) : make_launch(c);
+    TpcLaunch a = c->opt_shard_periodic ? make_launch_periodic(c, false) : make_launch(c);
     a.stream = st;
     if (pass == TPC_SHARD_INSERT) {
         TpcPartPlan pl = c->sh_ipl;
diff --git a/twopaco_amd/csrc/tpc_ctx.h b/twopaco_amd/csrc/tpc_ctx.h
--- a/twopaco_amd/csrc/tpc_ctx.h
+++ b/twopaco_amd/csrc/tpc_ctx.h
@@ -33,6 +33,22 @@
     bool periodic_any_q = false, periodic_any_i = false;
     int opt_periodic = 1;
     bool opt_shard_periodic = false;
+    uint32_t *far_masks = nullptr;
+    uint64_t *far_D = nullptr;
+    uint32_t *far_lists = nullptr;
+    std::vector<uint64_t> far_D_host;
+    std::vector<uint32_t> far_level_host, far_list_off;
+    bool far_valid = false, far_on = false;
+    bool far_any_q = false, far_any_i = false;
+    int far_levels = 0;
+    int64_t far_stat_q = 0, far_stat_i = 0, far_stat_blocks = 0;
+    static constexpr int FAR_TB_KEYS = 64, FAR_TB_WGS = 1024;
+    uint32_t *far_tile_live = nullptr, *far_tb = nullptr;
+    std::vector<uint32_t> far_tile_live_host;
+    std::vector<uint64_t> far_tb_keys;
+    int far_stat_balanced = 0;
+    int opt_far = -1;
+    int64_t opt_far_min = 1 << 25;
     uint64_t *bases_alloc = nullptr;
     uint32_t *nmask_alloc = nullptr;
     int opt_text_window = 0;
@@ -252,6 +268,7 @@
     int64_t stat_insert_overflow = 0;
     int64_t stat_pbuf_releases = 0;
     uint32_t sh_rank = 0, sh_world = 1;
+    bool sh_configured = false;
     TpcPartPlan sh_ipl;
     TpcQPlan sh_qpl;
     bool sh_have[2] = {false, false};
@@ -284,8 +301,12 @@
 
 int fail(tpc_ctx *c, int code, const char *fmt, ...);
 TpcLaunch make_launch(const tpc_ctx *c);
-TpcLaunch make_launch_periodic(const tpc_ctx *c);
+TpcLaunch make_launch_periodic(const tpc_ctx *c, bool with_far = true);
 void ensure_periodic(tpc_ctx *c);
+void ensure_far(tpc_ctx *c);
+void far_drop(tpc_ctx *c);
+int far_copy_levels(tpc_ctx *c);
+const uint32_t *far_balance(tpc_ctx *c, const TpcQPlan &pl);
 uint64_t rotln_host(uint64_t x, int L, int r);
 hipError_t dev_malloc(tpc_ctx *c, void **p, size_t bytes);
 int read_counter(tpc_ctx *c, int i, uint64_t *out);
diff --git a/twopaco_amd/csrc/tpc_farskip.hip b/twopaco_amd/csrc/tpc_farskip.hip
--- /dev/null
+++ b/twopaco_amd/csrc/tpc_farskip.hip
@@ -0,0 +1,245 @@
+#include "tpc_internal.h"
+
+namespace {
+
+constexpr int FAR_B = TPC_FAR_BLOCK, FAR_BW = TPC_FAR_BLOCK / 32;
+constexpr unsigned long long FAR_EMPTY = ~0ull;
+constexpr int FAR_PROBES = 64;
+
+__device__ __forceinline__ uint64_t far_mix(uint64_t x)
+{
+    x ^= x >> 30; x *= 0xBF58476D1CE4E5B9ull;
+    x ^= x >> 27; x *= 0x94D049BB133111EBull;
+    return x ^ (x >> 31);
+}
+
+__device__ __forceinline__ void far_chars32(const uint64_t *__restrict__ bases, const uint32_t *__restrict__ nmask, int64_t n_words, int64_t s, uint64_t &ch, uint32_t &nn)
+{
+    const int64_t w = s >> 5;
+    const uint32_t off = (uint32_t)(s & 31);
+    const bool in0 = w >= 0 && w < n_words, in1 = w + 1 >= 0 && w + 1 < n_words;
+    const uint64_t b0 = in0 ? bases[w] : 0ull;
+    const uint32_t n0 = in0 ? nmask[w] : 0xFFFFFFFFu;
+    if (off == 0u) { ch = b0; nn = n0; return; }
+    const uint64_t b1 = in1 ? bases[w + 1] : 0ull;
+    const uint32_t n1 = in1 ? nmask[w + 1] : 0xFFFFFFFFu;
+    ch = (b0 >> (2u * off)) | (b1 << (64u - 2u * off));
+    nn = (n0 >> off) | (n1 << (32u - off));
+}
+
+__device__ __forceinline__ uint32_t far_even_bits(uint64_t x)
+{
+    x &= 0x5555555555555555ull;
+    x = (x | (x >> 1)) & 0x3333333333333333ull;
+    x = (x | (x >> 2)) & 0x0F0F0F0F0F0F0F0Full;
+    x = (x | (x >> 4)) & 0x00FF00FF00FF00FFull;
+    x = (x | (x >> 8)) & 0x0000FFFF0000FFFFull;
+    x = (x | (x >> 16)) & 0x00000000FFFFFFFFull;
+    return (uint32_t)x;
+}
+
+__device__ __forceinline__ uint32_t far_eq32(const uint64_t *__restrict__ bases, const uint32_t *__restrict__ nmask, int64_t n_words, int64_t a, uint64_t D)
+{
+    uint64_t c0, c1;
+    uint32_t n0, n1;
+    far_chars32(bases, nmask, n_words, a, c0, n0);
+    if (n0 == 0xFFFFFFFFu) return 0u;
+    far_chars32(bases, nmask, n_words, a - (int64_t)D, c1, n1);
+    const uint64_t x = c0 ^ c1;
+    return far_even_bits(~(x | (x >> 1))) & ~n0 & ~n1;
+}
+
+__global__ void __launch_bounds__(256) k_far_sample(const uint64_t *__restrict__ bases, const uint32_t *__restrict__ nmask, uint64_t n_words, int m, uint32_t smask, unsigned long long *keys,
+                                                    unsigned long long *pos, uint64_t tmask)
+{
+    const uint64_t w = (uint64_t)blockIdx.x * 256 + threadIdx.x;
+    if (w >= n_words) return;
+    const uint64_t b0 = bases[w], b1 = w + 1 < n_words ? bases[w + 1] : 0ull;
+    const uint64_t nb = (uint64_t)nmask[w] | ((uint64_t)(w + 1 < n_words ? nmask[w + 1] : 0xFFFFFFFFu) << 32);
+    const uint64_t vm = m == 32 ? ~0ull : (1ull << (2 * m)) - 1ull, nm = m == 32 ? 0xFFFFFFFFull : (1ull << m) - 1ull;
+    for (uint32_t j = 0; j < 32u; j++) {
+        if ((nb >> j) & nm) continue;
+        const uint64_t v = (j ? (b0 >> (2u * j)) | (b1 << (64u - 2u * j)) : b0) & vm;
+        const uint64_t h = far_mix(v);
+        if (((uint32_t)h & smask) != 0u || v == FAR_EMPTY) continue;
+        uint64_t slot = (h >> 32) & tmask;
+        for (int t = 0; t < FAR_PROBES; t++, slot = (slot + 1) & tmask) {
+            const unsigned long long old = atomicCAS(&keys[slot], FAR_EMPTY, (unsigned long long)v);
+            if (old == FAR_EMPTY || old == v) { atomicMin(&pos[slot], (unsigned long long)((w << 5) + j)); break; }
+        }
+    }
+}
+
+__global__ void __launch_bounds__(64) k_far_propose(const uint64_t *__restrict__ bases, const uint32_t *__restrict__ nmask, uint64_t n_words, int m, uint32_t smask,
+                                                    const unsigned long long *__restrict__ keys, const unsigned long long *__restrict__ pos, uint64_t tmask, uint64_t *__restrict__ D_out)
+{
+    __shared__ uint64_t s_c[64][2];
+    __shared__ uint64_t s_cand[TPC_FAR_CANDS];
+    __shared__ uint32_t s_score[TPC_FAR_CANDS];
+    __shared__ int s_n;
+    const uint64_t b = blockIdx.x;
+    const uint32_t lane = threadIdx.x;
+    const uint64_t bstart = b * (uint64_t)FAR_B;
+    const int64_t w = (int64_t)(b * FAR_BW) + (lane < 32u ? (int64_t)lane : (int64_t)lane - 32 - FAR_BW);
+    uint64_t c0 = 0, c1 = 0;
+    if (w >= 0 && (uint64_t)w < n_words) {
+        const uint64_t b0 = bases[w], b1 = (uint64_t)w + 1 < n_words ? bases[w + 1] : 0ull;
+        const uint64_t nb = (uint64_t)nmask[w] | ((uint64_t)((uint64_t)w + 1 < n_words ? nmask[w + 1] : 0xFFFFFFFFu) << 32);
+        const uint64_t vm = m == 32 ? ~0ull : (1ull << (2 * m)) - 1ull, nm = m == 32 ? 0xFFFFFFFFull : (1ull << m) - 1ull;
+        for (uint32_t j = 0; j < 32u && c1 == 0; j++) {
+            if ((nb >> j) & nm) continue;
+            const uint64_t v = (j ? (b0 >> (2u * j)) | (b1 << (64u - 2u * j)) : b0) & vm;
+            const uint64_t h = far_mix(v);
+            if (((uint32_t)h & smask) != 0u || v == FAR_EMPTY) continue;
+            uint64_t slot = (h >> 32) & tmask;
+            for (int t = 0; t < FAR_PROBES; t++, slot = (slot + 1) & tmask) {
+                const unsigned long long key = keys[slot];
+                if (key == FAR_EMPTY) break;
+                if (key != v) continue;
+                const uint64_t i = ((uint64_t)w << 5) + j, e = pos[slot];
+                if (e < i && i - e >= 2ull * FAR_B && i - e <= bstart) {
+                    const uint64_t d = i - e;
+                    if (c0 == 0) c0 = d; else if (d != c0) c1 = d;
+                }
+                break;
+            }
+        }
+    }
+    s_c[lane][0] = c0; s_c[lane][1] = c1;
+    if (lane < TPC_FAR_CANDS) { s_cand[lane] = 0; s_score[lane] = 0; }
+    __syncthreads();
+    if (lane == 0) {
+        int n = 0;
+        for (int l = 0; l < 64 && n < TPC_FAR_CANDS; l++)
+            for (int q = 0; q < 2 && n < TPC_FAR_CANDS; q++) {
+                const uint64_t d = s_c[l][q];
+                bool seen = d == 0;
+                for (int t = 0; t < n; t++) seen = seen || s_cand[t] == d;
+                if (!seen) s_cand[n++] = d;
+            }
+        s_n = n;
+    }
+    __syncthreads();
+    const int n = s_n;
+    if (lane < 32u)
+        for (int t = 0; t < n; t++) {
+            const uint32_t E = far_eq32(bases, nmask, (int64_t)n_words, (int64_t)(bstart + 32u * lane), s_cand[t]);
+            const uint32_t sc = ((E & 0xFFFFu) == 0xFFFFu ? 16u : 0u) + ((E >> 16) == 0xFFFFu ? 16u : 0u);
+            if (sc) atomicAdd(&s_score[t], sc);
+        }
+    __syncthreads();
+    if (lane == 0) {
+        uint64_t best = 0;
+        uint32_t best_score = 0;
+        for (int t = 0; t < n; t++) if (s_score[t] > best_score) { best_score = s_score[t]; best = s_cand[t]; }
+        D_out[b] = best;
+    }
+}
+
+__global__ void __launch_bounds__(256) k_far_build(const uint64_t *__restrict__ bases, const uint32_t *__restrict__ nmask, uint64_t n_words, int k, const uint64_t *__restrict__ Dtab,
+                                                   const uint32_t *__restrict__ per_qs, const uint32_t *__restrict__ per_i, uint32_t *__restrict__ far_qs, uint32_t *__restrict__ far_i,
+                                                   uint32_t *__restrict__ comb_qs, uint32_t *__restrict__ comb_i, unsigned long long *counts)
+{
+    __shared__ uint32_t s_cnt[2];
+    if (threadIdx.x < 2) s_cnt[threadIdx.x] = 0;
+    __syncthreads();
+    const uint64_t w = (uint64_t)blockIdx.x * 256 + threadIdx.x;
+    if (w < n_words) {
+        const uint64_t D = Dtab[w / FAR_BW];
+        uint32_t oqs = 0, oin = 0;
+        if (D) {
+            const int64_t first = (int64_t)(w << 5);
+            int run = (int)(far_eq32(bases, nmask, (int64_t)n_words, first - 32, D) >> 31);
+            for (int64_t a = first; a <= first + 31 + k; a += 32) {
+                const uint32_t E = far_eq32(bases, nmask, (int64_t)n_words, a, D);
+                if (E == 0u) { run = 0; continue; }
+                for (int t = 0; t < 32; t++) {
+                    run = ((E >> t) & 1u) ? run + 1 : 0;
+                    const int64_t i = a + t - k;
+                    if (i < first || i > first + 31) continue;
+                    if (run >= k + 2) oqs |= 1u << (uint32_t)(i - first);
+                    if (run >= k + 1) oin |= 1u << (uint32_t)(i - first);
+                }
+            }
+        }
+        uint32_t pq = 0, pi = 0;
+        if (per_qs) {
+            pq = per_qs[w];
+            uint64_t lo = (uint64_t)pq | ((uint64_t)(w + 1 < n_words ? per_qs[w + 1] : 0u) << 32), hi = w + 2 < n_words ? per_qs[w + 2] : 0u;
+            auto shr = [&lo, &hi](uint32_t s) { const uint64_t l = (lo >> s) | (hi << (64u - s)), h = hi >> s; lo |= l; hi |= h; };
+            lo = (lo >> 1) | (hi << 63); hi >>= 1;
+            shr(1); shr(2); shr(4); shr(8); shr(16); shr(31);
+            oqs &= ~(pq | (uint32_t)lo);
+        }
+        if (per_i) { pi = per_i[w]; oin &= ~pi; }
+        far_qs[w] = oqs; far_i[w] = oin;
+        if (comb_qs != far_qs) comb_qs[w] = oqs | pq;
+        if (comb_i != far_i) comb_i[w] = oin | pi;
+        if (oqs) atomicAdd(&s_cnt[0], (uint32_t)__popc(oqs));
+        if (oin) atomicAdd(&s_cnt[1], (uint32_t)__popc(oin));
+    }
+    __syncthreads();
+    if (threadIdx.x < 2 && s_cnt[threadIdx.x]) atomicAdd(&counts[threadIdx.x], (unsigned long long)s_cnt[threadIdx.x]);
+}
+
+__global__ void __launch_bounds__(256) k_far_copy(uint32_t *__restrict__ rmask, const uint32_t *__restrict__ far_qs, const uint64_t *__restrict__ Dtab,
+                                                  const uint32_t *__restrict__ blocks, uint32_t n_blocks)
+{
+    const uint32_t idx = blockIdx.x * 256u + threadIdx.x, bi = idx / FAR_BW;
+    if (bi >= n_blocks) return;
+    const uint64_t b = blocks[bi], w = b * FAR_BW + (idx % FAR_BW);
+    const uint32_t F = far_qs[w];
+    if (F == 0u) return;
+    const uint64_t s = (w << 5) - Dtab[b];
+    const uint32_t off = (uint32_t)(s & 31);
+    uint32_t v = rmask[s >> 5] >> off;
+    if (off) v |= rmask[(s >> 5) + 1] << (32u - off);
+    rmask[w] = (rmask[w] & ~F) | (v & F);
+}
+
+__global__ void __launch_bounds__(256) k_far_tile_live(const uint32_t *__restrict__ skip_qs, const uint32_t *__restrict__ nmask, uint64_t n_words, uint32_t *__restrict__ tile_live)
+{
+    __shared__ uint32_t s_n;
+    if (threadIdx.x == 0) s_n = 0;
+    __syncthreads();
+    uint32_t n = 0;
+    for (uint32_t i = threadIdx.x; i < 512u; i += 256u) {
+        const uint64_t w = (uint64_t)blockIdx.x * 512u + i;
+        if (w < n_words) n += (uint32_t)__popc(~(skip_qs[w] | nmask[w]));
+    }
+    if (n) atomicAdd(&s_n, n);
+    __syncthreads();
+    if (threadIdx.x == 0) tile_live[blockIdx.x] = s_n;
+}
+
+}
+
+int tpc_launch_far_tile_live(hipStream_t stream, const uint32_t *skip_qs, const uint32_t *nmask, uint64_t n_words, uint32_t *tile_live, uint64_t n_tiles)
+{
+    if (n_tiles) hipLaunchKernelGGL(k_far_tile_live, dim3((unsigned)n_tiles), dim3(256), 0, stream, skip_qs, nmask, n_words, tile_live);
+    return hipGetLastError() == hipSuccess ? 0 : -1;
+}
+
+int tpc_launch_far_detect(hipStream_t stream, const uint64_t *bases, const uint32_t *nmask, uint64_t n_words, int k, int sample_bits, unsigned long long *keys, unsigned long long *pos,
+                          uint64_t slots, uint64_t *D, uint64_t n_blocks)
+{
+    const int m = k < 32 ? k : 32;
+    const uint32_t smask = (1u << sample_bits) - 1u;
+    if (hipMemsetAsync(keys, 0xFF, slots * sizeof(unsigned long long), stream) != hipSuccess || hipMemsetAsync(pos, 0xFF, slots * sizeof(unsigned long long), stream) != hipSuccess) return -1;
+    hipLaunchKernelGGL(k_far_sample, dim3((unsigned)((n_words + 255) / 256)), dim3(256), 0, stream, bases, nmask, n_words, m, smask, keys, pos, slots - 1);
+    hipLaunchKernelGGL(k_far_propose, dim3((unsigned)n_blocks), dim3(64), 0, stream, bases, nmask, n_words, m, smask, keys, pos, slots - 1, D);
+    return hipGetLastError() == hipSuccess ? 0 : -1;
+}
+
+int tpc_launch_far_build(hipStream_t stream, const uint64_t *bases, const uint32_t *nmask, uint64_t n_words, int k, const uint64_t *D, const uint32_t *per_qs, const uint32_t *per_i,
+                         uint32_t *far_qs, uint32_t *far_i, uint32_t *comb_qs, uint32_t *comb_i, unsigned long long *counts)
+{
+    hipLaunchKernelGGL(k_far_build, dim3((unsigned)((n_words + 255) / 256)), dim3(256), 0, stream, bases, nmask, n_words, k, D, per_qs, per_i, far_qs, far_i, comb_qs, comb_i, counts);
+    return hipGetLastError() == hipSuccess ? 0 : -1;
+}
+
+int tpc_launch_far_copy(hipStream_t stream, uint32_t *rmask, const uint32_t *far_qs, const uint64_t *D, const uint32_t *blocks, uint32_t n_blocks)
+{
+    if (n_blocks) hipLaunchKernelGGL(k_far_copy, dim3((n_blocks * (uint32_t)FAR_BW + 255u) / 256u), dim3(256), 0, stream, rmask, far_qs, D, blocks, n_blocks);
+    return hipGetLastError() == hipSuccess ? 0 : -1;
+}
diff --git a/twopaco_amd/csrc/tpc_internal.h b/twopaco_amd/csrc/tpc_internal.h
--- a/twopaco_amd/csrc/tpc_internal.h
+++ b/twopaco_amd/csrc/tpc_internal.h
@@ -82,6 +82,15 @@
 int tpc_launch_periodic_build(const TpcLaunch &a, uint32_t *qs, uint32_t *qd, uint64_t stride, uint32_t *ins, uint64_t w_begin, uint64_t w_end, uint64_t pos_lo, uint64_t pos_hi,
                               uint32_t *any);
 int tpc_launch_periodic_copy(hipStream_t stream, uint32_t *rmask, const uint32_t *qs, const uint32_t *qd, uint64_t stride, uint64_t n_words);
+constexpr int TPC_FAR_BLOCK = 1024;
+constexpr int TPC_FAR_MAX_LEVEL = 8;
+constexpr int TPC_FAR_CANDS = 8;
+int tpc_launch_far_detect(hipStream_t stream, const uint64_t *bases, const uint32_t *nmask, uint64_t n_words, int k, int sample_bits, unsigned long long *keys, unsigned long long *pos,
+                          uint64_t slots, uint64_t *D, uint64_t n_blocks);
+int tpc_launch_far_build(hipStream_t stream, const uint64_t *bases, const uint32_t *nmask, uint64_t n_words, int k, const uint64_t *D, const uint32_t *per_qs, const uint32_t *per_i,
+                         uint32_t *far_qs, uint32_t *far_i, uint32_t *comb_qs, uint32_t *comb_i, unsigned long long *counts);
+int tpc_launch_far_copy(hipStream_t stream, uint32_t *rmask, const uint32_t *far_qs, const uint64_t *D, const uint32_t *blocks, uint32_t n_blocks);
+int tpc_launch_far_tile_live(hipStream_t stream, const uint32_t *skip_qs, const uint32_t *nmask, uint64_t n_words, uint32_t *tile_live, uint64_t n_tiles);
 
 int tpc_launch_insert(const TpcLaunch &a, uint64_t lo, uint64_t hi, bool gated, bool test, unsigned long long *n_kmers);
 int tpc_launch_query(const TpcLaunch &a, uint32_t *rmask, uint64_t lo, uint64_t hi, bool gated, unsigned long long *n_marks);
@@ -163,6 +172,7 @@
     int fmt = 0;
     bool presplit = false;
     uint32_t tiles_per_wg = 0, n_groups = 0, pb2 = 0;
+    const uint32_t *tile_begin = nullptr, *tile_live = nullptr;
     uint32_t *bnd = nullptr;
     uint32_t *pass = nullptr;
     uint32_t *mark_buf = nullptr;
diff --git a/twopaco_amd/csrc/tpc_qpartition.hip b/twopaco_amd/csrc/tpc_qpartition.hip
--- a/twopaco_amd/csrc/tpc_qpartition.hip
+++ b/twopaco_amd/csrc/tpc_qpartition.hip
@@ -222,7 +222,7 @@
           const uint32_t *__restrict__ nmask, uint64_t n_text, uint64_t tile0, uint64_t n_tiles, int pos_per_round,
           uint64_t lo, uint64_t hi, uint64_t *buf1, uint32_t *cnt1, uint64_t cap1, QOverflow ovf, PtPerm perm, PtShard sh,
           uint64_t gbase, uint32_t *__restrict__ rmask, uint32_t tiles_per_wg, const uint16_t *__restrict__ skip16, uint32_t mode,
-          const uint4 *__restrict__ qseed)
+          const uint4 *__restrict__ qseed, const uint32_t *__restrict__ tile_begin, const uint32_t *__restrict__ tile_live)
 {
     using V = LeanV<LHI>;
     extern __shared__ __attribute__((aligned(16))) unsigned char smem[];
@@ -271,13 +271,19 @@
     const uint32_t ppr_mask = (uint32_t)pos_per_round - 1u;
     constexpr bool half_rounds = HALF;
     const uint32_t p0 = 32u + tid * (uint32_t)QH_RUN;
-    const uint64_t t_first = tile0 + (tiles_per_wg ? (uint64_t)blockIdx.x * tiles_per_wg : (uint64_t)blockIdx.x);
-    const uint64_t t_end = tiles_per_wg ? min(tile0 + n_tiles, t_first + tiles_per_wg) : tile0 + n_tiles;
+    const bool ranges = tiles_per_wg && tile_begin;
+    const uint64_t t_first = tile0 + (ranges ? (uint64_t)tile_begin[blockIdx.x] : tiles_per_wg ? (uint64_t)blockIdx.x * tiles_per_wg : (uint64_t)blockIdx.x);
+    const uint64_t t_end = ranges ? min(tile0 + n_tiles, tile0 + (uint64_t)tile_begin[blockIdx.x + 1u]) : tiles_per_wg ? min(tile0 + n_tiles, t_first + tiles_per_wg) : tile0 + n_tiles;
     const uint64_t t_step = tiles_per_wg ? 1u : gridDim.x;
     for (uint64_t tile = t_first; tile < t_end; tile += t_step) {
         const uint64_t wfirst = tile * PT_THREADS;
         __syncthreads();
         const uint32_t sk = skip16 ? (uint32_t)skip16[(wfirst * 2) + tid] : 0u;
+        uint32_t fmask = ppr_mask;
+        if (tile_live) {
+            const uint32_t live = tile_live[tile];
+            for (uint32_t full = (uint32_t)(PT_THREADS * TPC_RUN) / 2u; live < full && fmask < (uint32_t)QH_RUN - 1u; full >>= 1) fmask = (fmask << 1) | 1u;
+        }
         for (int i = (int)tid; i < PT_THREADS + 1 + xw; i += QH_THREADS) {
             const int64_t w = (int64_t)wfirst - 1 + i;
             uint64_t b = w >= 0 ? bases[w] : 0ull;
@@ -434,7 +440,7 @@
                 ncnt += (int)(cn >> 2) - (int)(cf >> 2);
                 cp = cf;
             }
-            if ((((uint32_t)s + 1u) & ppr_mask) == 0u) bins.template flush<false>(lost);
+            if ((((uint32_t)s + 1u) & fmask) == 0u) bins.template flush<false>(lost);
         }
         rmask16[(wfirst * 2) + tid] = (uint16_t)word;
     }
@@ -449,7 +455,7 @@
           const uint32_t *__restrict__ cnt1, uint64_t cap1, uint64_t *buf2, uint32_t *cnt2, const uint64_t *__restrict__ off2, QOverflow ovf,
           PtShard sh, uint32_t prev_wpb, int log_prev_nb2, uint32_t nreg_cap, uint32_t sched_cap, const uint64_t *__restrict__ off1,
           const uint64_t *__restrict__ own1, const uint32_t *__restrict__ owncnt1, uint32_t *__restrict__ bnd = nullptr, uint32_t n_groups = 0,
-          uint32_t tiles_per_wg = 0, uint32_t batch_tiles = 0, uint32_t pb2 = 0)
+          uint32_t tiles_per_wg = 0, uint32_t batch_tiles = 0, uint32_t pb2 = 0, const uint32_t *__restrict__ tile_begin = nullptr)
 {
     extern __shared__ __attribute__((aligned(16))) unsigned char smem[];
     const uint32_t NB1 = 1u << LOG_NB1, NB2 = 1u << LOG_NB2;
@@ -481,7 +487,10 @@
     const uint32_t S6 = (uint32_t)slice_bits, PB2 = pb2;
     uint32_t next_g = 1;
     uint32_t *my_bnd = P6 ? bnd + (uint64_t)blockIdx.x * NB2 * n_groups * 2u : nullptr;
-    auto gmax = [=](uint32_t w) { return (uint32_t)((min((uint64_t)(w + 1u) * tiles_per_wg, (uint64_t)batch_tiles) * (uint64_t)(PT_THREADS * TPC_RUN) - 1ull) >> PB2); };
+    auto gmax = [=](uint32_t w) {
+        const uint64_t e = tile_begin ? min((uint64_t)tile_begin[w + 1u], (uint64_t)batch_tiles) : min((uint64_t)(w + 1u) * tiles_per_wg, (uint64_t)batch_tiles);
+        return e ? (uint32_t)((e * (uint64_t)(PT_THREADS * TPC_RUN) - 1ull) >> PB2) : 0u;
+    };
     struct Lost6 {
         QOverflow ovf; const uint32_t *next_g; uint32_t b1, S6, PB2; int shift1;
         __device__ __forceinline__ void pair(uint32_t b2, uint64_t val, uint64_t &addr, uint64_t &sid) const
@@ -1428,7 +1437,7 @@
                            pl.tile0, pl.n_tiles, pl.pos_per_round, lo, hi, pl.buf1, pl.cnt1, pl.cap1, ovf, perm, sh,                          \
                            pl.tile0_global * (uint64_t)(PT_THREADS * TPC_RUN), rmask, pl.fmt == 6 ? pl.tiles_per_wg : 0u,                  \
                            reinterpret_cast<const uint16_t *>(a.per_qs),            \
-                           mode, reinterpret_cast<const uint4 *>(a.qseed));                                                                \
+                           mode, reinterpret_cast<const uint4 *>(a.qseed), pl.fmt == 6 ? pl.tile_begin : nullptr, pl.tile_live);            \
     } while (0)
 #define TPC_QHASH2_GS(H, X, C)                                                                                                              \
     do {                                                                                                                                    \
@@ -1638,7 +1647,7 @@
     (void)hipFuncSetAttribute((const void *)k_q_split<false, false, true>, hipFuncAttributeMaxDynamicSharedMemorySize, (int)lds);
     hipLaunchKernelGGL((k_q_split<false, false, true>), dim3((1u << pl.b1) * pl.wpb), dim3(QS_THREADS), lds, a.stream, pl.b1, pl.b2, a.P.L, pl.slice_bits, pl.loads, pl.nwg1, pl.wpb,
                        pl.rbuf1, pl.rcnt1, pl.cap1, pl.buf2, pl.cnt2, pl.off2, ovf, sh, 0u, 0, nreg_cap, sched_cap, pl.roff1, (const uint64_t *)nullptr, (const uint32_t *)nullptr,
-                       pl.bnd, pl.n_groups, pl.tiles_per_wg, (uint32_t)pl.n_tiles, pl.pb2);
+                       pl.bnd, pl.n_groups, pl.tiles_per_wg, (uint32_t)pl.n_tiles, pl.pb2, pl.tile_begin);
 }
 
 constexpr int MK_LOADS = 4;
```

After: 22.68 billion (median of 6 runs). +72.4%, better.
